# ShenhanQian/KGDet

Measured on AMD Instinct MI355X. Metric: training images/sec (whole node) KGDet R50-FPN 800x1333, higher is better.
Workload: dtype f32 (3 MFMA products per multiply on hi/lo-split operands -- fp16 parts forward, bf16 parts for gradients --, f32 accumulate); 1 GPU; KGDet R50-FPN train step, 2 img/GPU at 800x1333 (padded 800x1344), DeformConv fwd/bwd + focal/moment losses + grad-clip + Adam; no collective at dp1 (one rank: nothing to exchange); global_batch=2, parallelism=dp1

## Files before the change

include/kgdet_hip.h:

```cpp
#ifndef KGDET_HIP_H_
#define KGDET_HIP_H_

#include <stddef.h>
#include <stdint.h>

#ifdef __cplusplus
extern "C" {
#endif

#define KGDET_OK 0
#define KGDET_E_SHAPE 1
#define KGDET_E_WORKSPACE 2
#define KGDET_E_HIP 3
size_t kgdet_conv_packed_bytes(int32_t M, int32_t K, int32_t taps);
int kgdet_conv_pack(const float *w, int32_t O, int32_t C, int32_t taps, int32_t transpose, void *packed, void *stream);
int kgdet_conv_pack_fmt(const float *w, int32_t O, int32_t C, int32_t taps, int32_t transpose, void *packed,
                        int32_t operand_format, void *stream);
int kgdet_conv_pack_both_fmt(const float *w, int32_t O, int32_t C, int32_t taps, void *packed, void *packed_t,
                             int32_t forward_format, void *stream);
int kgdet_conv_apply_epilogue_fmt(const void *packed, const float *x, float *y, const float *bias, const float *residual,
                                  int32_t relu, int64_t B, int32_t M, int32_t K, int32_t H, int32_t W, int32_t taps,
                                  int32_t stride, int32_t operand_format, void *workspace, size_t workspace_bytes,
                                  void *stream);
int kgdet_conv_apply_gated_fmt(const void *packed, const float *x, float *y, const float *bias, const float *residual,
                               int32_t relu, const float *gate, int64_t B, int32_t M, int32_t K, int32_t H, int32_t W,
                               int32_t taps, int32_t stride, int32_t operand_format, void *workspace, size_t workspace_bytes,
                               void *stream);
int kgdet_stem_conv7x7_s2_fmt(const void *packed, const float *x, float *y, int64_t B, int32_t H, int32_t W,
                              int32_t operand_format, void *stream);
int kgdet_conv_pack_both(const float *w, int32_t O, int32_t C, int32_t taps, void *packed, void *packed_t, void *stream);
int64_t kgdet_conv_pack_blocks(int32_t O, int32_t C, int32_t taps);
int kgdet_conv_pack_multi(const int64_t *desc_dev, int32_t n, int64_t total_blocks, void *stream);
size_t kgdet_conv_apply_workspace_bytes(int64_t B, int32_t M, int32_t K, int32_t H, int32_t W, int32_t taps,
                                        int32_t stride);
int kgdet_conv_apply(const void *packed, const float *x, float *y, int64_t B, int32_t M, int32_t K, int32_t H, int32_t W,
                     int32_t taps, int32_t stride, void *workspace, size_t workspace_bytes, void *stream);
int kgdet_conv_apply_epilogue(const void *packed, const float *x, float *y, const float *bias, const float *residual,
                              int32_t relu, int64_t B, int32_t M, int32_t K, int32_t H, int32_t W, int32_t taps,
                              int32_t stride, void *workspace, size_t workspace_bytes, void *stream);
int kgdet_stem_conv7x7_s2(const void *packed, const float *x, float *y, int64_t B, int32_t H, int32_t W, void *stream);
int kgdet_conv3x3_s2_grad_input(const void *packed_t, const float *grad_y, float *grad_x, int64_t B, int32_t C, int32_t O,
                                int32_t Hin, int32_t Win, void *stream);
size_t kgdet_conv3x3_s2_grad_weight_workspace_bytes(int64_t B, int32_t O, int32_t C, int32_t H, int32_t W);
int kgdet_conv3x3_s2_grad_weight(const float *grad_y, const float *x, float *grad_w, int64_t B, int32_t O, int32_t C, int32_t H,
                                 int32_t W, void *workspace, size_t workspace_bytes, void *stream);
size_t kgdet_conv1x1_grad_weight_workspace_bytes(int64_t B, int32_t O, int32_t C, int64_t HW);
int kgdet_conv1x1_grad_weight(const float *grad_y, const float *x, float *grad_w, int64_t B, int32_t O, int32_t C,
                              int64_t HW, void *workspace, size_t workspace_bytes, void *stream);
size_t kgdet_conv3x3_grad_weight_workspace_bytes(int64_t B, int32_t O, int32_t C, int32_t H, int32_t W);
int kgdet_conv3x3_grad_weight(const float *grad_y, const float *x, float *grad_w, int64_t B, int32_t O, int32_t C,
                              int32_t H, int32_t W, void *workspace, size_t workspace_bytes, void *stream);

int kgdet_bn_act_forward(const float *x, const float *gamma, const float *beta, const float *mean, const float *var,
                         float eps, const float *residual, float *y, int64_t N, int32_t C, int64_t HW, int32_t relu,
                         void *stream);
int32_t kgdet_bn_act_partials(int64_t N, int32_t C, int64_t HW);
int kgdet_bn_act_backward(const float *grad_y, const float *x, const float *y, const float *gamma, const float *beta,
                          const float *mean, const float *var, float eps, int32_t has_residual, int32_t relu,
                          float *grad_x, float *grad_residual, float *partial, float *sums, int64_t N, int32_t C,
                          int64_t HW, void *stream);
int kgdet_conv1x1_nhwc_residual(const void *x, const void *weight, const float *bias, const void *residual, void *out,
                                int64_t M, int32_t K, int32_t N, int32_t relu, void *stream);
int kgdet_conv1x1_nhwc_residual_in(const void *x, const float *in_bias, const void *weight, const float *bias,
                                   const void *residual, void *out, int64_t M, int32_t K, int32_t N, int32_t relu,
                                   void *stream);
int kgdet_bn_fold_backward(const float *grad_z, const float *z, int32_t relu, float *g, float *partial, int64_t N, int32_t C,
                           int64_t HW, void *stream);
int kgdet_bn_fold_finish(const float *partial, int32_t P, const float *w, float *G , const float *s,
                         const float *mean, const float *var, float eps, float *grad_beta ,
                         float *grad_gamma , int32_t O, int32_t CK, void *stream);
int kgdet_conv1x1_grad_weight_fold(const float *grad_y, const float *x, float *grad_w, int64_t B, int32_t O, int32_t C,
                                   int64_t HW, void *workspace, size_t workspace_bytes, const float *w, const float *s,
                                   const float *mean, const float *var, float eps, const float *bn_partial, int32_t P,
                                   float *grad_beta , float *grad_gamma , void *stream);
int kgdet_conv3x3_grad_weight_fold(const float *grad_y, const float *x, float *grad_w, int64_t B, int32_t O, int32_t C,
                                   int32_t H, int32_t W, void *workspace, size_t workspace_bytes, const float *w,
                                   const float *s, const float *mean, const float *var, float eps, const float *bn_partial,
                                   int32_t P, float *grad_beta , float *grad_gamma , void *stream);
int kgdet_bn_relu_maxpool(const float *x, const float *gamma, const float *beta, const float *mean, const float *var,
                          float eps, float *y, int64_t N, int32_t C, int32_t H, int32_t W, void *stream);

int kgdet_bias_act(void *x, const float *bias, const void *residual, int64_t N, int32_t C, int64_t HW, int32_t dtype,
                   int32_t relu, int32_t channels_last, void *stream);
int kgdet_bias_relu_maxpool_nhwc(const void *x, const float *bias, void *y, int64_t N, int32_t C, int32_t H, int32_t W,
                                 int32_t dtype, void *stream);

#define KGDET_E_UNSUPPORTED 4
#define KGDET_E_PARTIAL 5

const char *kgdet_last_error(void);
int kgdet_version(void);
int kgdet_device_cu_count(void);

#define KGDET_OPT_EXACT_BACKWARD 0
#define KGDET_OPT_FWD_COLUMN_WAVE 1
#define KGDET_OPT_WGRAD_STREAMK 2
#define KGDET_OPT_BWD_PHASE 3
#define KGDET_OPT_COUNT 4
int kgdet_set_option(int32_t option, int32_t value);

typedef struct kgdet_dcn_shape {
  int32_t N, C, H, W;
  int32_t O, kh, kw;
  int32_t stride_h, stride_w, pad_h, pad_w, dil_h, dil_w;
  int32_t groups, deformable_groups;
  int32_t out_channel_offset, out_channels_total;
} kgdet_dcn_shape;

#define KGDET_DCN_RELU 1u
#define KGDET_DCN_BF16 2u
#define KGDET_DCN_EXACT_FP32 4u

int kgdet_dcn_output_size(const kgdet_dcn_shape *s, int32_t *Ho, int32_t *Wo);

size_t kgdet_dcn_packed_weight_bytes(const kgdet_dcn_shape *s);
size_t kgdet_dcn_workspace_bytes(const kgdet_dcn_shape *s);

int kgdet_dcn_pack_weight(const kgdet_dcn_shape *s, const float *weight, float *packed, void *stream);
int kgdet_dcn_pack_weight_multi(int32_t n, const kgdet_dcn_shape *const *shapes, const float *const *weights,
                                float *const *packeds, void *stream);
int kgdet_dcn_pack_weight_images(int32_t n, const kgdet_dcn_shape *const *shapes, const float *const *weights,
                                 float *const *packeds, uint32_t images, void *stream);
int32_t kgdet_dcn_split_path_complete(const kgdet_dcn_shape *shape);
int kgdet_dcn_unpack_weight_grad(const kgdet_dcn_shape *s, const float *packed, float *grad_weight,
                                 int accumulate, void *stream);

int kgdet_deform_conv_forward(const kgdet_dcn_shape *s, const float *input, const float *offset,
                              const float *mask , const float *packed_weight,
                              const float *bias , float *output, uint32_t flags,
                              void *workspace, size_t workspace_bytes, void *stream);

size_t kgdet_dcn_group_workspace_bytes(int32_t n, const kgdet_dcn_shape *const *shapes);

int kgdet_deform_conv_forward_grouped(int32_t n, const kgdet_dcn_shape *const *shapes, const float *const *inputs,
                                      const float *const *offsets, const float *const *masks ,
                                      const float *const *packed_weights, const float *const *biases ,
                                      float *const *outputs, uint32_t flags, void *workspace,
                                      size_t workspace_bytes, void *stream);

int kgdet_deform_conv_grad_input(const kgdet_dcn_shape *s, const float *offset, const float *mask ,
                                 const float *packed_weight, const float *grad_output, float *grad_input,
                                 uint32_t flags, void *workspace, size_t workspace_bytes, void *stream);

int kgdet_deform_conv_grad_offset(const kgdet_dcn_shape *s, const float *input, const float *offset,
                                  const float *packed_weight, const float *grad_output, float *grad_offset,
                                  uint32_t flags, void *workspace, size_t workspace_bytes, void *stream);

int kgdet_deform_conv_backward_input_grouped(int32_t n, const kgdet_dcn_shape *const *shapes, const float *const *inputs,
                                             const float *const *offsets, const float *const *packed_weights,
                                             const float *const *grad_outputs, float *const *grad_inputs,
                                             float *const *grad_offsets, void *workspace, size_t workspace_bytes,
                                             void *stream);

int kgdet_deform_conv_grad_weight_grouped(int32_t n, const kgdet_dcn_shape *const *shapes, const float *const *inputs,
                                          const float *const *offsets, const float *const *grad_outputs,
                                          float *const *grad_weights, void *workspace, size_t workspace_bytes,
                                          void *stream);

int kgdet_deform_conv_backward_input(const kgdet_dcn_shape *s, const float *input, const float *offset,
                                     const float *mask , const float *packed_weight,
                                     const float *grad_output, float *grad_input, float *grad_offset,
                                     float *grad_mask , void *workspace,
                                     size_t workspace_bytes, void *stream);

int kgdet_deform_conv_backward_weight(const kgdet_dcn_shape *s, const float *input, const float *offset,
                                      const float *mask , const float *grad_output,
                                      float *grad_weight, float *grad_bias , int accumulate,
                                      void *workspace, size_t workspace_bytes, void *stream);

typedef struct kgdet_psroi_shape {
  int32_t B, C, H, W;
  int32_t R;
  int32_t out_dim, group_size, pooled_size, part_size, sample_per_part;
  int32_t no_trans, num_classes;
  float spatial_scale, trans_std;
} kgdet_psroi_shape;

size_t kgdet_deform_psroi_forward_workspace_bytes(const kgdet_psroi_shape *s);
int kgdet_deform_psroi_forward(const kgdet_psroi_shape *s, const float *data, const float *rois,
                               const float *trans, float *out, float *count, void *workspace, size_t workspace_bytes,
                               void *stream);
size_t kgdet_deform_psroi_backward_workspace_bytes(const kgdet_psroi_shape *s);
int kgdet_deform_psroi_backward(const kgdet_psroi_shape *s, const float *grad_out, const float *count,
                                const float *data, const float *rois, const float *trans,
                                float *grad_data, float *grad_trans, void *workspace, size_t workspace_bytes,
                                void *stream);

int kgdet_sigmoid_focal_loss_forward(const float *logits, const int64_t *targets, int64_t num,
                                     int32_t num_classes, float gamma, float alpha, float *losses,
                                     void *stream);
int kgdet_sigmoid_focal_loss_backward(const float *logits, const int64_t *targets, const float *d_losses,
                                      int64_t num, int32_t num_classes, float gamma, float alpha,
                                      float *d_logits, void *stream);

#define KGDET_HEAD_MAX_IMAGES 16
typedef struct kgdet_head_targets {
  int32_t B, H, W, num_classes, num_keypoints;
  float stride;
  int32_t num_gt[KGDET_HEAD_MAX_IMAGES];
  const float *gt_bboxes[KGDET_HEAD_MAX_IMAGES];
  const int64_t *gt_labels[KGDET_HEAD_MAX_IMAGES];
  const float *gt_keypoints[KGDET_HEAD_MAX_IMAGES];
  int32_t valid_h[KGDET_HEAD_MAX_IMAGES], valid_w[KGDET_HEAD_MAX_IMAGES];
} kgdet_head_targets;
// ... 108 lines not shown
```

kgdet_amd/conv1x1.py:

```python
import ctypes
import weakref

import torch

from . import _lib


import os as _os
SPLIT_GRAD_WEIGHT_3X3 = _os.environ.get('KGDET_SPLIT_WGRAD3', '1') == '1'
PACK_BOTH = _os.environ.get('KGDET_PACK_BOTH', '1') == '1'


PAD_GRAD_WEIGHT_3X3 = _os.environ.get('KGDET_NO_WPAD') is None
DIRECT_ODD_MAPS = _os.environ.get('KGDET_DIRECT_ODD_MAPS', '1') == '1'
ENABLED = True


RAGGED_1X1 = _os.environ.get('KGDET_CONV_RAGGED_1X1', '1') == '1'


def applicable(x, weight, stride=(1, 1), padding=(0, 0), dilation=(1, 1), groups=1):
    k = weight.shape[2]
    aligned = weight.shape[1] % 16 == 0 and weight.shape[0] % 16 == 0
    return (ENABLED and x.is_cuda and x.dtype == torch.float32 and weight.dtype == torch.float32 and x.dim() == 4
            and weight.shape[2] == weight.shape[3] and k in (1, 3) and tuple(stride) == (1, 1)
            and tuple(padding) == (k // 2, k // 2) and tuple(dilation) == (1, 1) and groups == 1
            and x.is_contiguous() and (aligned or (k == 1 and RAGGED_1X1 and (weight.shape[0] * weight.shape[1]) % 2 == 0))
            and ((x.shape[2] * x.shape[3]) % 2 == 0 or DIRECT_ODD_MAPS) and x.shape[2] * x.shape[3] >= 4
            and not torch.is_autocast_enabled())


_L = None
_sizes = {}


def _lib_sizes():
    global _L
    if _L is None:
        L = _lib.lib()
        vp, i32, i64, sz = ctypes.c_void_p, ctypes.c_int32, ctypes.c_int64, ctypes.c_size_t
        for name, res, args in (
                ('kgdet_conv_packed_bytes', sz, [i32, i32, i32]),
                ('kgdet_conv_apply_workspace_bytes', sz, [i64, i32, i32, i32, i32, i32, i32]),
                ('kgdet_conv1x1_grad_weight_workspace_bytes', sz, [i64, i32, i32, i64]),
                ('kgdet_conv3x3_grad_weight_workspace_bytes', sz, [i64, i32, i32, i32, i32]),
                ('kgdet_conv_pack_fmt', ctypes.c_int, [vp, i32, i32, i32, i32, vp, i32, vp]),
                ('kgdet_conv_pack_both_fmt', ctypes.c_int, [vp, i32, i32, i32, vp, vp, i32, vp]),
                ('kgdet_conv_pack_blocks', i64, [i32, i32, i32]),
                ('kgdet_conv_pack_multi', ctypes.c_int, [vp, i32, i64, vp]),
                ('kgdet_conv_apply', ctypes.c_int, [vp, vp, vp, i64, i32, i32, i32, i32, i32, i32, vp, sz, vp]),
                ('kgdet_conv_apply_epilogue_fmt', ctypes.c_int,
                 [vp, vp, vp, vp, vp, i32, i64, i32, i32, i32, i32, i32, i32, i32, vp, sz, vp]),
                ('kgdet_conv_apply_gated_fmt', ctypes.c_int,
                 [vp, vp, vp, vp, vp, i32, vp, i64, i32, i32, i32, i32, i32, i32, i32, vp, sz, vp]),
                ('kgdet_conv3x3_s2_grad_input', ctypes.c_int, [vp, vp, vp, i64, i32, i32, i32, i32, vp]),
                ('kgdet_conv3x3_s2_grad_weight_workspace_bytes', sz, [i64, i32, i32, i32, i32]),
                ('kgdet_conv3x3_s2_grad_weight', ctypes.c_int, [vp, vp, vp, i64, i32, i32, i32, i32, vp, sz, vp]),
                ('kgdet_conv1x1_grad_weight', ctypes.c_int, [vp, vp, vp, i64, i32, i32, i64, vp, sz, vp]),
                ('kgdet_conv1x1_grad_weight_fold', ctypes.c_int,
                 [vp, vp, vp, i64, i32, i32, i64, vp, sz, vp, vp, vp, vp, ctypes.c_float, vp, i32, vp, vp, vp]),
                ('kgdet_conv3x3_grad_weight_fold', ctypes.c_int,
                 [vp, vp, vp, i64, i32, i32, i32, i32, vp, sz, vp, vp, vp, vp, ctypes.c_float, vp, i32, vp, vp, vp]),
                ('kgdet_conv3x3_grad_weight', ctypes.c_int, [vp, vp, vp, i64, i32, i32, i32, i32, vp, sz, vp])):
            fn = getattr(L, name)
            fn.restype, fn.argtypes = res, args
        _L = L
    return _L


def _size(name, *args):
    key = (name, args)
    n = _sizes.get(key)
    if n is None:
        n = _sizes[key] = getattr(_lib_sizes(), name)(*args)
    return n


def _stream():
    return _lib.raw_stream()


FORWARD_F16 = _os.environ.get('KGDET_CONV_FWD_F16', '1') == '1'


def _mark(img, f16):
    img.kgdet_f16 = bool(f16)
    return img


def _pack(weight, transpose):
    L = _lib_sizes()
    O, C, taps = weight.shape[0], weight.shape[1], weight.shape[2] * weight.shape[3]
    M, K = (C, O) if transpose else (O, C)
    img = torch.empty(_size('kgdet_conv_packed_bytes', M, K, taps), dtype=torch.uint8, device=weight.device)
    f16 = FORWARD_F16 and not transpose
    _lib.check(L.kgdet_conv_pack_fmt(weight.data_ptr(), O, C, taps, 1 if transpose else 0, img.data_ptr(), 1 if f16 else 0,
                                     _stream()), 'conv_pack')
    return _mark(img, f16)


def _pack_both(weight):
    L = _lib_sizes()
    O, C, taps = weight.shape[0], weight.shape[1], weight.shape[2] * weight.shape[3]
    img = torch.empty(_size('kgdet_conv_packed_bytes', O, C, taps), dtype=torch.uint8, device=weight.device)
    img_t = torch.empty(_size('kgdet_conv_packed_bytes', C, O, taps), dtype=torch.uint8, device=weight.device)
    _lib.check(L.kgdet_conv_pack_both_fmt(weight.data_ptr(), O, C, taps, img.data_ptr(), img_t.data_ptr(),
                                          1 if FORWARD_F16 else 0, _stream()), 'conv_pack_both')
    return _mark(img, FORWARD_F16), _mark(img_t, False)


def _apply(img, x, M, taps, stride=1, bias=None, residual=None, relu=False, gate=None):
    L = _lib_sizes()
    B, K, H, W = x.shape
    y = torch.empty((B, M, (H + stride - 1) // stride, (W + stride - 1) // stride), dtype=torch.float32, device=x.device)
    nbytes = _size('kgdet_conv_apply_workspace_bytes', B, M, K, H, W, taps, stride)
    ws = torch.empty(nbytes, dtype=torch.uint8, device=x.device) if nbytes else None
    if gate is not None and (gate.shape != y.shape or gate.dtype != torch.float32 or not gate.is_contiguous()):
        raise ValueError('gate must be a contiguous fp32 tensor of the output\'s shape')
    _lib.check(L.kgdet_conv_apply_gated_fmt(
        img.data_ptr(), x.data_ptr(), y.data_ptr(), bias.data_ptr() if bias is not None else None,
        residual.data_ptr() if residual is not None else None, 1 if relu else 0,
        gate.data_ptr() if gate is not None else None, B, M, K, H, W, taps, stride,
        1 if getattr(img, 'kgdet_f16', False) else 0, ws.data_ptr() if nbytes else None, nbytes, _stream()), 'conv_apply')
    return y


def gate_applicable(y_shape):
    return (y_shape[2] * y_shape[3]) % 2 == 0


class _Entry(object):
    __slots__ = ('ref', 'img', 'img_t', 'token', 'ptr')


_entries = {}
_token = 0
_generation = 0
_table = None
PACK_MULTI = _os.environ.get('KGDET_PACK_MULTI', '1') == '1'


FOLD_BN = _os.environ.get('KGDET_FOLD_BN', '1') == '1'


class _FoldEntry(object):
    __slots__ = ('ref', 'bn', 'img', 'img_t', 's', 't', 'token', 'ptr')


_fold_entries = {}
_fold_flat = None


def _fold_refresh(live):
    global _fold_flat
    key = tuple((k, e.ptr, id(e.bn()), id(e.bn().weight), id(e.bn().bias), id(e.bn().running_mean), id(e.bn().running_var),
                 e.bn().weight.data_ptr(), e.bn().running_var.data_ptr()) for k, e in live)
    if _fold_flat is None or _fold_flat[0] != key:
        dev = live[0][1].img.device
        sizes = [e.ref().shape[0] for _, e in live]
        total = sum(sizes)
        S, T, TMP = (torch.empty(total, dtype=torch.float32, device=dev) for _ in range(3))
        EPS = torch.cat([torch.full((n,), float(e.bn().eps), dtype=torch.float32) for n, (_, e) in zip(sizes, live)]).to(dev)
        sv, tv, mv, off = [], [], [], 0
        for n, (_, e) in zip(sizes, live):
            sv.append(S[off:off + n]); tv.append(T[off:off + n]); mv.append(TMP[off:off + n])
            e.s, e.t = sv[-1], tv[-1]
            off += n
        bns = [e.bn() for _, e in live]
        _fold_flat = (key, S, T, TMP, EPS, sv, tv, mv, [b.weight for b in bns], [b.bias for b in bns],
                      [b.running_mean for b in bns], [b.running_var for b in bns])
    _, S, T, TMP, EPS, sv, tv, mv, gammas, betas, means, vars_ = _fold_flat
    with torch.no_grad():
        torch._foreach_copy_(mv, vars_)
        TMP.add_(EPS).rsqrt_()
        torch._foreach_copy_(sv, gammas)
        S.mul_(TMP)
        torch._foreach_copy_(tv, means)
        T.mul_(S).neg_()
        torch._foreach_add_(tv, betas)


def _launch_multi():
    global _table
    dead = [k for k, e in _entries.items() if e.ref() is None or e.ref().data_ptr() != e.ptr]
    for k in dead:
        del _entries[k]
    dead = [k for k, e in _fold_entries.items() if e.ref() is None or e.bn() is None or e.ref().data_ptr() != e.ptr]
    for k in dead:
        del _fold_entries[k]
    for k in _fold_entries:
        _entries.pop(k, None)
    if not _entries and not _fold_entries:
        return
    live = list(_entries.items())
    folded = list(_fold_entries.items())
    if folded:
        _fold_refresh(folded)
    key = (tuple((k, e.ptr, e.img.data_ptr(), e.img_t.data_ptr()) for k, e in live),
           tuple((k, e.ptr, e.img.data_ptr(), e.img_t.data_ptr(), e.s.data_ptr()) for k, e in folded))
    L = _lib_sizes()
    if _table is None or _table[0] != key:
        rows, first = [], 0
        for _, e in live + folded:
            w = e.ref()
            O, C, taps = w.shape[0], w.shape[1], w.shape[2] * w.shape[3]
            rows.append([w.data_ptr(), e.img.data_ptr(), e.img_t.data_ptr(), (O << 32) | C,
                         (taps << 32) | first | ((1 << 62) if getattr(e.img, 'kgdet_f16', False) else 0),
                         e.s.data_ptr() if isinstance(e, _FoldEntry) else 0])
            first += L.kgdet_conv_pack_blocks(O, C, taps)
        dev = (live + folded)[0][1].img.device
        _table = (key, torch.tensor(rows, dtype=torch.int64).to(dev), first)
    _lib.check(L.kgdet_conv_pack_multi(_table[1].data_ptr(), len(live) + len(folded), _table[2], _stream()), 'conv_pack_multi')
    for _, e in live + folded:
        e.token = _token


def fold_images(weight, bn):
    if not (FOLD_BN and PACK_MULTI and _token):
        return None
    e = _fold_entries.get(id(weight))
    if e is not None and e.ref() is weight and e.ptr == weight.data_ptr() and e.bn() is bn:
        return (e.img, e.img_t, e.s, e.t) if e.token == _token else None
    O, C, taps = weight.shape[0], weight.shape[1], weight.shape[2] * weight.shape[3]
    if (isinstance(weight, torch.nn.Parameter) and weight.is_contiguous() and O % 16 == 0 and C % 16 == 0 and bn.affine
            and taps in (1, 9)):
        e = _FoldEntry()
        e.ref, e.bn, e.ptr, e.token = weakref.ref(weight), weakref.ref(bn), weight.data_ptr(), 0
        e.img = _mark(torch.empty(_size('kgdet_conv_packed_bytes', O, C, taps), dtype=torch.uint8, device=weight.device),
                      FORWARD_F16)
        e.img_t = _mark(torch.empty(_size('kgdet_conv_packed_bytes', C, O, taps), dtype=torch.uint8, device=weight.device), False)
        e.s = e.t = None
        _fold_entries[id(weight)] = e
    return None


class step_scope(object):

    def __enter__(self):
        global _token, _generation
        self.prev = _token
        _generation += 1
        _token = _generation
        if PACK_MULTI and (_entries or _fold_entries):
            _launch_multi()

    def __exit__(self, *exc):
        global _token
        _token = self.prev


_aliases = {}


def alias(proxy, param):
    key = id(proxy)
    _aliases[key] = (weakref.ref(proxy, lambda _r, key=key: _aliases.pop(key, None)), weakref.ref(param))


def forward_images(x, weight):
    both = PACK_BOTH and x.requires_grad and (weight.shape[0] % 16 == 0 or weight.shape[2] == 1)
    a = _aliases.get(id(weight))
    if a is not None and a[0]() is weight:
        origin = a[1]()
        if origin is not None and origin.data_ptr() == weight.data_ptr() and origin.shape == weight.shape:
            weight = origin
    if both and PACK_MULTI and _token:
        e = _entries.get(id(weight))
        if e is not None and e.ref() is weight and e.ptr == weight.data_ptr():
            if e.token != _token:
                _lib.check(_lib_sizes().kgdet_conv_pack_both_fmt(weight.data_ptr(), weight.shape[0], weight.shape[1],
                                                                 weight.shape[2] * weight.shape[3], e.img.data_ptr(),
                                                                 e.img_t.data_ptr(), 1 if getattr(e.img, 'kgdet_f16', False) else 0,
                                                                 _stream()), 'conv_pack_both')
                e.token = _token
            return e.img, e.img_t
        img, img_t = _pack_both(weight)
        if isinstance(weight, torch.nn.Parameter):
            e = _Entry()
            e.ref, e.img, e.img_t, e.token, e.ptr = weakref.ref(weight), img, img_t, _token, weight.data_ptr()
            _entries[id(weight)] = e
        return img, img_t
    if both:
        return _pack_both(weight)
    return _pack(weight, False), None


def grad_weight(x, weight, gy):
    O, C, k = weight.shape[0], weight.shape[1], weight.shape[2]
    L = _lib_sizes()
    if k == 3 and SPLIT_GRAD_WEIGHT_3X3 and C % 128 == 0:
        if x.shape[3] % 4 and not PAD_GRAD_WEIGHT_3X3:
            return torch.nn.grad.conv2d_weight(x, weight.shape, gy, padding=1)
        B, H, W = x.shape[0], x.shape[2], x.shape[3]
        nbytes = _size('kgdet_conv3x3_grad_weight_workspace_bytes', B, O, C, H, W)
        ws = torch.empty(nbytes, dtype=torch.uint8, device=x.device)
        gw = torch.empty_like(weight)
        _lib.check(L.kgdet_conv3x3_grad_weight(gy.data_ptr(), x.data_ptr(), gw.data_ptr(), B, O, C, H, W,
                                               ws.data_ptr(), nbytes, _stream()), 'conv3x3_grad_weight')
        return gw
    if k != 1 or ((x.shape[2] * x.shape[3]) % 4 != 0 and not PAD_GRAD_WEIGHT_3X3):
        return torch.nn.grad.conv2d_weight(x, weight.shape, gy, padding=k // 2)
    B, HW = x.shape[0], x.shape[2] * x.shape[3]
    nbytes = _size('kgdet_conv1x1_grad_weight_workspace_bytes', B, O, C, HW)
    ws = torch.empty(nbytes, dtype=torch.uint8, device=x.device)
    gw = torch.empty_like(weight)
    _lib.check(L.kgdet_conv1x1_grad_weight(gy.data_ptr(), x.data_ptr(), gw.data_ptr(), B, O, C, HW,
                                           ws.data_ptr(), nbytes, _stream()), 'conv1x1_grad_weight')
    return gw


def grad_weight_fold_route(x, weight):
    C, k = weight.shape[1], weight.shape[2]
    if k == 3 and SPLIT_GRAD_WEIGHT_3X3 and C % 128 == 0 and (x.shape[3] % 4 == 0 or PAD_GRAD_WEIGHT_3X3):
        return 3
    if k == 1 and ((x.shape[2] * x.shape[3]) % 4 == 0 or PAD_GRAD_WEIGHT_3X3):
        return 1
    return 0


def grad_weight_fold(x, weight, gy, s, mean, var, eps, bn_partial, P, want_gamma=True):
    O, C, k = weight.shape[0], weight.shape[1], weight.shape[2]
    L = _lib_sizes()
    if bn_partial is None:
        P = 0

        class bn_partial(object):
            @staticmethod
            def data_ptr():
                return None
    if k == 3 and SPLIT_GRAD_WEIGHT_3X3 and C % 128 == 0 and (x.shape[3] % 4 == 0 or PAD_GRAD_WEIGHT_3X3):
        B, H, W = x.shape[0], x.shape[2], x.shape[3]
        nbytes = _size('kgdet_conv3x3_grad_weight_workspace_bytes', B, O, C, H, W)
        ws = torch.empty(nbytes, dtype=torch.uint8, device=x.device)
        gw = torch.empty_like(weight)
        sums = torch.empty((2, O), dtype=torch.float32, device=x.device)
        _lib.check(L.kgdet_conv3x3_grad_weight_fold(gy.data_ptr(), x.data_ptr(), gw.data_ptr(), B, O, C, H, W, ws.data_ptr(), nbytes,
                                                    weight.data_ptr(), s.data_ptr(), mean.data_ptr(), var.data_ptr(), eps,
                                                    bn_partial.data_ptr(), P, sums[0].data_ptr(),
                                                    sums[1].data_ptr() if want_gamma else None, _stream()), 'conv3x3_grad_weight_fold')
        return gw, sums
    if k == 1 and ((x.shape[2] * x.shape[3]) % 4 == 0 or PAD_GRAD_WEIGHT_3X3):
        B, HW = x.shape[0], x.shape[2] * x.shape[3]
        nbytes = _size('kgdet_conv1x1_grad_weight_workspace_bytes', B, O, C, HW)
        ws = torch.empty(nbytes, dtype=torch.uint8, device=x.device)
        gw = torch.empty_like(weight)
        sums = torch.empty((2, O), dtype=torch.float32, device=x.device)
        _lib.check(L.kgdet_conv1x1_grad_weight_fold(gy.data_ptr(), x.data_ptr(), gw.data_ptr(), B, O, C, HW, ws.data_ptr(), nbytes,
                                                    weight.data_ptr(), s.data_ptr(), mean.data_ptr(), var.data_ptr(), eps,
                                                    bn_partial.data_ptr(), P, sums[0].data_ptr(),
                                                    sums[1].data_ptr() if want_gamma else None, _stream()), 'conv1x1_grad_weight_fold')
        return gw, sums
    return None


def grad_input(weight, img_t, gy, residual=None, gate=None):
    C, k = weight.shape[1], weight.shape[2]
    return _apply(img_t if img_t is not None else _pack(weight, True), gy, C, k * k, residual=residual, gate=gate)


class _ConvSplit(torch.autograd.Function):
    @staticmethod
    def forward(ctx, x, weight):
        weight = weight.contiguous()
        img, ctx.img_t = forward_images(x, weight)
        ctx.save_for_backward(x, weight)
        return _apply(img, x, weight.shape[0], weight.shape[2] * weight.shape[3])

    @staticmethod
    def backward(ctx, gy):
        x, weight = ctx.saved_tensors
        gy = gy.contiguous()
        gx = grad_input(weight, ctx.img_t, gy) if ctx.needs_input_grad[0] else None
        gw = grad_weight(x, weight, gy) if ctx.needs_input_grad[1] else None
        return gx, gw


def conv_split(x, weight):
    return _ConvSplit.apply(x, weight)


PAD_ODD_MAPS = _os.environ.get('KGDET_PAD_ODD_MAPS', '1') == '1'


def odd_map_applicable(x, weight, stride=(1, 1), padding=(0, 0), dilation=(1, 1), groups=1):
    return (PAD_ODD_MAPS and x.dim() == 4 and (x.shape[2] * x.shape[3]) % 2 == 1 and x.shape[2] % 2 == 1 and x.is_cuda
            and x.dtype == torch.float32 and x.is_contiguous()
            and applicable(_PadProbe(x), weight, stride, padding, dilation, groups))


class _PadProbe(object):

    def __init__(self, x):
        self.is_cuda, self.dtype = x.is_cuda, x.dtype
        self.shape = (x.shape[0], x.shape[1], x.shape[2], x.shape[3] + 1)

    def dim(self):
        return 4

    def is_contiguous(self):
        return True


def pad_odd(x):
    return torch.nn.functional.pad(x, (0, 1))


def unpad_odd(y, width):
    return y[..., :width].contiguous()


conv1x1 = conv_split


BIAS_GRAD_IN_WGRAD = _os.environ.get('KGDET_BIAS_GRAD_IN_WGRAD', '1') == '1'
_ones_cache = {}


def _ones(n, device):
    t = _ones_cache.get((n, device))
    if t is None:
        t = _ones_cache[(n, device)] = torch.ones(n, dtype=torch.float32, device=device)
    return t


class _ConvBiasAct(torch.autograd.Function):

    @staticmethod
    def forward(ctx, x, weight, bias, relu):
        weight = weight.contiguous()
        img, ctx.img_t = forward_images(x, weight)
        y = _apply(img, x, weight.shape[0], weight.shape[2] * weight.shape[3], 1, bias.contiguous(), None, relu)
        ctx.relu = relu
        ctx.save_for_backward(x, weight, y if relu else None)
        return y

    @staticmethod
    def backward(ctx, gy):
        x, weight, y = ctx.saved_tensors
        if ctx.relu:
            gy = torch.ops.aten.threshold_backward(gy, y, 0)
        gy = gy.contiguous()
        gx = grad_input(weight, ctx.img_t, gy) if ctx.needs_input_grad[0] else None
        if BIAS_GRAD_IN_WGRAD and ctx.needs_input_grad[1] and ctx.needs_input_grad[2] and grad_weight_fold_route(x, weight):
            one = _ones(weight.shape[0], weight.device)
            res = grad_weight_fold(x, weight, gy, one, one, one, 0.0, None, 0, want_gamma=False)
            if res is not None:
                return gx, res[0], res[1][0], None
        gw = grad_weight(x, weight, gy) if ctx.needs_input_grad[1] else None
        gb = gy.sum((0, 2, 3)) if ctx.needs_input_grad[2] else None
        return gx, gw, gb, None


CACHE_INFER_CASTS = _os.environ.get('KGDET_CACHE_INFER_CASTS', '1') == '1'


GEMM_1X1_NCHW = _os.environ.get('KGDET_INFER_GEMM_1X1_NCHW', '1') == '1'


_cast_cache = weakref.WeakKeyDictionary()


def invalidate_inference_caches():
    global _fold_flat
    _cast_cache.clear()
    _fold_flat = None
    from . import backbone, dcn
    backbone.clear_fold_cache()
    dcn.clear_pack_cache()


def conv_infer(conv, x):
    if (CACHE_INFER_CASTS and type(conv) is torch.nn.Conv2d and not torch.is_grad_enabled() and x.is_cuda
            and torch.is_autocast_enabled() and conv.weight.dtype == torch.float32 and conv.padding_mode == 'zeros'):
        dt = torch.get_autocast_dtype('cuda')
        cl = x.dim() == 4 and not x.is_contiguous() and x.is_contiguous(memory_format=torch.channels_last)
        key = (conv.weight._version, conv.weight.data_ptr(), id(conv.weight),
               None if conv.bias is None else (conv.bias._version, conv.bias.data_ptr(), id(conv.bias)), dt, cl)
        c = _cast_cache.get(conv)
        if c is None or c[0] != key:
            w = conv.weight.detach().to(dt)
            if cl:
                w = w.contiguous(memory_format=torch.channels_last)
            c = (key, w, None if conv.bias is None else conv.bias.detach().to(dt))
            _cast_cache[conv] = c
        if (GEMM_1X1_NCHW and not cl and x.dim() == 4 and x.is_contiguous() and x.dtype == dt and conv.kernel_size == (1, 1)
                and conv.stride == (1, 1) and conv.padding == (0, 0) and conv.groups == 1):
            B, _, H, W = x.shape
            y = torch.matmul(c[1].view(c[1].shape[0], -1), x.view(B, x.shape[1], H * W))
            if c[2] is not None:
                y += c[2].view(1, -1, 1)
            return y.view(B, -1, H, W)
        return torch.nn.functional.conv2d(x, c[1], c[2], conv.stride, conv.padding, conv.dilation, conv.groups)
    return conv(x)


def conv_bias_act(conv, x, relu=False):
    if (type(conv) is torch.nn.Conv2d and conv.bias is not None and torch.is_grad_enabled()
            and conv.bias.dtype == torch.float32
            and applicable(x, conv.weight, conv.stride, conv.padding, conv.dilation, conv.groups)):
        return _ConvBiasAct.apply(x, conv.weight, conv.bias, relu)
    if (type(conv) is torch.nn.Conv2d and conv.bias is not None and torch.is_grad_enabled() and conv.bias.dtype == torch.float32
            and odd_map_applicable(x, conv.weight, conv.stride, conv.padding, conv.dilation, conv.groups)):
        return unpad_odd(_ConvBiasAct.apply(pad_odd(x), conv.weight, conv.bias, relu), x.shape[3])
    y = conv_infer(conv, x)
    return torch.relu(y) if relu else y


class _ConvSplitStride2(torch.autograd.Function):

    @staticmethod
# ... 54 lines not shown
```

kgdet_amd/csrc/conv1x1.hip:

```cpp
#include "common.h"

namespace kgdet {

namespace {

typedef __bf16 bf16x8 __attribute__((ext_vector_type(8)));
typedef float f32x16 __attribute__((ext_vector_type(16)));
typedef float f32x4 __attribute__((ext_vector_type(4)));
typedef float f32x2 __attribute__((ext_vector_type(2)));

constexpr int kTM = 128, kTN = 128, kTK = 16;
constexpr int kPart = 2 * kTM * 16;
constexpr int kStage = 2 * kPart;

typedef __bf16 bf16x2 __attribute__((ext_vector_type(2)));
__device__ __forceinline__ void split_pair(float v0, float v1, unsigned &hi, unsigned &lo) {
  const f32x2 v = {v0, v1};
  hi = __builtin_bit_cast(unsigned, __builtin_convertvector(v, bf16x2));
  const f32x2 hf = {__uint_as_float(hi << 16), __uint_as_float(hi & 0xffff0000u)};
  lo = __builtin_bit_cast(unsigned, __builtin_convertvector(v - hf, bf16x2));
}
__device__ __forceinline__ void split8(const float (&v)[8], bf16x8 &hi, bf16x8 &lo) {
  typedef unsigned u32x4 __attribute__((ext_vector_type(4)));
  u32x4 h, l;
// ... 277 lines not shown
    }
    const float *xp = xb + (long long)(c16 * kTK + kq * 4) * Nin + shift;
    if (TAPS == 1 && (K & (kTK - 1)) && c16 == K / kTK) {
#pragma unroll
      for (int j = 0; j < 4; ++j) R.v[j] = xb[(long long)min(c16 * kTK + kq * 4 + j, K - 1) * Nin];
    } else {
#pragma unroll
      for (int j = 0; j < 4; ++j) R.v[j] = xp[(long long)j * Nin];
    }
  };
  auto commit = [&](int buf, const Regs &R) {
    unsigned char *As = smem + buf * kBuf, *Bs = As + kStage;
    *reinterpret_cast<f32x4 *>(As + (tid & 511) * 16) = R.a;
    uint2 hi, lo;
#ifdef KGDET_CONV_ABL_NOSPLIT
    hi.x = __float_as_uint(R.v[0]); hi.y = __float_as_uint(R.v[1]); lo.x = __float_as_uint(R.v[2]); lo.y = __float_as_uint(R.v[3]);
#else
    split_pair_t<F16>(R.live ? R.v[0] : 0.0f, R.live ? R.v[1] : 0.0f, hi.x, lo.x);
    split_pair_t<F16>(R.live ? R.v[2] : 0.0f, R.live ? R.v[3] : 0.0f, hi.y, lo.y);
#endif
    unsigned char *dst = Bs + (kq >> 1) * (TN * 16) + n_local * 16 + (kq & 1) * 8;
    *reinterpret_cast<uint2 *>(dst) = hi;
    *reinterpret_cast<uint2 *>(dst + kPartB) = lo;
  };
  auto multiply = [&](int buf) {
    const unsigned char *A = smem + buf * kBuf + (lane >> 5) * (kTM * 16) + (wm * 64 + (lane & 31)) * 16;
    const unsigned char *Bp = smem + buf * kBuf + kStage + (lane >> 5) * (TN * 16) + (wn * 32 + (lane & 31)) * 16;
    bf16x8 a[2][2], bb[2];
#ifdef KGDET_CONV_ABL_NOLDSREAD
#pragma unroll
    for (int pt = 0; pt < 2; ++pt) {
      a[pt][0] = __builtin_bit_cast(bf16x8, acc[0].lo.lo); a[pt][1] = __builtin_bit_cast(bf16x8, acc[1].lo.lo);
      bb[pt] = __builtin_bit_cast(bf16x8, acc[1].hi.lo);
    }
#else
#pragma unroll
    for (int pt = 0; pt < 2; ++pt) {
      a[pt][0] = *reinterpret_cast<const bf16x8 *>(A + pt * kPart);
      a[pt][1] = *reinterpret_cast<const bf16x8 *>(A + pt * kPart + 32 * 16);
      bb[pt] = *reinterpret_cast<const bf16x8 *>(Bp + pt * kPartB);
    }
#endif
#ifdef KGDET_CONV_ABL_NOMFMA
#pragma unroll
    for (int mi = 0; mi < 2; ++mi) {
      const f32x4 q = __builtin_bit_cast(f32x4, a[0][mi]) + __builtin_bit_cast(f32x4, a[1][mi]) + __builtin_bit_cast(f32x4, bb[0]) + __builtin_bit_cast(f32x4, bb[1]);
      acc[mi][0] += q[0]; acc[mi][1] += q[1]; acc[mi][2] += q[2]; acc[mi][3] += q[3];
    }
    if (false)
#endif
#pragma unroll
    for (int mi = 0; mi < 2; ++mi) {
      acc[mi] = mfma_t<F16>(a[1][mi], bb[0], acc[mi]);
      acc[mi] = mfma_t<F16>(a[0][mi], bb[1], acc[mi]);
      acc[mi] = mfma_t<F16>(a[0][mi], bb[0], acc[mi]);
    }
  };
  {
    Regs R[kPF];
#pragma unroll
    for (int i = 0; i < kPF; ++i) issue(i, R[i]);
#ifdef KGDET_GATE_EARLY
    if (!F16 && gate) {
#pragma unroll
      for (int mi = 0; mi < 2; ++mi)
#pragma unroll
        for (int r = 0; r < 16; ++r) asm volatile("" : "+v"(gv[mi][r]));
    }
#endif
    commit(0, R[0]);
    const int full = stages / kPF * kPF;
    for (int s0 = 0; s0 < full; s0 += kPF) {
#pragma unroll
      for (int u = 0; u < kPF; ++u) {
        const int s = s0 + u;
        __syncthreads();
        issue(s + kPF, R[u]);
        multiply(s & 1);
        commit((s + 1) & 1, R[(u + 1) % kPF]);
      }
    }
#pragma unroll
    for (int u = 0; u < kPF - 1; ++u) {
      const int s = full + u;
      if (s < stages) {
        __syncthreads();
        multiply(s & 1);
        if (s + 1 < stages) commit((s + 1) & 1, R[u + 1]);
      }
    }
  }

  float *yb = y + (long long)part * part_stride + (long long)b * M * N;
  const int n = n0 + wn * 32 + (lane & 31);
  if constexpr (F16) {
#pragma unroll
    for (int mi = 0; mi < 2; ++mi)
#pragma unroll
      for (int r = 0; r < 16; ++r) acc[mi][r] *= 1.0f / kF16WeightScale;
  }
  if (bias || residual) {
    const int nc = min(n, N - 1);
    float add[2][16];
#pragma unroll
    for (int mi = 0; mi < 2; ++mi)
#pragma unroll
      for (int r = 0; r < 16; ++r) {
        const int m = min(mt * kTM + wm * 64 + mi * 32 + (r & 3) + 8 * (r >> 2) + 4 * (lane >> 5), M - 1);
        float v = bias ? bias[m] : 0.0f;
        if (residual) v += residual[((long long)b * M + m) * N + nc];
        add[mi][r] = v;
      }
#pragma unroll
    for (int mi = 0; mi < 2; ++mi)
#pragma unroll
      for (int r = 0; r < 16; ++r) acc[mi][r] += add[mi][r];
  }
  if (gate) {
#ifdef KGDET_GATE_EARLY
    if constexpr (F16)
#endif
    {
    const int nc = min(n, N - 1);
#pragma unroll
    for (int mi = 0; mi < 2; ++mi)
#pragma unroll
      for (int r = 0; r < 16; ++r) {
        const int m = min(mt * kTM + wm * 64 + mi * 32 + (r & 3) + 8 * (r >> 2) + 4 * (lane >> 5), M - 1);
        gv[mi][r] = gate[((long long)b * M + m) * N + nc];
      }
    }
#pragma unroll
    for (int mi = 0; mi < 2; ++mi)
#pragma unroll
      for (int r = 0; r < 16; ++r) acc[mi][r] = gv[mi][r] > 0.0f ? acc[mi][r] : 0.0f;
  }
#pragma unroll
  for (int mi = 0; mi < 2; ++mi)
#pragma unroll
    for (int r = 0; r < 16; ++r) {
      const int m = mt * kTM + wm * 64 + mi * 32 + (r & 3) + 8 * (r >> 2) + 4 * (lane >> 5);
      if (m < M && n < N) yb[(long long)m * N + n] = relu ? fmaxf(acc[mi][r], 0.0f) : acc[mi][r];
    }
}

#ifdef KGDET_CONV_TRACE
static __device__ unsigned long long g_conv_trace[1024 * 8];
#define CV_NOW() __builtin_amdgcn_s_memtime()
#define CV_ADD(cat) do { const unsigned long long n__ = CV_NOW(); tr[cat] += n__ - tr_t; tr_t = n__; } while (0)
#else
#define CV_ADD(cat) do { } while (0)
#endif
constexpr int kPatchMax = 256;
constexpr int kPatchPart = 2 * kPatchMax * 16;
constexpr int kPatchBuf = 2 * kPatchPart;
constexpr int kPatchLds = 6 * kStage + 2 * kPatchBuf;

__global__ __launch_bounds__(kNNThreads) void conv3x3_patch(const unsigned char *__restrict__ img,
                                                            const float *__restrict__ x, float *__restrict__ y, int M,
                                                            int K, int H, int W, int n_mt, int tiles_x, int n_nt, int tiles,
                                                            int ksplit, long long part_stride, int TX, int TY,
                                                            const float *__restrict__ bias,
                                                            const float *__restrict__ residual, int relu,
    const float *__restrict__ gate = nullptr) {
  extern __shared__ __attribute__((aligned(16))) unsigned char smem[];
  const int unit = xcd_tile(blockIdx.x, tiles * ksplit);
  if (unit >= tiles * ksplit) return;
  const int part = unit % ksplit, tile = unit / ksplit;
  const int tid = threadIdx.x, lane = tid & 63, wave = tid >> 6, wm = wave & 1, wn = wave >> 1;
  const int N = H * W;
  const int chunks_all = K / kTK, per = (chunks_all + ksplit - 1) / ksplit;
  const int c_begin = part * per, c_end = max(c_begin, min(chunks_all, c_begin + per));
  const int chunks = c_end - c_begin, stages = chunks * 9;
  const int mt = tile % n_mt, nt = (tile / n_mt) % n_nt, b = tile / (n_mt * n_nt);
  const int y0 = (nt / tiles_x) * TY, x0 = (nt % tiles_x) * TX;
  const int PW = TX + 2, PP = PW * (TY + 2);

  const int khalf_l = tid >> 8, pp = tid & 255;
  const int ppy = pp / PW, ppx = pp - ppy * PW;
  const int iy = y0 - 1 + ppy, ix = x0 - 1 + ppx;
  const bool p_live = pp < PP && iy >= 0 && iy < H && ix >= 0 && ix < W;
  const float *xb = x + ((long long)b * K + khalf_l * 8) * N + (p_live ? iy * W + ix : 0);
  unsigned char *b_dst = smem + 6 * kStage + (khalf_l * kPatchMax + pp) * 16;

  const int q = min(wn * 32 + (lane & 31), TX * TY - 1);
  const int py = q / TX, px = q - py * TX;
  const unsigned char *b_row0 = smem + 6 * kStage + ((lane >> 5) * kPatchMax + py * PW + px) * 16;
  const int row_pitch = PW * 16;
  const unsigned char *a_rd = smem + (lane >> 5) * (kTM * 16) + (wm * 64 + (lane & 31)) * 16;
  const unsigned char *ai = img + (long long)mt * (chunks_all * 9) * kStage + (long long)min(c_begin, chunks_all - 1) * 9 * kStage + tid * 16;

  f32x16 acc[2];
#pragma unroll
  for (int i = 0; i < 2; ++i)
#pragma unroll
    for (int r = 0; r < 16; ++r) acc[i][r] = 0.0f;

  float bv[8];
  auto issue_b = [&](int ci) {
    const float *xp = xb + (long long)min(c_begin + min(ci, chunks - 1), chunks_all - 1) * kTK * N;
#pragma unroll
    for (int j = 0; j < 8; ++j) bv[j] = xp[(long long)j * N];
  };
  auto commit_b = [&](int buf) {
    float v[8];
#pragma unroll
    for (int j = 0; j < 8; ++j) asm volatile("" : "+v"(bv[j]));
#pragma unroll
    for (int j = 0; j < 8; ++j) v[j] = p_live ? bv[j] : 0.0f;
    bf16x8 hi, lo;
    split8(v, hi, lo);
    *reinterpret_cast<bf16x8 *>(b_dst + buf * kPatchBuf) = hi;
    *reinterpret_cast<bf16x8 *>(b_dst + buf * kPatchBuf + kPatchPart) = lo;
  };
  f32x4 R[3];
#ifdef KGDET_PATCH_ABL_NOAGLOBAL
  auto issue_a = [&](int s, f32x4 &r) { r[0] = (float)s; };
#else
  auto issue_a = [&](int s, f32x4 &r) { r = *reinterpret_cast<const f32x4 *>(ai + (long long)max(min(s, stages - 1), 0) * kStage); };
#endif

  struct Frags {
    bf16x8 a[2][2], b[2];
  };
  auto read_frags = [&](Frags &F, const unsigned char *A, const unsigned char *Bp) {
#ifdef KGDET_PATCH_ABL_NOLDSREAD
#pragma unroll
    for (int pt = 0; pt < 2; ++pt) {
      F.a[pt][0] = __builtin_bit_cast(bf16x8, acc[0].lo.lo); F.a[pt][1] = __builtin_bit_cast(bf16x8, acc[1].lo.lo);
      F.b[pt] = __builtin_bit_cast(bf16x8, acc[1].hi.lo);
    }
    return;
#endif
#pragma unroll
    for (int pt = 0; pt < 2; ++pt) {
      F.a[pt][0] = *reinterpret_cast<const bf16x8 *>(A + pt * kPart);
      F.a[pt][1] = *reinterpret_cast<const bf16x8 *>(A + pt * kPart + 32 * 16);
      F.b[pt] = *reinterpret_cast<const bf16x8 *>(Bp + pt * kPatchPart);
    }
  };
  auto mma = [&](const Frags &F) {
#ifdef KGDET_PATCH_ABL_NOMFMA
#pragma unroll
    for (int mi = 0; mi < 2; ++mi) {
      const f32x4 qv = __builtin_bit_cast(f32x4, F.a[0][mi]) + __builtin_bit_cast(f32x4, F.a[1][mi]) + __builtin_bit_cast(f32x4, F.b[0]) + __builtin_bit_cast(f32x4, F.b[1]);
      acc[mi][0] += qv[0]; acc[mi][1] += qv[1]; acc[mi][2] += qv[2]; acc[mi][3] += qv[3];
    }
    return;
#endif
#pragma unroll
    for (int mi = 0; mi < 2; ++mi) {
      acc[mi] = __builtin_amdgcn_mfma_f32_32x32x16_bf16(F.a[1][mi], F.b[0], acc[mi], 0, 0, 0);
      acc[mi] = __builtin_amdgcn_mfma_f32_32x32x16_bf16(F.a[0][mi], F.b[1], acc[mi], 0, 0, 0);
      acc[mi] = __builtin_amdgcn_mfma_f32_32x32x16_bf16(F.a[0][mi], F.b[0], acc[mi], 0, 0, 0);
    }
  };
#ifdef KGDET_CONV_TRACE
  unsigned long long tr[8] = {0, 0, 0, 0, 0, 0, 0, 0};
  unsigned long long tr_t = CV_NOW();
  const unsigned long long tr_start = tr_t;
#endif
  issue_b(0);
#pragma unroll
  for (int j = 0; j < 3; ++j) issue_a(j, R[j]);
  commit_b(0);
#pragma unroll
  for (int j = 0; j < 3; ++j) {
    *reinterpret_cast<f32x4 *>(smem + j * kStage + tid * 16) = R[j];
    issue_a(3 + j, R[j]);
  }
  Frags F[2];
  CV_ADD(5);
  for (int ci = 0; ci < chunks; ++ci) {
    issue_b(ci + 1);
    const unsigned char *brow = b_row0 + (ci & 1) * kPatchBuf;
    const int set0 = (ci & 1) * 3 * kStage;
#pragma unroll
    for (int r = 0; r < 3; ++r) {
      const int g = ci * 3 + r;
      const int cur = (r & 1) ? 3 * kStage - set0 : set0, nxt = 3 * kStage - cur;
#ifndef KGDET_PATCH_ABL_NOBARRIER
      __syncthreads();
#endif
      CV_ADD(0);
      read_frags(F[0], a_rd + cur, brow + r * row_pitch);
#pragma unroll
      for (int j = 0; j < 3; ++j) {
        if (j < 2) read_frags(F[(j + 1) & 1], a_rd + cur + (j + 1) * kStage, brow + r * row_pitch + (j + 1) * 16);
        __builtin_amdgcn_sched_barrier(0);
        CV_ADD(1);
        mma(F[j & 1]);
        __builtin_amdgcn_sched_barrier(0);
        CV_ADD(2);
        *reinterpret_cast<f32x4 *>(smem + nxt + j * kStage + tid * 16) = R[j];
        issue_a(3 * (g + 2) + j, R[j]);
        if (r == 2 && j == 1) commit_b((ci + 1) & 1);
        __builtin_amdgcn_sched_barrier(0);
        CV_ADD(3);
      }
    }
  }

#ifdef KGDET_CONV_TRACE
  tr[6] = CV_NOW() - tr_start;
  tr[7] = stages;
  tr[4] = ((unsigned long long)__builtin_amdgcn_s_getreg((20 << 0) | (0 << 6) | (31 << 11)) << 32) |
          __builtin_amdgcn_s_getreg((4 << 0) | (0 << 6) | (31 << 11));
  tr[5] = tr_start;
  if (tid == 0 && blockIdx.x < 1024)
    for (int c = 0; c < 8; ++c) g_conv_trace[blockIdx.x * 8 + c] = tr[c];
#endif
  float *yb = y + (long long)part * part_stride + (long long)b * M * N;
  const int qq = wn * 32 + (lane & 31);
  const int oy = y0 + py, ox = x0 + px;
  const bool o_live = qq < TX * TY && oy < H && ox < W;
  const int n = o_live ? oy * W + ox : 0;
  if (bias || residual) {
    float add[2][16];
#pragma unroll
    for (int mi = 0; mi < 2; ++mi)
#pragma unroll
      for (int r = 0; r < 16; ++r) {
        const int m = min(mt * kTM + wm * 64 + mi * 32 + (r & 3) + 8 * (r >> 2) + 4 * (lane >> 5), M - 1);
        float v = bias ? bias[m] : 0.0f;
        if (residual) v += residual[((long long)b * M + m) * N + n];
        add[mi][r] = v;
      }
#pragma unroll
    for (int mi = 0; mi < 2; ++mi)
#pragma unroll
      for (int r = 0; r < 16; ++r) acc[mi][r] += add[mi][r];
  }
  if (gate) {
    float gv[2][16];
#pragma unroll
    for (int mi = 0; mi < 2; ++mi)
#pragma unroll
      for (int r = 0; r < 16; ++r) {
        const int m = min(mt * kTM + wm * 64 + mi * 32 + (r & 3) + 8 * (r >> 2) + 4 * (lane >> 5), M - 1);
        gv[mi][r] = gate[((long long)b * M + m) * N + n];
      }
#pragma unroll
    for (int mi = 0; mi < 2; ++mi)
#pragma unroll
      for (int r = 0; r < 16; ++r) acc[mi][r] = gv[mi][r] > 0.0f ? acc[mi][r] : 0.0f;
  }
#pragma unroll
  for (int mi = 0; mi < 2; ++mi)
#pragma unroll
    for (int r = 0; r < 16; ++r) {
      const int m = mt * kTM + wm * 64 + mi * 32 + (r & 3) + 8 * (r >> 2) + 4 * (lane >> 5);
      if (m < M && o_live) yb[(long long)m * N + n] = relu ? fmaxf(acc[mi][r], 0.0f) : acc[mi][r];
    }
}

template <int WAVES, int NB, bool F16 = false>
__global__ __launch_bounds__(64 * WAVES) void conv3x3_patch4(const unsigned char *__restrict__ img,
                                                             const float *__restrict__ x, float *__restrict__ y, int M,
                                                             int K, int H, int W, int n_mt, int tiles_x, int n_nt,
                                                             int tiles, int ksplit, long long part_stride, int TX, int TY,
                                                             const float *__restrict__ bias,
                                                             const float *__restrict__ residual, int relu,
    const float *__restrict__ gate = nullptr) {
  __shared__ __attribute__((aligned(16))) unsigned char smem[2 * kPatchBuf];
  if constexpr (F16) f16_saturate_on();
  constexpr int HALVES = 4 / WAVES, THREADS = 64 * WAVES, PXT = kPatchMax / THREADS;
  const int unit0 = xcd_tile(blockIdx.x, tiles * ksplit * HALVES);
  if (unit0 >= tiles * ksplit * HALVES) return;
  const int half = unit0 % HALVES, unit = unit0 / HALVES;
  const int part = unit % ksplit, tile = unit / ksplit;
  const int tid = threadIdx.x, lane = tid & 63, wave = (tid >> 6) + half * WAVES;
  const int N = H * W;
  const int chunks_all = K / kTK, per = (chunks_all + ksplit - 1) / ksplit;
  const int c_begin = part * per, c_end = max(c_begin, min(chunks_all, c_begin + per));
  const int chunks = c_end - c_begin, stages = chunks * 9;
  const int mt = tile % n_mt, nt = (tile / n_mt) % n_nt, b = tile / (n_mt * n_nt);
  const int y0 = (nt / tiles_x) * TY, x0 = (nt % tiles_x) * TX;
  const int PW = TX + 2, PP = PW * (TY + 2);

  if (mt * kTM + half * 64 >= M) return;
  bool p_live[PXT];
  int p_off[PXT];
#pragma unroll
  for (int i = 0; i < PXT; ++i) {
    const int pp = tid + i * THREADS;
    const int ppy = pp / PW, ppx = pp - ppy * PW;
    const int iy = y0 - 1 + ppy, ix = x0 - 1 + ppx;
    p_live[i] = pp < PP && iy >= 0 && iy < H && ix >= 0 && ix < W;
    p_off[i] = p_live[i] ? iy * W + ix : 0;
  }
  const float *xb = x + (long long)b * K * N;
  unsigned char *b_dst = smem + tid * 16;

  int b_rd[NB], o_n[NB];
  bool o_live[NB];
#pragma unroll
  for (int nb = 0; nb < NB; ++nb) {
    const int qq = nb * 32 + (lane & 31), q = min(qq, TX * TY - 1);
    const int py = q / TX, px = q - py * TX;
    b_rd[nb] = ((lane >> 5) * kPatchMax + py * PW + px) * 16;
    o_live[nb] = qq < TX * TY && y0 + py < H && x0 + px < W;
    o_n[nb] = o_live[nb] ? (y0 + py) * W + x0 + px : 0;
  }
  const int row_pitch = PW * 16;
  const unsigned char *ag = img + ((long long)mt * chunks_all + min(c_begin, chunks_all - 1)) * 9 * kStage +
                            (lane >> 5) * (kTM * 16) + (wave * 32 + (lane & 31)) * 16;

  f32x16 acc[NB];
#pragma unroll
  for (int i = 0; i < NB; ++i)
#pragma unroll
    for (int r = 0; r < 16; ++r) acc[i][r] = 0.0f;

  float bv[PXT][16];
  auto issue_b = [&](int ci) {
    const float *xp = xb + (long long)min(c_begin + min(ci, chunks - 1), chunks_all - 1) * kTK * N;
#pragma unroll
    for (int i = 0; i < PXT; ++i)
#pragma unroll
      for (int j = 0; j < 16; ++j) bv[i][j] = xp[(long long)j * N + p_off[i]];
  };
  auto commit_b = [&](int buf) {
#pragma unroll
    for (int i = 0; i < PXT; ++i)
#pragma unroll
      for (int j = 0; j < 16; ++j) asm volatile("" : "+v"(bv[i][j]));
#pragma unroll
    for (int i = 0; i < PXT; ++i)
#pragma unroll
      for (int kh = 0; kh < 2; ++kh) {
        float v[8];
#pragma unroll
        for (int j = 0; j < 8; ++j) v[j] = p_live[i] ? bv[i][kh * 8 + j] : 0.0f;
        bf16x8 hi, lo;
        split8_t<F16>(v, hi, lo);
        unsigned char *d = b_dst + i * THREADS * 16 + buf * kPatchBuf + kh * (kPatchMax * 16);
        *reinterpret_cast<bf16x8 *>(d) = hi;
        *reinterpret_cast<bf16x8 *>(d + kPatchPart) = lo;
      }
  };
  bf16x8 AR[3][2];
  auto issue_a = [&](int s, bf16x8 (&r)[2]) {
    const unsigned char *p = ag + (long long)max(min(s, stages - 1), 0) * kStage;
    r[0] = *reinterpret_cast<const bf16x8 *>(p);
    r[1] = *reinterpret_cast<const bf16x8 *>(p + kPart);
  };

  issue_b(0);
#pragma unroll
  for (int j = 0; j < 3; ++j) issue_a(j, AR[j]);
  commit_b(0);
  for (int ci = 0; ci < chunks; ++ci) {
    issue_b(ci + 1);
    __syncthreads();
    const unsigned char *bbuf = smem + (ci & 1) * kPatchBuf;
#pragma unroll
    for (int t = 0; t < 9; ++t) {
      const int s = ci * 9 + t;
      const unsigned char *bt = bbuf + (t / 3) * row_pitch + (t % 3) * 16;
      bf16x8 bf[NB][2];
#pragma unroll
      for (int nb = 0; nb < NB; ++nb) {
        bf[nb][0] = *reinterpret_cast<const bf16x8 *>(bt + b_rd[nb]);
        bf[nb][1] = *reinterpret_cast<const bf16x8 *>(bt + b_rd[nb] + kPatchPart);
      }
#pragma unroll
      for (int nb = 0; nb < NB; ++nb) acc[nb] = mfma_t<F16>(AR[t % 3][1], bf[nb][0], acc[nb]);
#pragma unroll
      for (int nb = 0; nb < NB; ++nb) acc[nb] = mfma_t<F16>(AR[t % 3][0], bf[nb][1], acc[nb]);
#pragma unroll
      for (int nb = 0; nb < NB; ++nb) acc[nb] = mfma_t<F16>(AR[t % 3][0], bf[nb][0], acc[nb]);
      __builtin_amdgcn_sched_barrier(0);
      issue_a(s + 3, AR[t % 3]);
      if (t == 6) commit_b((ci + 1) & 1);
      __builtin_amdgcn_sched_barrier(0);
    }
  }

  float *yb = y + (long long)part * part_stride + (long long)b * M * N;
  const int m0 = mt * kTM + wave * 32 + 4 * (lane >> 5);
#pragma unroll
  for (int nb = 0; nb < NB; ++nb) {
    if constexpr (F16) {
#pragma unroll
      for (int r = 0; r < 16; ++r) acc[nb][r] *= 1.0f / kF16WeightScale;
    }
    if (bias || residual) {
      float add[16];
#pragma unroll
      for (int r = 0; r < 16; ++r) {
        const int m = min(m0 + (r & 3) + 8 * (r >> 2), M - 1);
        float v = bias ? bias[m] : 0.0f;
        if (residual) v += residual[((long long)b * M + m) * N + o_n[nb]];
        add[r] = v;
      }
#pragma unroll
      for (int r = 0; r < 16; ++r) acc[nb][r] += add[r];
    }
    if (gate) {
      float gv[16];
#pragma unroll
      for (int r = 0; r < 16; ++r) gv[r] = gate[((long long)b * M + min(m0 + (r & 3) + 8 * (r >> 2), M - 1)) * N + o_n[nb]];
#pragma unroll
      for (int r = 0; r < 16; ++r) acc[nb][r] = gv[r] > 0.0f ? acc[nb][r] : 0.0f;
    }
#pragma unroll
    for (int r = 0; r < 16; ++r) {
      const int m = m0 + (r & 3) + 8 * (r >> 2);
      if (m < M && o_live[nb]) yb[(long long)m * N + o_n[nb]] = relu ? fmaxf(acc[nb][r], 0.0f) : acc[nb][r];
    }
  }
}

__global__ __launch_bounds__(256) void conv3x3_s2_grad_input(const unsigned char *__restrict__ img_t,
                                                             const float *__restrict__ gy, float *__restrict__ gx, int M,
                                                             int K, int H, int W, int Hin, int Win, int n_mt, int tiles_x,
                                                             int n_nt, int tiles, int TX, int TY) {
  __shared__ __attribute__((aligned(16))) unsigned char smem[2 * kPatchBuf];
  constexpr int NB = 2;
  const int tile = xcd_tile(blockIdx.x, tiles);
  if (tile >= tiles) return;
  const int tid = threadIdx.x, lane = tid & 63, wave = tid >> 6;
  const int N = H * W;
  const int chunks = K / kTK, stages = chunks * 9;
  const int mt = tile % n_mt, nt = (tile / n_mt) % n_nt, b = tile / (n_mt * n_nt);
  const int y0 = (nt / tiles_x) * TY, x0 = (nt % tiles_x) * TX;
  const int PW = TX + 2, PP = PW * (TY + 2);

  const int pp = tid;
  const int ppy = pp / PW, ppx = pp - ppy * PW;
  const int iy = y0 - 1 + ppy, ix = x0 - 1 + ppx;
  const bool p_live = pp < PP && iy >= 0 && iy < H && ix >= 0 && ix < W;
  const float *xb = gy + (long long)b * K * N + (p_live ? iy * W + ix : 0);
  unsigned char *b_dst = smem + pp * 16;

  int b_rd[NB], o_y[NB], o_x[NB];
#pragma unroll
  for (int nb = 0; nb < NB; ++nb) {
    const int qq = nb * 32 + (lane & 31), q = min(qq, TX * TY - 1);
    const int py = q / TX, px = q - py * TX;
    b_rd[nb] = ((lane >> 5) * kPatchMax + py * PW + px) * 16;
    const bool live = qq < TX * TY && y0 + py < H && x0 + px < W;
    o_y[nb] = live ? 2 * (y0 + py) : Hin;
    o_x[nb] = 2 * (x0 + px);
  }
  const int row_pitch = PW * 16;
  const unsigned char *ag = img_t + (long long)mt * stages * kStage + (lane >> 5) * (kTM * 16) + (wave * 32 + (lane & 31)) * 16;

  f32x16 acc[4][NB];
#pragma unroll
  for (int c = 0; c < 4; ++c)
#pragma unroll
    for (int i = 0; i < NB; ++i)
#pragma unroll
      for (int r = 0; r < 16; ++r) acc[c][i][r] = 0.0f;

  float bv[16];
  auto issue_b = [&](int ci) {
    const float *xp = xb + (long long)min(ci, chunks - 1) * kTK * N;
#pragma unroll
    for (int j = 0; j < 16; ++j) bv[j] = xp[(long long)j * N];
  };
  auto commit_b = [&](int buf) {
#pragma unroll
    for (int j = 0; j < 16; ++j) asm volatile("" : "+v"(bv[j]));
#pragma unroll
    for (int kh = 0; kh < 2; ++kh) {
      float v[8];
#pragma unroll
      for (int j = 0; j < 8; ++j) v[j] = p_live ? bv[kh * 8 + j] : 0.0f;
      bf16x8 hi, lo;
      split8(v, hi, lo);
      *reinterpret_cast<bf16x8 *>(b_dst + buf * kPatchBuf + kh * (kPatchMax * 16)) = hi;
      *reinterpret_cast<bf16x8 *>(b_dst + buf * kPatchBuf + kh * (kPatchMax * 16) + kPatchPart) = lo;
    }
  };
  bf16x8 AR[3][2];
  auto issue_a = [&](int s, bf16x8 (&r)[2]) {
    const int sc = min(s, stages - 1), ci = sc / 9, t = sc - ci * 9;
    const unsigned char *p = ag + (long long)(ci * 9 + 8 - t) * kStage;
    r[0] = *reinterpret_cast<const bf16x8 *>(p);
    r[1] = *reinterpret_cast<const bf16x8 *>(p + kPart);
  };

  issue_b(0);
#pragma unroll
  for (int j = 0; j < 3; ++j) issue_a(j, AR[j]);
  commit_b(0);
  for (int ci = 0; ci < chunks; ++ci) {
    issue_b(ci + 1);
    __syncthreads();
    const unsigned char *bbuf = smem + (ci & 1) * kPatchBuf;
#pragma unroll
    for (int t = 0; t < 9; ++t) {
      constexpr int kDummy = 0;
      const int ky = t / 3, kx = t % 3;
      const int cls = 2 * (ky != 1) + (kx != 1), dy = ky == 0, dx = kx == 0;
      const unsigned char *bt = bbuf + (1 + dy) * row_pitch + (1 + dx) * 16;
      bf16x8 bf[NB][2];
#pragma unroll
      for (int nb = 0; nb < NB; ++nb) {
        bf[nb][0] = *reinterpret_cast<const bf16x8 *>(bt + b_rd[nb]);
        bf[nb][1] = *reinterpret_cast<const bf16x8 *>(bt + b_rd[nb] + kPatchPart);
      }
#pragma unroll
      for (int nb = 0; nb < NB; ++nb) acc[cls][nb] = __builtin_amdgcn_mfma_f32_32x32x16_bf16(AR[t % 3][1], bf[nb][0], acc[cls][nb], 0, 0, 0);
#pragma unroll
      for (int nb = 0; nb < NB; ++nb) acc[cls][nb] = __builtin_amdgcn_mfma_f32_32x32x16_bf16(AR[t % 3][0], bf[nb][1], acc[cls][nb], 0, 0, 0);
#pragma unroll
      for (int nb = 0; nb < NB; ++nb) acc[cls][nb] = __builtin_amdgcn_mfma_f32_32x32x16_bf16(AR[t % 3][0], bf[nb][0], acc[cls][nb], 0, 0, 0);
      __builtin_amdgcn_sched_barrier(0);
      issue_a(ci * 9 + t + 3, AR[t % 3]);
      if (t == 6) commit_b((ci + 1) & 1);
      __builtin_amdgcn_sched_barrier(0);
      (void)kDummy;
    }
  }

  const long long Nin = (long long)Hin * Win;
  float *xo = gx + (long long)b * M * Nin;
  const int m0 = mt * kTM + wave * 32 + 4 * (lane >> 5);
#pragma unroll
  for (int nb = 0; nb < NB; ++nb)
#pragma unroll
    for (int r = 0; r < 16; ++r) {
      const int m = m0 + (r & 3) + 8 * (r >> 2);
      if (m >= M) continue;
      float *row = xo + (long long)m * Nin;
#pragma unroll
      for (int pa = 0; pa < 2; ++pa) {
        const int oy = o_y[nb] + pa;
        if (oy >= Hin) continue;
#pragma unroll
        for (int qa = 0; qa < 2; ++qa)
          if (o_x[nb] + qa < Win) row[(long long)oy * Win + o_x[nb] + qa] = acc[2 * pa + qa][nb][r];
      }
    }
}

constexpr int kStemTY = 8, kStemTX = 16, kStemPH = 2 * kStemTY + 5, kStemPW = 2 * kStemTX + 5, kStemK = 160;

template <bool F16>
__global__ __launch_bounds__(256) void stem_conv7x7_s2(const unsigned char *__restrict__ img, const float *__restrict__ x,
                                                       float *__restrict__ y, int H, int W, int Ho, int Wo, int tiles_x,
                                                       int tiles_per_image) {
  __shared__ float patch[3 * kStemPH * kStemPW];
  __shared__ int koff[kStemK];
  if constexpr (F16) f16_saturate_on();
  const int tid = threadIdx.x, lane = tid & 63, wave = tid >> 6;
  const int b = blockIdx.x / tiles_per_image, nt = blockIdx.x - b * tiles_per_image;
  const int oy0 = (nt / tiles_x) * kStemTY, ox0 = (nt % tiles_x) * kStemTX;
  const int iy0 = 2 * oy0 - 3, ix0 = 2 * ox0 - 3;
  const float *xb = x + (long long)b * 3 * H * W;
  for (int i = tid; i < 3 * kStemPH * kStemPW; i += 256) {
    const int c = i / (kStemPH * kStemPW), r = i - c * (kStemPH * kStemPW), py = r / kStemPW, px = r - py * kStemPW;
    const int iy = iy0 + py, ix = ix0 + px;
    patch[i] = (iy >= 0 && iy < H && ix >= 0 && ix < W) ? xb[((long long)c * H + iy) * W + ix] : 0.0f;
  }
  if (tid < kStemK) {
    const int c = tid / 49, r = tid - c * 49, ky = r / 7, kx = r - ky * 7;
    koff[tid] = tid < 147 ? c * (kStemPH * kStemPW) + ky * kStemPW + kx : 0;
  }
  __syncthreads();
  const int q = wave * 32 + (lane & 31), py = q / kStemTX, px = q - py * kStemTX;
  const float *pbase = patch + (2 * py) * kStemPW + 2 * px;
  const int kh = (lane >> 5) * 8;
  const unsigned char *ag = img + (lane >> 5) * (kTM * 16) + (lane & 31) * 16;
  f32x16 acc[2];
#pragma unroll
  for (int i = 0; i < 2; ++i)
#pragma unroll
    for (int r = 0; r < 16; ++r) acc[i][r] = 0.0f;
#pragma unroll
  for (int s = 0; s < kStemK / kTK; ++s) {
    bf16x8 a[2][2];
#pragma unroll
    for (int mi = 0; mi < 2; ++mi) {
      a[0][mi] = *reinterpret_cast<const bf16x8 *>(ag + (long long)s * kStage + mi * 32 * 16);
      a[1][mi] = *reinterpret_cast<const bf16x8 *>(ag + (long long)s * kStage + kPart + mi * 32 * 16);
    }
    float v[8];
#pragma unroll
    for (int j = 0; j < 8; ++j) v[j] = pbase[koff[s * kTK + kh + j]];
    bf16x8 bhi, blo;
    split8_t<F16>(v, bhi, blo);
#pragma unroll
    for (int mi = 0; mi < 2; ++mi) {
      acc[mi] = mfma_t<F16>(a[1][mi], bhi, acc[mi]);
      acc[mi] = mfma_t<F16>(a[0][mi], blo, acc[mi]);
      acc[mi] = mfma_t<F16>(a[0][mi], bhi, acc[mi]);
    }
  }
  const int oy = oy0 + py, ox = ox0 + px;
  if (oy < Ho && ox < Wo) {
    float *yb = y + (long long)b * 64 * Ho * Wo + (long long)oy * Wo + ox;
#pragma unroll
    for (int mi = 0; mi < 2; ++mi)
#pragma unroll
      for (int r = 0; r < 16; ++r) {
        const int m = mi * 32 + (r & 3) + 8 * (r >> 2) + 4 * (lane >> 5);
        yb[(long long)m * Ho * Wo] = F16 ? acc[mi][r] * (1.0f / kF16WeightScale) : acc[mi][r];
      }
  }
}

__global__ __launch_bounds__(256) void conv1x1_sum(const float *__restrict__ parts, float *__restrict__ out,
                                                   long long n, long long stride, int count) {
  for (long long i = (blockIdx.x * 256LL + threadIdx.x) * 2; i < n; i += gridDim.x * 512LL) {
    f32x2 s = {0.0f, 0.0f};
    int k = 0;
    for (; k + 8 <= count; k += 8) {
      f32x2 v[8];
#pragma unroll
      for (int e = 0; e < 8; ++e) v[e] = *reinterpret_cast<const f32x2 *>(parts + (long long)(k + e) * stride + i);
#pragma unroll
      for (int e = 0; e < 8; ++e) s += v[e];
    }
    for (; k + 2 <= count; k += 2) {
      const f32x2 v0 = *reinterpret_cast<const f32x2 *>(parts + (long long)k * stride + i);
      const f32x2 v1 = *reinterpret_cast<const f32x2 *>(parts + (long long)(k + 1) * stride + i);
      s = (s + v0) + v1;
    }
    for (; k < count; ++k) s += *reinterpret_cast<const f32x2 *>(parts + (long long)k * stride + i);
    *reinterpret_cast<f32x2 *>(out + i) = s;
  }
}

__global__ __launch_bounds__(256) void conv1x1_sum_epilogue(const float *__restrict__ parts, float *__restrict__ out,
                                                            long long n, long long stride, int count,
                                                            const float *__restrict__ bias, const float *__restrict__ residual,
                                                            int relu, int M, long long HW,
                                                            const float *__restrict__ gate = nullptr) {
  for (long long i = (blockIdx.x * 256LL + threadIdx.x) * 2; i < n; i += gridDim.x * 512LL) {
    f32x2 s = {0.0f, 0.0f};
    int k = 0;
    for (; k + 4 <= count; k += 4) {
      f32x2 v[4];
#pragma unroll
      for (int e = 0; e < 4; ++e) v[e] = *reinterpret_cast<const f32x2 *>(parts + (long long)(k + e) * stride + i);
#pragma unroll
      for (int e = 0; e < 4; ++e) s += v[e];
    }
    for (; k < count; ++k) s += *reinterpret_cast<const f32x2 *>(parts + (long long)k * stride + i);
    if (bias) {
      const float b = bias[(i / HW) % M];
      s[0] += b; s[1] += b;
    }
    if (residual) s += *reinterpret_cast<const f32x2 *>(residual + i);
    if (relu) { s[0] = fmaxf(s[0], 0.0f); s[1] = fmaxf(s[1], 0.0f); }
    if (gate) {
      const f32x2 gv = *reinterpret_cast<const f32x2 *>(gate + i);
      s[0] = gv[0] > 0.0f ? s[0] : 0.0f; s[1] = gv[1] > 0.0f ? s[1] : 0.0f;
    }
    *reinterpret_cast<f32x2 *>(out + i) = s;
  }
}

struct ConvFoldArgs {
  const float *w, *s, *mean, *var, *bn_partial;
  float *grad_beta, *grad_gamma;
  float eps;
  int P;
};
template <bool T9>
__global__ __launch_bounds__(1024) void conv_wsum_fold(const float *__restrict__ parts, float *__restrict__ out, int C,
                                                       long long stride, int count, const ConvFoldArgs f) {
  extern __shared__ float row_s[];
  __shared__ float red[2][16];
  const int o = blockIdx.x, CK = T9 ? 9 * C : C;
  const int nthr = blockDim.x, tid = threadIdx.x;
  const float so = f.s[o];
  const float *wr = f.w + (long long)o * CK;
  const float *pr = parts + (long long)o * CK;
  float *gr = out + (long long)o * CK;
  float dot = 0.0f, sb = 0.0f;
  for (int q = tid; q < CK; q += nthr) {
    float g0 = 0.0f;
    int k = 0;
    for (; k + 16 <= count; k += 16) {
      float v[16];
#pragma unroll
      for (int e = 0; e < 16; ++e) v[e] = pr[(long long)(k + e) * stride + q];
#pragma unroll
      for (int e = 0; e < 16; ++e) g0 += v[e];
    }
    if (k + 8 <= count) {
      float v[8];
#pragma unroll
      for (int e = 0; e < 8; ++e) v[e] = pr[(long long)(k + e) * stride + q];
#pragma unroll
      for (int e = 0; e < 8; ++e) g0 += v[e];
      k += 8;
    }
    for (; k < count; ++k) g0 += pr[(long long)k * stride + q];
    if constexpr (T9) {
      row_s[(q % C) * 9 + q / C] = g0;
    } else {
      dot += wr[q] * g0;
      gr[q] = g0 * so;
    }
  }
  if constexpr (T9) {
    __syncthreads();
    for (int j = tid; j < CK; j += nthr) {
      const float g0 = row_s[j];
      dot += wr[j] * g0;
      gr[j] = g0 * so;
    }
  }
  for (int k = tid; k < f.P; k += nthr) sb += f.bn_partial[(long long)o * f.P + k];
#pragma unroll
  for (int d = 32; d > 0; d >>= 1) { dot += __shfl_xor(dot, d); sb += __shfl_xor(sb, d); }
  if ((tid & 63) == 0) { red[0][tid >> 6] = sb; red[1][tid >> 6] = dot; }
  __syncthreads();
  if (tid == 0) {
    float b = 0.0f, d = 0.0f;
    for (int w = 0; w < (nthr >> 6); ++w) { b += red[0][w]; d += red[1][w]; }
    if (f.grad_beta) f.grad_beta[o] = b;
    if (f.grad_gamma) f.grad_gamma[o] = (d - f.mean[o] * b) / sqrtf(f.var[o] + f.eps);
  }
}

__global__ __launch_bounds__(256) void conv3x3_wsum(const float *__restrict__ parts, float *__restrict__ out, int O, int C,
                                                    int count) {
  const long long n = (long long)O * C * 9;
  for (long long i = blockIdx.x * 256LL + threadIdx.x; i < n; i += gridDim.x * 256LL) {
    const int o = (int)(i / (9 * C)), rem = (int)(i - (long long)o * 9 * C), t = rem / C, ch = rem - t * C;
    float s = 0.0f;
    int k = 0;
    for (; k + 8 <= count; k += 8) {
      float v[8];
#pragma unroll
      for (int e = 0; e < 8; ++e) v[e] = parts[(long long)(k + e) * n + i];
#pragma unroll
      for (int e = 0; e < 8; ++e) s += v[e];
    }
    for (; k < count; ++k) s += parts[(long long)k * n + i];
    out[((long long)o * C + ch) * 9 + t] = s;
  }
}

template <int TAPS, int DX>
__device__ __forceinline__ void conv_nt8_body(const float *__restrict__ a, const float *__restrict__ bm,
                                              float *__restrict__ partial, int M, int N, int L, int B, int n_mt, int n_nt,
                                              int stages_per_image, int per, int H, int W, int Cin, int unit,
                                              unsigned char *smem, float *__restrict__ row_sums, int rs_stride) {
  const int tile = unit % (n_mt * n_nt), split = unit / (n_mt * n_nt);
  const int mt = tile % n_mt, nt = tile / n_mt;
  const int tid = threadIdx.x, lane = tid & 63, wave = tid >> 6, wm = wave & 1, wn = wave >> 1;
  const int row = tid >> 2, q = tid & 3;
  const bool rs_on = row_sums != nullptr && nt == 0;
  float rs = 0.0f;
  const int total = B * stages_per_image;
  const int s_begin = split * per, s_end = min(total, s_begin + per);
  const int am = min(mt * kTM + row, M - 1);
  const bool a_real = mt * kTM + row < M;
  const int tap = TAPS == 9 ? (nt * kTN) / Cin : 0;
  const int dy = TAPS == 9 ? tap / 3 - 1 : 0;
  constexpr int dx = DX, off = dx < 0 ? -4 : 0, sh = dx - off;
  constexpr int NB = (TAPS == 9 && dx != 0) ? 8 : 4;
  const int bcols = TAPS == 9 ? Cin : N;
  const int bn_raw = TAPS == 9 ? nt * kTN - tap * Cin + row : nt * kTN + row;
  const int bn = min(bn_raw, bcols - 1);
  const bool b_real = bn_raw < bcols;
  const float inv_w = 1.0f / (float)W;

  f32x16 acc[2];
#pragma unroll
  for (int i = 0; i < 2; ++i)
#pragma unroll
    for (int r = 0; r < 16; ++r) acc[i][r] = 0.0f;

  struct Regs {
    f32x4 va;
    float vb[NB];
    int p0;
  };
  auto issue = [&](int s, Regs &R) {
    const int sc = min(s, s_end - 1);
    const int img = sc / stages_per_image, st = sc - img * stages_per_image;
    const int p0 = st * kTK + q * 4;
    R.p0 = p0;
    const float *ap = a + ((long long)img * M + am) * L, *bp = bm + ((long long)img * bcols + bn) * L;
    R.va = *reinterpret_cast<const f32x4 *>(ap + min(p0, L - 4));
    const int base = p0 + dy * W + off;
#pragma unroll
    for (int k = 0; k < NB / 4; ++k) {
      const f32x4 w = *reinterpret_cast<const f32x4 *>(bp + min(max(base + 4 * k, 0), L - 4));
#pragma unroll
      for (int e = 0; e < 4; ++e) R.vb[4 * k + e] = w[e];
    }
  };
  auto commit = [&](int buf, const Regs &R, bool real = true) {
    unsigned char *As = smem + buf * 2 * kStage, *Bs = As + kStage;
    const bool in_img = R.p0 < L;
    bool row_ok = in_img && b_real;
    int w0 = 0;
    if (TAPS == 9) {
      const int h = (int)(((float)R.p0 + 0.5f) * inv_w);
      w0 = R.p0 - h * W;
      row_ok = row_ok && h + dy >= 0 && h + dy < H;
    }
    float fa[4], fb[4];
#pragma unroll
    for (int i = 0; i < 4; ++i) {
      fa[i] = (in_img && a_real) ? R.va[i] : 0.0f;
      const int col = w0 + i + dx;
      const bool ok = TAPS == 9 ? (row_ok && col >= 0 && col < W) : row_ok;
      fb[i] = ok ? R.vb[i + (TAPS == 9 ? sh : 0)] : 0.0f;
    }
    if (rs_on && real) rs += (fa[0] + fa[1]) + (fa[2] + fa[3]);
    uint2 ahi, alo, bhi, blo;
    split_pair(fa[0], fa[1], ahi.x, alo.x);
    split_pair(fa[2], fa[3], ahi.y, alo.y);
    split_pair(fb[0], fb[1], bhi.x, blo.x);
    split_pair(fb[2], fb[3], bhi.y, blo.y);
    const int o = (q >> 1) * (kTM * 16) + row * 16 + (q & 1) * 8;
    *reinterpret_cast<uint2 *>(As + o) = ahi;
    *reinterpret_cast<uint2 *>(As + kPart + o) = alo;
    *reinterpret_cast<uint2 *>(Bs + o) = bhi;
    *reinterpret_cast<uint2 *>(Bs + kPart + o) = blo;
  };
  auto multiply = [&](int buf) {
    const unsigned char *A = smem + buf * 2 * kStage + (lane >> 5) * (kTM * 16) + (wm * 64 + (lane & 31)) * 16;
    const unsigned char *Bp = smem + buf * 2 * kStage + kStage + (lane >> 5) * (kTN * 16) + (wn * 32 + (lane & 31)) * 16;
    bf16x8 fa[2][2], fb[2];
#pragma unroll
    for (int pt = 0; pt < 2; ++pt) {
      fa[pt][0] = *reinterpret_cast<const bf16x8 *>(A + pt * kPart);
      fa[pt][1] = *reinterpret_cast<const bf16x8 *>(A + pt * kPart + 32 * 16);
      fb[pt] = *reinterpret_cast<const bf16x8 *>(Bp + pt * kPart);
    }
#pragma unroll
    for (int mi = 0; mi < 2; ++mi) {
      acc[mi] = __builtin_amdgcn_mfma_f32_32x32x16_bf16(fa[1][mi], fb[0], acc[mi], 0, 0, 0);
      acc[mi] = __builtin_amdgcn_mfma_f32_32x32x16_bf16(fa[0][mi], fb[1], acc[mi], 0, 0, 0);
      acc[mi] = __builtin_amdgcn_mfma_f32_32x32x16_bf16(fa[0][mi], fb[0], acc[mi], 0, 0, 0);
    }
  };
  constexpr int PF = 4;
  const int n = s_end - s_begin;
  if (n > 0) {
    Regs R[PF];
#pragma unroll
    for (int i = 0; i < PF; ++i) issue(s_begin + i, R[i]);
    commit(0, R[0]);
    const int full = n / PF * PF;
    for (int j0 = 0; j0 < full; j0 += PF) {
#pragma unroll
      for (int u = 0; u < PF; ++u) {
        const int j = j0 + u;
        __syncthreads();
        issue(s_begin + j + PF, R[u]);
        multiply(j & 1);
        commit((j + 1) & 1, R[(u + 1) % PF], j + 1 < n);
      }
    }
#pragma unroll
    for (int u = 0; u < PF - 1; ++u) {
      const int j = full + u;
      if (j < n) {
        __syncthreads();
        multiply(j & 1);
        if (j + 1 < n) commit((j + 1) & 1, R[u + 1]);
      }
    }
  }
  float *out = partial + (long long)split * M * N;
  const int nn = nt * kTN + wn * 32 + (lane & 31);
#pragma unroll
  for (int mi = 0; mi < 2; ++mi)
#pragma unroll
    for (int r = 0; r < 16; ++r) {
      const int m = mt * kTM + wm * 64 + mi * 32 + (r & 3) + 8 * (r >> 2) + 4 * (lane >> 5);
      if (m < M && nn < N) out[(long long)m * N + nn] = acc[mi][r];
    }
  if (rs_on) {
    rs += __shfl_xor(rs, 1);
    rs += __shfl_xor(rs, 2);
    if (q == 0 && a_real) row_sums[(long long)(mt * kTM + row) * rs_stride + split] = rs;
  }
}

template <int TAPS>
__global__ __launch_bounds__(kNNThreads) void conv_nt8(const float *__restrict__ a, const float *__restrict__ bm,
                                                       float *__restrict__ partial, int M, int N, int L, int B, int n_mt,
                                                       int n_nt, int stages_per_image, int per, int H, int W, int Cin,
                                                       int units, float *__restrict__ row_sums = nullptr, int rs_stride = 0) {
  __shared__ __attribute__((aligned(16))) unsigned char smem[2 * 2 * kStage];
  const int unit = units > 0 ? xcd_tile(blockIdx.x, units) : (int)blockIdx.x;
  if (units > 0 && unit >= units) return;
  if (TAPS == 9) {
// ... 103 lines not shown
          w0 = p0 - h0 * W;
          row_ok = row_ok && (unsigned)(h0 + dy) < (unsigned)H;
        }
        ok[0] = row_ok && (TAPS == 1 || dx >= 0 || w0 > 0);
        ok[1] = ok[2] = row_ok;
        ok[3] = row_ok && (TAPS == 1 || dx <= 0 || w0 + 4 < W);
      } else {
        const int h0 = TAPS == 9 ? (int)(((float)p0 + 0.5f) * inv_w) : 0;
        const int w0 = p0 - h0 * W;
#pragma unroll
        for (int i = 0; i < 4; ++i) {
          bool v = p0 + i < L;
          if (TAPS == 9) {
            const bool wrap = w0 + i >= W;
            const int h = h0 + (wrap ? 1 : 0) + dy, w = w0 + i - (wrap ? W : 0) + dx;
            v = v && h >= 0 && h < H && w >= 0 && w < W;
          }
          ok[i] = v;
        }
      }
#pragma unroll
      for (int k = 0; k < 4; ++k) {
        f32x4 fa = R.va[k], fb = R.vb[k];
        if (rs_on) rs[k] += (p0 < L) ? (fa[0] + fa[1]) + (fa[2] + fa[3]) : 0.0f;
#pragma unroll
        for (int i = 0; i < 4; ++i) fb[i] = ok[i] ? fb[i] : 0.0f;
        uint2 ahi, alo, bhi, blo;
#ifdef KGDET_NTP_ABL_NOSPLIT
        ahi = uint2{__float_as_uint(fa[0]), __float_as_uint(fa[1])}; alo = uint2{__float_as_uint(fa[2]), __float_as_uint(fa[3])};
        bhi = uint2{__float_as_uint(fb[0]), __float_as_uint(fb[1])}; blo = uint2{__float_as_uint(fb[2]), __float_as_uint(fb[3])};
#else
        split_pair(fa[0], fa[1], ahi.x, alo.x);
        split_pair(fa[2], fa[3], ahi.y, alo.y);
        split_pair(fb[0], fb[1], bhi.x, blo.x);
        split_pair(fb[2], fb[3], bhi.y, blo.y);
#endif
        *reinterpret_cast<uint2 *>(As + k * 32 * 16) = ahi;
        *reinterpret_cast<uint2 *>(As + kPPart + k * 32 * 16) = alo;
        *reinterpret_cast<uint2 *>(Bs + k * 32 * 16) = bhi;
        *reinterpret_cast<uint2 *>(Bs + kPPart + k * 32 * 16) = blo;
      }
    };
    if (n > 0) {
      Regs R0, R1;
      issue(R0);
      issue(R1);
      commit(0, R0);
      issue(R0);
      __syncthreads();
      for (int j = 0; j < n; j += 2) {
        if (j + 1 < n) commit(1, R1);
        issue(R1);
        __syncthreads();
        if (j + 1 < n) {
          if (j + 2 < n) commit(0, R0);
          issue(R0);
          __syncthreads();
        }
      }
    }
    if (rs_on) {
#pragma unroll
      for (int k = 0; k < 4; ++k) {
        float v = rs[k];
        v += __shfl_xor(v, 1);
        v += __shfl_xor(v, 2);
        v += __shfl_xor(v, 4);
        const int m = mt * kTM + rp + 32 * k;
        if (q == 0 && m < M) row_sums[(long long)m * rs_stride + split] = v;
      }
    }
  } else {
    const int wm = wave & 1, wn = wave >> 1;
    f32x16 acc[2][kPNI];
#pragma unroll
    for (int mi = 0; mi < 2; ++mi)
#pragma unroll
      for (int ni = 0; ni < kPNI; ++ni)
#pragma unroll
        for (int r = 0; r < 16; ++r) acc[mi][ni][r] = 0.0f;
    const int fo = (lane >> 5) * kPKH + (lane & 31) * 16;
    auto multiply = [&](int buf) __attribute__((always_inline)) {
      const unsigned char *A = smem + buf * kPStage + fo + wm * 64 * 16;
      const unsigned char *Bp = smem + buf * kPStage + kPOperand + fo + wn * (32 * kPNI) * 16;
      bf16x8 fa[2][2][2], fb[2][2][kPNI];
#pragma unroll
      for (int ks = 0; ks < 2; ++ks)
#pragma unroll
        for (int pt = 0; pt < 2; ++pt) {
#pragma unroll
          for (int i = 0; i < 2; ++i) fa[ks][pt][i] = *reinterpret_cast<const bf16x8 *>(A + ks * kPKS + pt * kPPart + i * 32 * 16);
#pragma unroll
          for (int i = 0; i < kPNI; ++i) fb[ks][pt][i] = *reinterpret_cast<const bf16x8 *>(Bp + ks * kPKS + pt * kPPart + i * 32 * 16);
        }
#pragma unroll
      for (int ks = 0; ks < 2; ++ks) {
#pragma unroll
        for (int mi = 0; mi < 2; ++mi)
#pragma unroll
          for (int ni = 0; ni < kPNI; ++ni)
            acc[mi][ni] = __builtin_amdgcn_mfma_f32_32x32x16_bf16(fa[ks][1][mi], fb[ks][0][ni], acc[mi][ni], 0, 0, 0);
#pragma unroll
        for (int mi = 0; mi < 2; ++mi)
#pragma unroll
          for (int ni = 0; ni < kPNI; ++ni)
            acc[mi][ni] = __builtin_amdgcn_mfma_f32_32x32x16_bf16(fa[ks][0][mi], fb[ks][1][ni], acc[mi][ni], 0, 0, 0);
#pragma unroll
        for (int mi = 0; mi < 2; ++mi)
#pragma unroll
          for (int ni = 0; ni < kPNI; ++ni)
            acc[mi][ni] = __builtin_amdgcn_mfma_f32_32x32x16_bf16(fa[ks][0][mi], fb[ks][0][ni], acc[mi][ni], 0, 0, 0);
      }
    };
    if (n > 0) {
      __syncthreads();
      for (int j = 0; j < n; j += 2) {
        multiply(0);
        __syncthreads();
        if (j + 1 < n) {
          multiply(1);
          __syncthreads();
        }
      }
    }
    float *out = partial + (long long)split * M * N;
#pragma unroll
    for (int mi = 0; mi < 2; ++mi)
#pragma unroll
      for (int ni = 0; ni < kPNI; ++ni) {
        const int nn = nt * kTN + wn * (32 * kPNI) + ni * 32 + (lane & 31);
#pragma unroll
        for (int r = 0; r < 16; ++r) {
          const int m = mt * kTM + wm * 64 + mi * 32 + (r & 3) + 8 * (r >> 2) + 4 * (lane >> 5);
          if (m < M && nn < N) out[(long long)m * N + nn] = acc[mi][ni][r];
        }
      }
  }
}

template <int TAPS, bool ALIGNED>
__global__ __launch_bounds__(kPThreads, 1) void conv_ntp(const float *__restrict__ a, const float *__restrict__ bm,
                                                         float *__restrict__ partial, int M, int N, int L, int B, int n_mt,
                                                         int n_nt, int stages_per_image, int per, int H, int W, int Cin,
                                                         int units, float *__restrict__ row_sums = nullptr, int rs_stride = 0) {
  extern __shared__ __attribute__((aligned(16))) unsigned char smem[];
  const int unit = units > 0 ? xcd_tile(blockIdx.x, units) : (int)blockIdx.x;
  if (units > 0 && unit >= units) return;
  if (threadIdx.x >= kPCons * 64)
    conv_ntp_role<TAPS, true, ALIGNED>(a, bm, partial, M, N, L, B, n_mt, n_nt, stages_per_image, per, H, W, Cin, unit, smem, row_sums, rs_stride);
  else
    conv_ntp_role<TAPS, false, ALIGNED>(a, bm, partial, M, N, L, B, n_mt, n_nt, stages_per_image, per, H, W, Cin, unit, smem, row_sums, rs_stride);
}

namespace {

int nt_splits(int tiles, int total_stages) {
  static const int round_up = [] { const char *e = getenv("KGDET_NT_SPLITS_UP"); return e ? atoi(e) : 0; }();
  const int most = (total_stages + 31) / 32;
  int splits = (256 + tiles - 1) / tiles;
  if (!round_up) {
    double best = 1e30;
    const int s_max = 2 * ((256 + tiles - 1) / tiles) < 128 ? 2 * ((256 + tiles - 1) / tiles) : 128;
    for (int s = 1; s <= s_max; ++s) {
      const double t = (double)((tiles * s + 255) / 256) / s;
      if (t < best) best = t;
    }
    splits = 0;
    for (int s = 1; s <= s_max && !splits; ++s)
      if ((double)((tiles * s + 255) / 256) / s <= best * (1.0 + 1e-9) && tiles * s >= 224 && tiles * s <= 256) splits = s;
    for (int s = s_max; s >= 1 && !splits; --s)
      if ((double)((tiles * s + 255) / 256) / s <= best * (1.0 + 1e-9)) splits = s;
  }
  if (splits > most) splits = most;
  if (splits > 128) splits = 128;
  return splits < 1 ? 1 : splits;
}

bool nt_xcd() {
  static const bool on = [] { const char *e = getenv("KGDET_NT_XCD"); return !e || atoi(e) != 0; }();
  return on;
}
int nt_units(int units) { return nt_xcd() ? units : 0; }
int nt_grid(int units) { return nt_xcd() ? (units + 7) / 8 * 8 : units; }

bool ntp_on(int taps, bool odd = false) {
  static const int mode = [] { const char *e = getenv("KGDET_NT_PC"); return e ? atoi(e) : 1; }();
  return mode == 2 || (mode == 1 && (taps == 9 || odd));
}
int ntp_lds() { return kPLds; }
int ntp_attr() {
  static thread_local bool set = false;
  if (!set) {
    KGDET_HIP_TRY(hipFuncSetAttribute((const void *)conv_ntp<1, false>, hipFuncAttributeMaxDynamicSharedMemorySize, ntp_lds()));
    KGDET_HIP_TRY(hipFuncSetAttribute((const void *)conv_ntp<1, true>, hipFuncAttributeMaxDynamicSharedMemorySize, ntp_lds()));
    KGDET_HIP_TRY(hipFuncSetAttribute((const void *)conv_ntp<9, false>, hipFuncAttributeMaxDynamicSharedMemorySize, ntp_lds()));
    KGDET_HIP_TRY(hipFuncSetAttribute((const void *)conv_ntp<9, true>, hipFuncAttributeMaxDynamicSharedMemorySize, ntp_lds()));
    set = true;
  }
  return KGDET_OK;
}

int nn_ksplit(long long tiles, int stages) {
  if (tiles >= 200) return 1;
  int k = (int)((384 + tiles - 1) / tiles);
  const int most = stages / 8;
  if (k > most) k = most;
  if (k > 8) k = 8;
  return k < 1 ? 1 : k;
}

struct NNPlan {
  bool patch;
  int TX, TY, NB, NW, tiles_x, n_nt, ks;
  long long tiles;
};
int conv_patch_mode() {
  static const int on = [] { const char *e = getenv("KGDET_CONV3X3_PATCH"); return e ? atoi(e) : 2; }();
  return on;
}
bool conv_patch_enabled() { return conv_patch_mode() != 0; }
NNPlan plan_nn(long long B, int M, int K, int H, int W, int taps, int stride) {
  NNPlan p;
  const int Ho = (H + stride - 1) / stride, Wo = (W + stride - 1) / stride;
  const int n_mt = (M + kTM - 1) / kTM;
  p.patch = false;
  p.TX = p.TY = p.tiles_x = 0;
  p.NB = p.NW = 4;
  p.n_nt = (int)(((long long)Ho * Wo + kTN - 1) / kTN);
  if (taps == 9 && stride == 1 && conv_patch_enabled()) {
    long long best = -1;
    p.NB = 4;
    for (int cap = 128; cap <= (conv_patch_mode() >= 2 && M > 64 ? 160 : 128); cap += 32)
      for (int tx = 8; tx <= 126 && tx <= (W + 7) / 8 * 8; ++tx) {
        const int ty = cap / tx;
        if (ty < 1 || (tx + 2) * (ty + 2) > kPatchMax) continue;
        const long long n = (long long)((H + ty - 1) / ty) * ((W + tx - 1) / tx);
        const long long units = n * n_mt * B;
        const long long rounds = units <= 256 ? 256 : units <= 512 ? 512 : units;
        const long long cost = (rounds * (cap / 32)) * 4096 + n * 8 + (cap == 160) * 4 + ((tx + 2) * (ty + 2) > 230);
        if (best < 0 || cost < best) { best = cost; p.TX = tx; p.TY = ty; p.NB = cap / 32; }
      }
    static const int force_tx = [] { const char *e = getenv("KGDET_CONV_TX"); return e ? atoi(e) : 0; }();
    if (force_tx > 0 && (force_tx + 2) * (128 / force_tx + 2) <= kPatchMax) { p.TX = force_tx; p.TY = 128 / force_tx; p.NB = 4; }
    if (best >= 0) {
      p.patch = true;
      p.tiles_x = (W + p.TX - 1) / p.TX;
      p.n_nt = p.tiles_x * ((H + p.TY - 1) / p.TY);
    }
  }
  if (!p.patch) {
    static const int force_nw = [] { const char *e = getenv("KGDET_CONV_NW"); return e ? atoi(e) : 0; }();
    const long long hw = (long long)Ho * Wo;
    const long long u4 = (long long)n_mt * ((hw + 127) / 128) * B, u5 = (long long)n_mt * ((hw + 159) / 160) * B;
    const long long c4 = ((u4 + 255) / 256) * 4, c5 = ((u5 + 255) / 256) * 5;
    if (force_nw == 5 || (force_nw == 0 && u4 >= 200 && u5 >= 200 && c5 * 10 <= c4 * 9)) {
      p.NW = 5;
      p.n_nt = (int)((hw + 159) / 160);
    }
  }
  p.tiles = (long long)n_mt * p.n_nt * B;
  p.ks = nn_ksplit(p.tiles, taps * ((K + kTK - 1) / kTK));
  if (p.patch && p.tiles < 200) {
    static const int old_rule = [] { const char *e = getenv("KGDET_CONV_KS_OLD"); return e ? atoi(e) : 0; }();
    const int chunks = K / kTK;
    double best = 1e30;
    p.ks = 1;
    for (int ks = 1; ks <= 8 && ks * 2 <= chunks; ++ks) {
      const double out_mb = (double)B * M * Ho * Wo * 4e-6;
      const double cost = (double)((p.tiles * ks + 255) / 256) * ((chunks + ks - 1) / ks) + 0.114 * out_mb * ks;
      if (cost < best) { best = cost; p.ks = ks; }
    }
    if (old_rule) p.ks = nn_ksplit(p.tiles, chunks * 2);
  }
  static const int force_ks = [] { const char *e = getenv("KGDET_CONV_KS"); return e ? atoi(e) : 0; }();
  if (force_ks > 0) p.ks = force_ks;
  return p;
}

}

}

using namespace kgdet;

#ifdef KGDET_CONV_TRACE
extern "C" int kgdet_debug_read_conv_trace(unsigned long long *out) {
  return (int)hipMemcpyFromSymbol(out, HIP_SYMBOL(kgdet::g_conv_trace), sizeof(unsigned long long) * 1024 * 8);
}
#endif

extern "C" size_t kgdet_conv_packed_bytes(int32_t M, int32_t K, int32_t taps) {
  if (M <= 0 || K <= 0 || (taps == 9 && K % kTK) || (taps != 1 && taps != 9)) return 0;
  return (size_t)((M + kTM - 1) / kTM) * ((K + kTK - 1) / kTK) * taps * kStage;
}

extern "C" int kgdet_conv_pack_fmt(const float *w, int32_t O, int32_t C, int32_t taps, int32_t transpose, void *packed,
                                   int32_t operand_format, void *stream) {
  const int M = transpose ? C : O, K = transpose ? O : C;
  KGDET_CHECK_SHAPE(taps == 1 || taps == 9, "taps must be 1 (1x1) or 9 (3x3)");
  KGDET_CHECK_SHAPE(O > 0 && C > 0 && (taps == 1 || K % kTK == 0), "reduction length %d is not a multiple of 16", K);
  KGDET_CHECK_SHAPE(w && packed, "null pointer");
  const long long total = (long long)((M + kTM - 1) / kTM) * ((K + kTK - 1) / kTK) * taps * 2 * kTM;
  const long long blocks = (total + 255) / 256;
  hipLaunchKernelGGL(conv1x1_pack, dim3((unsigned)(blocks > 65535 ? 65535 : blocks)), dim3(256), 0, (hipStream_t)stream, w,
                     O, C, taps, transpose, (unsigned char *)packed, (unsigned char *)nullptr, operand_format == 1 ? 1 : 0);
  KGDET_CHECK_LAUNCH("conv_pack");
  return KGDET_OK;
}

extern "C" int kgdet_conv_pack(const float *w, int32_t O, int32_t C, int32_t taps, int32_t transpose, void *packed,
                               void *stream) {
  return kgdet_conv_pack_fmt(w, O, C, taps, transpose, packed, 0, stream);
}

extern "C" int kgdet_conv_pack_both_fmt(const float *w, int32_t O, int32_t C, int32_t taps, void *packed, void *packed_t,
                                        int32_t forward_format, void *stream) {
  KGDET_CHECK_SHAPE(taps == 1 || taps == 9, "taps must be 1 (1x1) or 9 (3x3)");
  KGDET_CHECK_SHAPE(O > 0 && C > 0 && (taps == 1 || (O % kTK == 0 && C % kTK == 0)), "O and C must be multiples of 16");
  KGDET_CHECK_SHAPE(w && packed && packed_t, "null pointer");
  const long long t0 = (long long)((O + kTM - 1) / kTM) * ((C + kTK - 1) / kTK) * taps * 2 * kTM;
  const long long t1 = (long long)((C + kTM - 1) / kTM) * ((O + kTK - 1) / kTK) * taps * 2 * kTM;
  const long long blocks = ((t0 > t1 ? t0 : t1) + 255) / 256;
  hipLaunchKernelGGL(conv1x1_pack, dim3((unsigned)(blocks > 32768 ? 32768 : blocks), 2), dim3(256), 0,
                     (hipStream_t)stream, w, O, C, taps, 0, (unsigned char *)packed, (unsigned char *)packed_t,
                     forward_format == 1 ? 1 : 0);
  KGDET_CHECK_LAUNCH("conv_pack_both");
  return KGDET_OK;
}

extern "C" int kgdet_conv_pack_both(const float *w, int32_t O, int32_t C, int32_t taps, void *packed, void *packed_t,
                                    void *stream) {
  return kgdet_conv_pack_both_fmt(w, O, C, taps, packed, packed_t, 0, stream);
}

extern "C" int64_t kgdet_conv_pack_blocks(int32_t O, int32_t C, int32_t taps) {
  if (O <= 0 || C <= 0 || (taps == 9 && (O % kTK || C % kTK)) || (taps != 1 && taps != 9)) return 0;
  const long long t0 = (long long)((O + kTM - 1) / kTM) * ((C + kTK - 1) / kTK) * taps * 2 * kTM;
  const long long t1 = (long long)((C + kTM - 1) / kTM) * ((O + kTK - 1) / kTK) * taps * 2 * kTM;
  return ((t0 > t1 ? t0 : t1) + 255) / 256;
}

extern "C" int kgdet_conv_pack_multi(const int64_t *desc_dev, int32_t n, int64_t total_blocks, void *stream) {
  KGDET_CHECK_SHAPE(desc_dev && n > 0 && total_blocks > 0 && total_blocks < (1LL << 31), "bad descriptor table");
  hipLaunchKernelGGL(conv1x1_pack_multi, dim3((unsigned)total_blocks), dim3(256), 0, (hipStream_t)stream,
                     (const long long *)desc_dev, n);
  KGDET_CHECK_LAUNCH("conv_pack_multi");
  return KGDET_OK;
}

// ... 314 lines not shown
  return conv3x3_s2_col_bytes(B, C, H, W) + conv1x1_gw_workspace(B, O, 9 * C, HWo, nullptr);
}

extern "C" int kgdet_conv3x3_s2_grad_weight(const float *grad_y, const float *x, float *grad_w, int64_t B, int32_t O, int32_t C,
                                            int32_t H, int32_t W, void *workspace, size_t workspace_bytes, void *stream) {
  KGDET_CHECK_SHAPE(B > 0 && O > 0 && C > 0 && H > 0 && W > 0 && (long long)9 * C * ((H + 1) / 2) * ((W + 1) / 2) < (1LL << 30), "bad sizes");
  KGDET_CHECK_SHAPE(grad_y && x && grad_w && workspace, "null pointer");
  KGDET_CHECK_SHAPE(workspace_bytes >= kgdet_conv3x3_s2_grad_weight_workspace_bytes(B, O, C, H, W), "workspace too small");
  KGDET_CHECK_SHAPE(((long long)O * C) % 2 == 0, "O*C must be even");
  const int Ho = (H + 1) / 2, Wo = (W + 1) / 2;
  float *col = static_cast<float *>(workspace);
  const long long total = (long long)B * C * Ho * Wo;
  const long long blocks = (total + 255) / 256;
  hipLaunchKernelGGL(conv_s2_gather9, dim3((unsigned)(blocks > 16384 ? 16384 : blocks)), dim3(256), 0, (hipStream_t)stream, x, col, C,
                     H, W, Ho, Wo, (long long)B * C);
  KGDET_CHECK_LAUNCH("conv_s2_gather9");
  const size_t cb = conv3x3_s2_col_bytes(B, C, H, W);
  return conv1x1_grad_weight_impl(grad_y, col, grad_w, B, O, 9 * C, (long long)Ho * Wo, static_cast<unsigned char *>(workspace) + cb,
                                  workspace_bytes - cb, stream, nullptr, C);
}

extern "C" int kgdet_conv1x1_grad_weight(const float *grad_y, const float *x, float *grad_w, int64_t B, int32_t O,
                                         int32_t C, int64_t HW, void *workspace, size_t workspace_bytes,
                                         void *stream) {
  return conv1x1_grad_weight_impl(grad_y, x, grad_w, B, O, C, HW, workspace, workspace_bytes, stream, nullptr);
}

static int fold_args(ConvFoldArgs &f, const float *w, const float *s, const float *mean, const float *var, float eps,
                     const float *bn_partial, int32_t P, float *grad_beta, float *grad_gamma) {
  KGDET_CHECK_SHAPE(w && s && mean && var && ((bn_partial && P > 0) || (!bn_partial && P == 0)),
                    "null pointer (folded BatchNorm arguments; bn_partial == NULL goes with P == 0)");
  f.w = w; f.s = s; f.mean = mean; f.var = var; f.bn_partial = bn_partial; f.grad_beta = grad_beta; f.grad_gamma = grad_gamma;
  f.eps = eps; f.P = P;
  return KGDET_OK;
}

extern "C" int kgdet_conv1x1_grad_weight_fold(const float *grad_y, const float *x, float *grad_w, int64_t B, int32_t O,
                                              int32_t C, int64_t HW, void *workspace, size_t workspace_bytes, const float *w,
                                              const float *s, const float *mean, const float *var, float eps,
                                              const float *bn_partial, int32_t P, float *grad_beta, float *grad_gamma,
                                              void *stream) {
  ConvFoldArgs f;
  if (int rc = fold_args(f, w, s, mean, var, eps, bn_partial, P, grad_beta, grad_gamma)) return rc;
  return conv1x1_grad_weight_impl(grad_y, x, grad_w, B, O, C, HW, workspace, workspace_bytes, stream, &f);
}

static size_t conv3x3_gw_workspace(int64_t B, int32_t O, int32_t C, int32_t H, int32_t W, size_t *rows_at) {
  const int Wp = (W + 3) & ~3;
  const int tiles = ((O + kTM - 1) / kTM) * (9 * C / kTN);
  const int stages = (int)(B * (((long long)H * Wp + kTK - 1) / kTK));
  const int splits = nt_splits(tiles, stages);
  size_t bytes = (size_t)splits * O * C * 9 * sizeof(float);
  if (Wp != W) bytes = ((bytes + 255) & ~(size_t)255) + (size_t)B * (O + C) * H * Wp * sizeof(float);
  bytes = (bytes + 255) & ~(size_t)255;
  if (rows_at) *rows_at = bytes;
  return bytes + (size_t)splits * O * sizeof(float);
}

extern "C" size_t kgdet_conv3x3_grad_weight_workspace_bytes(int64_t B, int32_t O, int32_t C, int32_t H, int32_t W) {
  if (B <= 0 || O <= 0 || C <= 0 || H <= 0 || W <= 0) return 0;
  return conv3x3_gw_workspace(B, O, C, H, W, nullptr);
}

static int conv3x3_grad_weight_impl(const float *grad_y, const float *x, float *grad_w, int64_t B, int32_t O, int32_t C,
                                    int32_t H, int32_t W, void *workspace, size_t workspace_bytes, void *stream,
                                    const ConvFoldArgs *fold) {
  KGDET_CHECK_SHAPE(B > 0 && O > 0 && C > 0 && H > 0 && W > 0 && (long long)H * (W + 3) < (1LL << 23), "bad sizes");
  if (C % kTN != 0) {
    set_error("conv3x3_grad_weight needs C %% 128 == 0 (C=%d)", C);
    return KGDET_E_UNSUPPORTED;
  }
  KGDET_CHECK_SHAPE(grad_y && x && grad_w && workspace, "null pointer");
  KGDET_CHECK_SHAPE(workspace_bytes >= kgdet_conv3x3_grad_weight_workspace_bytes(B, O, C, H, W), "workspace too small");
  const int W_true = W;
  size_t rows_at = 0;
  conv3x3_gw_workspace(B, O, C, H, W, &rows_at);
  float *row_sums = (fold && !fold->bn_partial) ? reinterpret_cast<float *>(static_cast<unsigned char *>(workspace) + rows_at) : nullptr;
  const bool use_ntp = ntp_on(9) && W >= 4 && (long long)H * W >= 4 && (long long)H * W <= (1ll << 21) &&
                       (long long)(O > C ? O : C) * H * ((W + 3) & ~3) < (1ll << 30);
  if (W % 4 && use_ntp) {
    W = (W + 3) & ~3;
  } else if (W % 4) {
    const int Wp = (W + 3) & ~3;
    const int tiles_ = ((O + kTM - 1) / kTM) * (9 * C / kTN);
    const int stages_ = (int)(B * (((long long)H * Wp + kTK - 1) / kTK));
    const size_t part = ((size_t)nt_splits(tiles_, stages_) * O * C * 9 * sizeof(float) + 255) & ~(size_t)255;
    float *gyp = reinterpret_cast<float *>(static_cast<unsigned char *>(workspace) + part);
    float *xp = gyp + (size_t)B * O * H * Wp;
    const long long rows_a = (long long)B * O * H, rows_b = (long long)B * C * H;
    const long long most = (rows_a > rows_b ? rows_a : rows_b) * Wp;
    const long long blocks = (most + 255) / 256;
    hipLaunchKernelGGL(pad_rows2, dim3((unsigned)(blocks > 4096 ? 4096 : blocks), 2), dim3(256), 0, (hipStream_t)stream,
                       grad_y, gyp, rows_a, x, xp, rows_b, W, Wp);
    KGDET_CHECK_LAUNCH("pad_rows2");
    grad_y = gyp;
    x = xp;
    W = Wp;
  }
  const int HW = H * W;
  const int n_mt = (O + kTM - 1) / kTM, n_nt = 9 * C / kTN, tiles = n_mt * n_nt;
  const int spi = (HW + kTK - 1) / kTK, total = (int)(B * spi);
  const int splits = nt_splits(tiles, total);
  const int per = (total + splits - 1) / splits;
  if (use_ntp) {
    if (int rc = ntp_attr()) return rc;
    const int L = H * W_true;
    const int spi32 = (L + kPK - 1) / kPK, total32 = (int)(B * spi32), per32 = (total32 + splits - 1) / splits;
    if (W_true % 4 == 0)
      hipLaunchKernelGGL((conv_ntp<9, true>), dim3(nt_grid(tiles * splits)), dim3(kPThreads), ntp_lds(), (hipStream_t)stream, grad_y, x,
                         (float *)workspace, O, 9 * C, L, (int)B, n_mt, n_nt, spi32, per32, H, W_true, C, nt_units(tiles * splits),
                         row_sums, splits);
    else
      hipLaunchKernelGGL((conv_ntp<9, false>), dim3(nt_grid(tiles * splits)), dim3(kPThreads), ntp_lds(), (hipStream_t)stream, grad_y, x,
                         (float *)workspace, O, 9 * C, L, (int)B, n_mt, n_nt, spi32, per32, H, W_true, C, nt_units(tiles * splits),
                         row_sums, splits);
    KGDET_CHECK_LAUNCH("conv_ntp<9>");
  } else {
    hipLaunchKernelGGL(conv_nt8<9>, dim3(nt_grid(tiles * splits)), dim3(kNNThreads), 0, (hipStream_t)stream, grad_y, x,
                       (float *)workspace, O, 9 * C, HW, (int)B, n_mt, n_nt, spi, per, H, W, C, nt_units(tiles * splits), row_sums,
                       splits);
    KGDET_CHECK_LAUNCH("conv_nt8<9>");
  }
  const long long n = (long long)O * C * 9;
  if (fold) {
    ConvFoldArgs f = *fold;
    if (row_sums) { f.bn_partial = row_sums; f.P = splits; }
    hipLaunchKernelGGL(conv_wsum_fold<true>, dim3(O), dim3(fold_threads(9 * C)), (size_t)9 * C * sizeof(float),
                       (hipStream_t)stream, (const float *)workspace, grad_w, C, n, splits, f);
    KGDET_CHECK_LAUNCH("conv_wsum_fold");
    return KGDET_OK;
  }
  const long long blocks = (n + 255) / 256;
  hipLaunchKernelGGL(conv3x3_wsum, dim3((unsigned)(blocks > 4096 ? 4096 : blocks)), dim3(256), 0, (hipStream_t)stream,
                     (const float *)workspace, grad_w, O, C, splits);
  KGDET_CHECK_LAUNCH("conv3x3_wsum");
  return KGDET_OK;
}

extern "C" int kgdet_conv3x3_grad_weight(const float *grad_y, const float *x, float *grad_w, int64_t B, int32_t O,
                                         int32_t C, int32_t H, int32_t W, void *workspace, size_t workspace_bytes,
                                         void *stream) {
  return conv3x3_grad_weight_impl(grad_y, x, grad_w, B, O, C, H, W, workspace, workspace_bytes, stream, nullptr);
}

extern "C" int kgdet_conv3x3_grad_weight_fold(const float *grad_y, const float *x, float *grad_w, int64_t B, int32_t O,
                                              int32_t C, int32_t H, int32_t W, void *workspace, size_t workspace_bytes,
                                              const float *w, const float *s, const float *mean, const float *var, float eps,
                                              const float *bn_partial, int32_t P, float *grad_beta, float *grad_gamma,
                                              void *stream) {
  ConvFoldArgs f;
  if (int rc = fold_args(f, w, s, mean, var, eps, bn_partial, P, grad_beta, grad_gamma)) return rc;
  return conv3x3_grad_weight_impl(grad_y, x, grad_w, B, O, C, H, W, workspace, workspace_bytes, stream, &f);
}
```

kgdet_amd/heads.py:

```python
from __future__ import division

import ctypes
import os

import numpy as np
import torch
import torch.nn as nn

from . import conv1x1, dcn, moment
from .layers import ConvModule, bias_init_with_prob, normal_init
from .points import (PointGenerator, dense_targets_applicable, multi_apply, point_target_kp,
                     point_target_kp_dense)
from .postprocess import multiclass_nms_kp, multiclass_nms_kp_batched
from .registry import HEADS, build_loss

_KERNELS = (3, 5, 7)
_GROUP_POINTS = (9, 25, 49)


def _base_offset(k):
    pad = (k - 1) // 2
    base = np.arange(-pad, pad + 1).astype(np.float64)
    yx = np.stack([np.repeat(base, k), np.tile(base, k)], axis=1).reshape(-1)
    return torch.tensor(yx).view(1, -1, 1, 1)


_FUSED_OFFSETS = os.environ.get('KGDET_FUSED_OFFSETS', '1') == '1'


class _PtsFromOffsets(torch.autograd.Function):

    @staticmethod
    def forward(ctx, pred, centres, stride, y_first):
        from . import _lib
        pred = pred.contiguous()
        B, C, H, W = pred.shape
        pts = pred.new_empty(B, H * W, C)
        _lib.check(_lib.lib().kgdet_pts_from_offsets_forward(
            _lib.ptr(pred), _lib.ptr(centres.contiguous()), _lib.ptr(pts), ctypes.c_int64(B), ctypes.c_int32(C),
            ctypes.c_int64(H * W), ctypes.c_float(stride), ctypes.c_int32(1 if y_first else 0), _lib.current_stream()),
            'pts_from_offsets_forward')
        ctx.shape, ctx.stride, ctx.y_first = (B, C, H, W), stride, y_first
        return pts

    @staticmethod
    @torch.autograd.function.once_differentiable
    def backward(ctx, g):
        from . import _lib
        B, C, H, W = ctx.shape
        g = g.contiguous()
        grad = g.new_empty(B, C, H, W)
        _lib.check(_lib.lib().kgdet_pts_from_offsets_backward(
            _lib.ptr(g), _lib.ptr(grad), ctypes.c_int64(B), ctypes.c_int32(C), ctypes.c_int64(H * W),
            ctypes.c_float(ctx.stride), ctypes.c_int32(1 if ctx.y_first else 0), _lib.current_stream()),
            'pts_from_offsets_backward')
        return grad, None, None, None


class _RepOffsets(torch.autograd.Function):

    @staticmethod
    def forward(ctx, reppts, gm):
        from . import _lib
        reppts = reppts.contiguous()
        B, C, H, W = reppts.shape
        ks = (ctypes.c_int32 * 3)(*_KERNELS)
        outs = [reppts.new_empty(B, 2 * k * k, H, W) for k in _KERNELS]
        _lib.check(_lib.lib().kgdet_reppts_offsets_forward(
            _lib.ptr(reppts), ctypes.c_int32(B), ctypes.c_int32(C), ctypes.c_int32(H * W), ks, ctypes.c_float(gm),
            _lib.ptr(outs[0]), _lib.ptr(outs[1]), _lib.ptr(outs[2]), _lib.current_stream()), 'reppts_offsets_forward')
        ctx.gm, ctx.shape = gm, (B, C, H, W)
        return tuple(outs)

    @staticmethod
    @torch.autograd.function.once_differentiable
    def backward(ctx, g0, g1, g2):
        from . import _lib
        B, C, H, W = ctx.shape
        gs = [None if g is None else g.contiguous() for g in (g0, g1, g2)]
        like = next(g for g in gs if g is not None)
        grad = like.new_empty(B, C, H, W)
        ks = (ctypes.c_int32 * 3)(*_KERNELS)
        _lib.check(_lib.lib().kgdet_reppts_offsets_backward(
            _lib.ptr(gs[0]), _lib.ptr(gs[1]), _lib.ptr(gs[2]), ctypes.c_int32(B), ctypes.c_int32(C), ctypes.c_int32(H * W), ks,
            ctypes.c_float(ctx.gm), _lib.ptr(grad), _lib.current_stream()), 'reppts_offsets_backward')
        return grad, None


class Kp3RepBlock(nn.Module):

    def __init__(self, deform_conv, cls_out_channels, in_channels=256, feat_channels=256, num_reppts=9,
                 num_keypts=17, gradient_mul=0.1):
        super().__init__()
        self.deform_conv = deform_conv
        self.gradient_mul = gradient_mul
        keypts_out_dim = 2 * num_keypts
        reppts_out_dim = 2 * num_reppts
        self.relu = nn.ReLU(inplace=False)

        if deform_conv:
            for k in _KERNELS:
                setattr(self, 'dcn_kernel_%d' % k, k)
                setattr(self, 'dcn_pad_%d' % k, (k - 1) // 2)
                setattr(self, 'dcn_base_offset_%d' % k, _base_offset(k))
                setattr(self, 'cls_dfmconv_%d' % k, dcn.DeformConv(in_channels, feat_channels, k, 1, (k - 1) // 2))
            self.cls_out = nn.Conv2d(feat_channels * 3, cls_out_channels, 1, 1, 0)
            for k in _KERNELS:
                setattr(self, 'keypts_dfmconv_%d' % k,
                        dcn.DeformConv(in_channels, feat_channels, k, 1, (k - 1) // 2))
            self.keypts_out = nn.Conv2d(feat_channels * 3, keypts_out_dim, 1, 1, 0)
            self.reppts_out = nn.Conv2d(keypts_out_dim, reppts_out_dim, 1, 1, 0)
        else:
            self.cls_conv = nn.Conv2d(in_channels, feat_channels, 3, 1, 1)
            self.cls_out = nn.Conv2d(feat_channels, cls_out_channels, 1, 1, 0)
            self.keypts_conv = nn.Conv2d(in_channels, feat_channels, 3, 1, 1)
            self.keypts_out = nn.Conv2d(feat_channels, keypts_out_dim, 1, 1, 0)
            self.reppts_out = nn.Conv2d(keypts_out_dim, reppts_out_dim, 1, 1, 0)

        bias_cls = bias_init_with_prob(0.01)
        if self.deform_conv:
            for k in _KERNELS:
                normal_init(getattr(self, 'cls_dfmconv_%d' % k), std=0.01)
                normal_init(getattr(self, 'keypts_dfmconv_%d' % k), std=0.01)
        else:
            normal_init(self.cls_conv, std=0.01)
            normal_init(self.keypts_conv, std=0.01)
        normal_init(self.cls_out, std=0.01, bias=bias_cls)
        normal_init(self.keypts_out, std=0.01)
        normal_init(self.reppts_out, std=0.01)

    def _dcn_offsets(self, reppts_offset, like):
        if (_FUSED_OFFSETS and reppts_offset.is_cuda and reppts_offset.dtype == torch.float32
                and not torch.is_autocast_enabled()):
            return list(_RepOffsets.apply(reppts_offset, float(self.gradient_mul)))
        offsets, start = [], 0
        for k, n in zip(_KERNELS, _GROUP_POINTS):
            part = reppts_offset[:, 2 * start:2 * (start + n), :, :]
            start += n
            part = self.gradient_mul * part + (1 - self.gradient_mul) * part.detach()
            offsets.append(part - self._base_offset_on(k, like))
        return offsets

    def _base_offset_on(self, k, like):
        cache = self.__dict__.setdefault('_base_offset_cache', {})
        key = (k, like.device, like.dtype)
        if key not in cache:
            cache[key] = getattr(self, 'dcn_base_offset_%d' % k).to(device=like.device, dtype=like.dtype)
        return cache[key]

    def forward(self, cls_feat, pts_feat, reppts_offset=None):
        if self.deform_conv:
            offsets = self._dcn_offsets(reppts_offset, pts_feat)
            pads = [getattr(self, 'dcn_pad_%d' % k) for k in _KERNELS]
            cls_dfmconv_feat, keypts_dfmconv_feat = dcn.deform_conv_cat_multi(
                [cls_feat, pts_feat], offsets,
                [[getattr(self, 'cls_dfmconv_%d' % k).weight for k in _KERNELS],
                 [getattr(self, 'keypts_dfmconv_%d' % k).weight for k in _KERNELS]], pads)
            cls_out = conv1x1.conv_bias_act(self.cls_out, cls_dfmconv_feat)
            keypts_out = conv1x1.conv_bias_act(self.keypts_out, keypts_dfmconv_feat)
            reppts_out = conv1x1.conv_bias_act(self.reppts_out, keypts_out)
        else:
            cls_out = conv1x1.conv_bias_act(self.cls_out, conv1x1.conv_bias_act(self.cls_conv, cls_feat, relu=True))
            keypts_out = conv1x1.conv_bias_act(self.keypts_out, conv1x1.conv_bias_act(self.keypts_conv, pts_feat, relu=True))
            reppts_out = conv1x1.conv_bias_act(self.reppts_out, keypts_out)
        return cls_out, keypts_out, reppts_out


def _normalised_loss(loss_module, pred, target, weight, normalize_term, avg_factor):
    from .losses import SmoothL1Loss
    if type(loss_module) is SmoothL1Loss:
        return loss_module(pred, target, weight, avg_factor=avg_factor, divisor=normalize_term)
    return loss_module(pred / normalize_term, target / normalize_term, weight, avg_factor=avg_factor)


class PointHeadMixin(object):

    def points2bbox(self, pts, y_first=True):
        pts_reshape = pts.reshape(pts.shape[0], -1, 2, *pts.shape[2:])
        pts_y = pts_reshape[:, :, 0, ...] if y_first else pts_reshape[:, :, 1, ...]
        pts_x = pts_reshape[:, :, 1, ...] if y_first else pts_reshape[:, :, 0, ...]
        if self.transform_method == 'minmax':
            pass
        elif self.transform_method == 'partial_minmax':
            pts_y = pts_y[:, :4, ...]
            pts_x = pts_x[:, :4, ...]
        elif self.transform_method == 'moment':
            moment_transfer = (self.moment_transfer * self.moment_mul) + (
                self.moment_transfer.detach() * (1 - self.moment_mul))
            if pts.dim() == 2:
                return moment.moment_bbox(pts.reshape(pts.shape[0], -1, 1, 1), moment_transfer, y_first).reshape(-1, 4)
            return moment.moment_bbox(pts, moment_transfer, y_first)
        else:
            raise NotImplementedError
        return torch.cat([pts_x.min(dim=1, keepdim=True)[0], pts_y.min(dim=1, keepdim=True)[0],
                          pts_x.max(dim=1, keepdim=True)[0], pts_y.max(dim=1, keepdim=True)[0]], dim=1)

    def points2kpt(self, pts, y_first=True):
        pts_reshape = pts.reshape(pts.shape[0], -1, 2, *pts.shape[2:])
        pts_y = pts_reshape[:, :, 0, ...] if y_first else pts_reshape[:, :, 1, ...]
        pts_x = pts_reshape[:, :, 1, ...] if y_first else pts_reshape[:, :, 0, ...]
        return torch.stack([pts_x, pts_y], dim=2).reshape(*pts.shape)

    def get_points(self, featmap_sizes, img_metas, device='cuda'):
        num_imgs = len(img_metas)
        num_levels = len(featmap_sizes)
        multi_level_points = [
            self.point_generators[i].grid_points(featmap_sizes[i], self.point_strides[i], device=device)
            for i in range(num_levels)
        ]
        points_list = [[point.clone() for point in multi_level_points] for _ in range(num_imgs)]
        valid_flag_list = []
        for img_meta in img_metas:
            multi_level_flags = []
            for i in range(num_levels):
                point_stride = self.point_strides[i]
                feat_h, feat_w = featmap_sizes[i]
                h, w, _ = img_meta['pad_shape']
                valid_feat_h = min(int(np.ceil(h / point_stride)), feat_h)
                valid_feat_w = min(int(np.ceil(w / point_stride)), feat_w)
                multi_level_flags.append(self.point_generators[i].valid_flags(
                    (feat_h, feat_w), (valid_feat_h, valid_feat_w), device=device))
            valid_flag_list.append(multi_level_flags)
        return points_list, valid_flag_list

    def centers_to_bboxes(self, point_list):
        bbox_list = []
        for point in point_list:
            bbox = []
            for i_lvl in range(len(self.point_strides)):
                scale = self.point_base_scale * self.point_strides[i_lvl] * 0.5
                bbox_shift = torch.Tensor([-scale, -scale, scale, scale]).view(1, 4).type_as(point[0])
                bbox_center = torch.cat([point[i_lvl][:, :2], point[i_lvl][:, :2]], dim=1)
                bbox.append(bbox_center + bbox_shift)
            bbox_list.append(bbox)
        return bbox_list

    def offset_to_pts(self, center_list, pred_list, y_first=True):
        num_points = pred_list[0].size(1) // 2
        pts_list = []
        for i_lvl in range(len(self.point_strides)):
            pred = pred_list[i_lvl]
            B = pred.shape[0]
            if (_FUSED_OFFSETS and pred.is_cuda and pred.dtype == torch.float32 and not torch.is_autocast_enabled()
                    and pred.numel() > 0):
                centers = torch.stack([center_list[i_img][i_lvl][:, :2] for i_img in range(B)], 0)
                pts_list.append(_PtsFromOffsets.apply(pred, centers, float(self.point_strides[i_lvl]), bool(y_first)))
                continue
            shift = pred.permute(0, 2, 3, 1).reshape(B, -1, num_points, 2)
            if y_first:
                shift = shift.flip(-1)
            centers = torch.stack([center_list[i_img][i_lvl][:, :2] for i_img in range(B)], 0)
            pts = shift * self.point_strides[i_lvl] + centers.unsqueeze(2)
            pts_list.append(pts.reshape(B, -1, 2 * num_points))
        return pts_list


@HEADS.register_module
class RepPointsHeadKp3RepCas1AssignOnce(PointHeadMixin, nn.Module):

    def __init__(self,
                 num_classes,
                 in_channels,
                 feat_channels=256,
                 point_feat_channels=256,
                 stacked_convs=3,
                 num_reppts=9,
                 num_keypts=17,
                 gradient_mul=0.1,
                 point_strides=[8, 16, 32, 64, 128],
                 point_base_scale=4,
                 flip_forward=False,
                 conv_cfg=None,
                 norm_cfg=None,
                 loss_cls_1=dict(type='FocalLoss', use_sigmoid=True, gamma=2.0, alpha=0.25, loss_weight=0.5),
                 loss_cls_2=dict(type='FocalLoss', use_sigmoid=True, gamma=2.0, alpha=0.25, loss_weight=0.5),
                 loss_cls_3=dict(type='FocalLoss', use_sigmoid=True, gamma=2.0, alpha=0.25, loss_weight=1.0),
                 loss_bbox_1=dict(type='SmoothL1Loss', beta=1.0 / 9.0, loss_weight=0.5),
                 loss_bbox_2=dict(type='SmoothL1Loss', beta=1.0 / 9.0, loss_weight=0.5),
                 loss_bbox_3=dict(type='SmoothL1Loss', beta=1.0 / 9.0, loss_weight=1.0),
                 loss_kpt_1=dict(type='SmoothL1Loss', beta=1.0 / 9.0, loss_weight=0.5),
                 loss_kpt_2=dict(type='SmoothL1Loss', beta=1.0 / 9.0, loss_weight=0.5),
                 loss_kpt_3=dict(type='SmoothL1Loss', beta=1.0 / 9.0, loss_weight=1.0),
                 use_grid_points=False,
                 center_init=True,
                 transform_method='moment',
                 moment_mul=0.01):
        super().__init__()
        self.in_channels = in_channels
        self.num_classes = num_classes
        self.feat_channels = feat_channels
        self.point_feat_channels = point_feat_channels
        self.stacked_convs = stacked_convs
        self.num_keypts = num_keypts
        self.num_reppts = sum(_GROUP_POINTS)
        self.gradient_mul = gradient_mul
        self.point_base_scale = point_base_scale
        self.point_strides = point_strides
        self.flip_forward = flip_forward
        self.conv_cfg = conv_cfg
        self.norm_cfg = norm_cfg
        self.use_sigmoid_cls = loss_cls_3.get('use_sigmoid', False)
        self.sampling = loss_cls_3['type'] not in ['FocalLoss']
        for stage, cfgs in enumerate(((loss_cls_1, loss_bbox_1, loss_kpt_1), (loss_cls_2, loss_bbox_2, loss_kpt_2),
                                      (loss_cls_3, loss_bbox_3, loss_kpt_3)), 1):
            setattr(self, 'loss_cls_%d' % stage, build_loss(cfgs[0]))
            setattr(self, 'loss_bbox_%d' % stage, build_loss(cfgs[1]))
            setattr(self, 'loss_kpt_%d' % stage, build_loss(cfgs[2]))
        self.use_grid_points = use_grid_points
        self.center_init = center_init
        self.transform_method = transform_method
        if self.transform_method == 'moment':
            self.moment_transfer = nn.Parameter(data=torch.zeros(2), requires_grad=True)
            self.moment_mul = moment_mul
        self.cls_out_channels = self.num_classes - 1 if self.use_sigmoid_cls else self.num_classes
        self.point_generators = [PointGenerator() for _ in self.point_strides]
        self._init_layers()

    def _init_layers(self):
        self.relu = nn.ReLU(inplace=False)
        self.cls_convs = nn.ModuleList()
        self.reg_convs = nn.ModuleList()
        for i in range(self.stacked_convs):
            chn = self.in_channels if i == 0 else self.feat_channels
            self.cls_convs.append(ConvModule(chn, self.feat_channels, 3, stride=1, padding=1,
                                             conv_cfg=self.conv_cfg, norm_cfg=self.norm_cfg))
            self.reg_convs.append(ConvModule(chn, self.feat_channels, 3, stride=1, padding=1,
                                             conv_cfg=self.conv_cfg, norm_cfg=self.norm_cfg))
        for stage, deform in ((1, False), (2, True), (3, True)):
            setattr(self, 'kp_rep_block_%d' % stage,
                    Kp3RepBlock(deform, self.cls_out_channels, self.feat_channels, self.point_feat_channels,
                                self.num_reppts, self.num_keypts, self.gradient_mul))

    def init_weights(self):
        for m in self.cls_convs:
            normal_init(m.conv, std=0.01)
        for m in self.reg_convs:
            normal_init(m.conv, std=0.01)

    def forward_single(self, x):
        cls_feat = x
        pts_feat = x
        for cls_conv in self.cls_convs:
            cls_feat = cls_conv(cls_feat)
        for reg_conv in self.reg_convs:
            pts_feat = reg_conv(pts_feat)

        cls_out_1, keypts_out_1, reppts_out_1 = self.kp_rep_block_1(cls_feat, pts_feat)
        bbox_out_1 = self.points2bbox(reppts_out_1)

        cls_out_2, keypts_out_2, reppts_out_2 = self.kp_rep_block_2(cls_feat, pts_feat, reppts_out_1)
        keypts_out_2 = keypts_out_2 + keypts_out_1.detach()
        reppts_out_2 = reppts_out_2 + reppts_out_1.detach()
        bbox_out_2 = self.points2bbox(reppts_out_2)

        cls_out_3, keypts_out_3, reppts_out_3 = self.kp_rep_block_3(cls_feat, pts_feat, reppts_out_2)
        keypts_out_3 = keypts_out_3 + keypts_out_2.detach()
        reppts_out_3 = reppts_out_3 + reppts_out_2.detach()
        bbox_out_3 = self.points2bbox(reppts_out_3)
        return (cls_out_1, cls_out_2, cls_out_3, keypts_out_1, keypts_out_2, keypts_out_3, bbox_out_1,
                bbox_out_2, bbox_out_3)

    def forward_single_flip(self, feat, img_metas):
        output = self.forward_single(feat)
        output_flip = self.forward_single(torch.flip(feat, [3]))
        num_stage = len(output) // 3
        flip_indices = img_metas[0]['flip_indices']
        fused = []
        for i in range(len(output)):
            back = torch.flip(output_flip[i], [3])
            kind = i // num_stage
            if kind == 1:
                back[:, 1::2, :, :] = -back[:, 1::2, :, :]
                back = back[:, flip_indices, :, :]
            elif kind == 2:
                back[:, 0::2, :, :] = -back[:, 0::2, :, :]
                back = back[:, [2, 1, 0, 3], :, :]
            fused.append((output[i] + back) / 2)
        return tuple(fused)

    def forward(self, feats, img_metas):
        if self.flip_forward:
            return multi_apply(self.forward_single_flip, feats, img_metas=img_metas)
        return multi_apply(self.forward_single, feats)

    def loss_single(self, cls_score_1, cls_score_2, cls_score_3, kpt_pred_1, kpt_pred_2, kpt_pred_3, bbox_pred_1,
                    bbox_pred_2, bbox_pred_3, labels, label_weights, bbox_gt, bbox_weights, kpt_gt, kpt_weights,
                    stride, num_total_samples):
        labels = labels.reshape(-1)
        label_weights = label_weights.reshape(-1)
        normalize_term = self.point_base_scale * stride
        bbox_gt = bbox_gt.reshape(-1, 4)
        bbox_weights = bbox_weights.reshape(-1, 4)
        kpt_gt = kpt_gt.reshape(-1, self.num_keypts * 2)
        kpt_weights = kpt_weights.reshape(-1, self.num_keypts * 2)
        kpt_pos_num = kpt_weights.sum(1)
        kpt_weights = kpt_weights / kpt_pos_num.clamp(min=1).unsqueeze(1) * 4

        losses = []
        for stage, cls_score in enumerate((cls_score_1, cls_score_2, cls_score_3), 1):
            cls_score = cls_score.permute(0, 2, 3, 1).reshape(-1, self.cls_out_channels)
            losses.append(getattr(self, 'loss_cls_%d' % stage)(cls_score, labels, label_weights,
                                                               avg_factor=num_total_samples))
        for stage, bbox_pred in enumerate((bbox_pred_1, bbox_pred_2, bbox_pred_3), 1):
            losses.append(_normalised_loss(getattr(self, 'loss_bbox_%d' % stage), bbox_pred.reshape(-1, 4), bbox_gt,
                                           bbox_weights, normalize_term, num_total_samples))
        for stage, kpt_pred in enumerate((kpt_pred_1, kpt_pred_2, kpt_pred_3), 1):
            losses.append(_normalised_loss(getattr(self, 'loss_kpt_%d' % stage), kpt_pred.reshape(-1, self.num_keypts * 2),
                                           kpt_gt, kpt_weights, normalize_term, num_total_samples))
        return tuple(losses)

    def loss(self, cls_scores_1, cls_scores_2, cls_scores_3, keypts_preds_1, keypts_preds_2, keypts_preds_3,
             bbox_preds_1, bbox_preds_2, bbox_preds_3, gt_bboxes, gt_labels, gt_keypoints, img_metas, cfg,
             gt_bboxes_ignore=None):
        featmap_sizes = [featmap.size()[-2:] for featmap in cls_scores_3]
        assert len(featmap_sizes) == len(self.point_generators)
        label_channels = self.cls_out_channels if self.use_sigmoid_cls else 1
        device = cls_scores_3[0].device

        if cfg.uniform.assigner['type'] != 'PointAssigner':
            raise NotImplementedError
        valid_sizes = [[(min(int(np.ceil(meta['pad_shape'][0] / s)), fs[0]), min(int(np.ceil(meta['pad_shape'][1] / s)), fs[1]))
                        for s, fs in zip(self.point_strides, featmap_sizes)] for meta in img_metas]
        all_valid = all(v == tuple(fs) for per_img in valid_sizes for v, fs in zip(per_img, featmap_sizes))
        from . import head_loss
        stages = ((cls_scores_1, cls_scores_2, cls_scores_3), (keypts_preds_1, keypts_preds_2, keypts_preds_3),
                  (bbox_preds_1, bbox_preds_2, bbox_preds_3))
        level0 = None if all_valid else [per_img[0] for per_img in valid_sizes]
        if head_loss.applicable(self, cfg.uniform, stages[0], stages[1], stages[2], gt_bboxes, gt_labels, gt_keypoints,
                                gt_bboxes_ignore, valid_sizes=level0):
            return head_loss.head_loss(self, cfg.uniform, stages[0], stages[1], stages[2], gt_bboxes, gt_labels,
                                       gt_keypoints, valid_sizes=level0)

        center_list, valid_flag_list = self.get_points(featmap_sizes, img_metas, device=device)
        kpt_coords = [self.offset_to_pts(center_list, p) for p in (keypts_preds_1, keypts_preds_2, keypts_preds_3)]
        bbox_coords = [self.offset_to_pts(center_list, p, y_first=False)
                       for p in (bbox_preds_1, bbox_preds_2, bbox_preds_3)]
        candidate_list = center_list
        if not self.sampling and dense_targets_applicable(cfg.uniform, len(self.point_strides), all_valid,
                                                          gt_bboxes_ignore):
            cls_reg_targets = point_target_kp_dense(candidate_list, gt_bboxes, gt_keypoints, cfg.uniform,
                                                    gt_labels_list=gt_labels,
                                                    valid_flag_list=None if all_valid else valid_flag_list)
        else:
            cls_reg_targets = point_target_kp(candidate_list, valid_flag_list, gt_bboxes, gt_keypoints, img_metas,
                                              cfg.uniform, gt_bboxes_ignore_list=gt_bboxes_ignore,
                                              gt_labels_list=gt_labels, label_channels=label_channels,
                                              sampling=self.sampling)
        (labels_list, label_weights_list, bbox_gt_list, candidate_list, bbox_weights_list, keypoint_gt_list,
         keypoint_weights_list, num_total_pos, num_total_neg) = cls_reg_targets
        num_total_samples = (num_total_pos + num_total_neg if self.sampling else num_total_pos)

        per_level = multi_apply(self.loss_single, cls_scores_1, cls_scores_2, cls_scores_3, kpt_coords[0],
                                kpt_coords[1], kpt_coords[2], bbox_coords[0], bbox_coords[1], bbox_coords[2],
                                labels_list, label_weights_list, bbox_gt_list, bbox_weights_list, keypoint_gt_list,
                                keypoint_weights_list, self.point_strides, num_total_samples=num_total_samples)
        names = ['loss_cls_1', 'loss_cls_2', 'loss_cls_3', 'loss_bbox_1', 'loss_bbox_2', 'loss_bbox_3',
                 'loss_kpt_1', 'loss_kpt_2', 'loss_kpt_3']
        return dict(zip(names, per_level))

    def _decode_level(self, cls_score, bbox_pred, kpt_pred, points, stride, img_shape, cfg):
        num_kpt = self.num_keypts
        num_kp_channel = kpt_pred.size(0) // num_kpt
        assert num_kp_channel == 2 or num_kp_channel == 3
        assert cls_score.size()[-2:] == bbox_pred.size()[-2:] == kpt_pred.size()[-2:]
        cls_score = cls_score.permute(1, 2, 0).reshape(-1, self.cls_out_channels)
        scores = cls_score.sigmoid() if self.use_sigmoid_cls else cls_score.softmax(-1)
        bbox_pred = bbox_pred.permute(1, 2, 0).reshape(-1, 4)
        if num_kp_channel == 3:
            kpt_pred = kpt_pred.permute(1, 2, 0).reshape(-1, num_kpt * num_kp_channel)
        else:
            kpt_pred = kpt_pred.permute(1, 2, 0).reshape(-1, num_kpt, num_kp_channel)
            kpt_pred = torch.cat([kpt_pred, kpt_pred.new_full(kpt_pred[:, :, :1].size(), 1)], dim=2)
            kpt_pred = kpt_pred.reshape(-1, num_kpt * 3)
        nms_pre = cfg.get('nms_pre', -1)
        if nms_pre > 0 and scores.shape[0] > nms_pre:
            max_scores, _ = scores.max(dim=1) if self.use_sigmoid_cls else scores[:, 1:].max(dim=1)
            _, topk_inds = max_scores.topk(nms_pre)
            points = points[topk_inds, :]
            bbox_pred = bbox_pred[topk_inds, :]
            kpt_pred = kpt_pred[topk_inds, :]
            scores = scores[topk_inds, :]
        bbox_pos_center = torch.cat([points[:, :2], points[:, :2]], dim=1)
        bboxes = bbox_pred * stride + bbox_pos_center
        kpts = kpt_pred.view(-1, num_kpt, 3).clone()
        kpts[:, :, :2] = kpts[:, :, :2] * stride + points[:, :2].unsqueeze(dim=1)
        bboxes = torch.stack([bboxes[:, 0].clamp(min=0, max=img_shape[1]), bboxes[:, 1].clamp(min=0, max=img_shape[0]),
                              bboxes[:, 2].clamp(min=0, max=img_shape[1]), bboxes[:, 3].clamp(min=0, max=img_shape[0])],
                             dim=-1)
        kpts[:, :, 0] = kpts[:, :, 0].clamp(min=0, max=img_shape[1])
        kpts[:, :, 1] = kpts[:, :, 1].clamp(min=0, max=img_shape[0])
        return bboxes, scores, kpts

    def get_bboxes_single(self, cls_scores, bbox_preds, kpt_preds, mlvl_points, img_shape, scale_factor, cfg,
                          rescale=False, nms=True):
        assert len(cls_scores) == len(bbox_preds) == len(mlvl_points) == len(kpt_preds)
        decoded = [self._decode_level(c, b, k, p, self.point_strides[i], img_shape, cfg)
                   for i, (c, b, k, p) in enumerate(zip(cls_scores, bbox_preds, kpt_preds, mlvl_points))]
        mlvl_bboxes = torch.cat([d[0] for d in decoded])
# ... 156 lines not shown
```

kgdet_amd/layers.py:

```python
import ctypes
import os as _os
import warnings

import numpy as np
import torch
import torch.nn as nn

from . import conv1x1

_NORMS = {'BN': ('bn', nn.BatchNorm2d), 'SyncBN': ('bn', nn.SyncBatchNorm), 'GN': ('gn', nn.GroupNorm)}
_CONVS = {'Conv': nn.Conv2d}


def build_norm_layer(cfg, num_features, postfix=''):
    assert isinstance(cfg, dict) and 'type' in cfg
    cfg_ = dict(cfg)
    layer_type = cfg_.pop('type')
    if layer_type not in _NORMS:
        raise KeyError('Unrecognized norm type {}'.format(layer_type))
    abbr, norm_layer = _NORMS[layer_type]
    assert isinstance(postfix, (int, str))
    name = abbr + str(postfix)
    requires_grad = cfg_.pop('requires_grad', True)
    cfg_.setdefault('eps', 1e-5)
    if layer_type != 'GN':
        layer = norm_layer(num_features, **cfg_)
    else:
        assert 'num_groups' in cfg_
        layer = norm_layer(num_channels=num_features, **cfg_)
    for param in layer.parameters():
        param.requires_grad = requires_grad
    return name, layer


def build_conv_layer(cfg, *args, **kwargs):
    if cfg is None:
        cfg_ = dict(type='Conv')
    else:
        assert isinstance(cfg, dict) and 'type' in cfg
        cfg_ = dict(cfg)
    layer_type = cfg_.pop('type')
    if layer_type not in _CONVS:
        raise KeyError('Unrecognized norm type {}'.format(layer_type))
    return _CONVS[layer_type](*args, **kwargs, **cfg_)


def constant_init(module, val, bias=0):
    nn.init.constant_(module.weight, val)
    if hasattr(module, 'bias') and module.bias is not None:
        nn.init.constant_(module.bias, bias)


def xavier_init(module, gain=1, bias=0, distribution='normal'):
    assert distribution in ['uniform', 'normal']
    if distribution == 'uniform':
        nn.init.xavier_uniform_(module.weight, gain=gain)
    else:
        nn.init.xavier_normal_(module.weight, gain=gain)
    if hasattr(module, 'bias') and module.bias is not None:
        nn.init.constant_(module.bias, bias)


def normal_init(module, mean=0, std=1, bias=0):
    nn.init.normal_(module.weight, mean, std)
    if hasattr(module, 'bias') and module.bias is not None:
        nn.init.constant_(module.bias, bias)


def kaiming_init(module, mode='fan_out', nonlinearity='relu', bias=0, distribution='normal'):
    assert distribution in ['uniform', 'normal']
    if distribution == 'uniform':
        nn.init.kaiming_uniform_(module.weight, mode=mode, nonlinearity=nonlinearity)
    else:
        nn.init.kaiming_normal_(module.weight, mode=mode, nonlinearity=nonlinearity)
    if hasattr(module, 'bias') and module.bias is not None:
        nn.init.constant_(module.bias, bias)


def bias_init_with_prob(prior_prob):
    return float(-np.log((1 - prior_prob) / prior_prob))


FUSED_GN = _os.environ.get('KGDET_FUSED_GN', '1') == '1'
GN_SPLIT = _os.environ.get('KGDET_GN_SPLIT', '1') == '1'


def gn_act_applicable(x, norm):
    return (FUSED_GN and type(norm) is nn.GroupNorm and x.is_cuda and x.dtype == torch.float32 and x.dim() == 4
            and x.is_contiguous() and x.numel() > 0 and not torch.is_autocast_enabled()
            and norm.num_channels // norm.num_groups <= 64
            and (norm.num_channels // norm.num_groups) * x.shape[2] * x.shape[3] < (2 ** 31 if GN_SPLIT else 65537))


def _gn_scratch(x, N, C, groups, HW):
    from . import _lib
    L = _lib.lib()
    L.kgdet_gn_act_scratch_floats.restype = ctypes.c_size_t
    n = L.kgdet_gn_act_scratch_floats(ctypes.c_int64(N), ctypes.c_int32(C), ctypes.c_int32(groups), ctypes.c_int64(HW))
    return torch.empty(n, dtype=torch.float32, device=x.device) if n else None


def gn_act_bf16_applicable(x, norm):
    return (FUSED_GN and type(norm) is nn.GroupNorm and x.is_cuda and x.dtype == torch.bfloat16 and x.dim() == 4
            and (x.is_contiguous() or x.is_contiguous(memory_format=torch.channels_last))
            and x.numel() > 0 and not torch.is_grad_enabled()
            and norm.num_channels // norm.num_groups <= 64
            and (norm.num_channels // norm.num_groups) * x.shape[2] * x.shape[3] < (2 ** 31 if GN_SPLIT else 65537))


def gn_act_bf16(x, norm, relu):
    from . import _lib
    N, C = x.shape[0], x.shape[1]
    y = torch.empty_like(x)
    if (C // norm.num_groups) * x.shape[2] * x.shape[3] > 65536:
        scratch = _gn_scratch(x, N, C, norm.num_groups, x.shape[2] * x.shape[3])
        _lib.check(_lib.lib().kgdet_gn_act_forward_bf16_split(
            _lib.ptr(x), ctypes.c_int32(0 if x.is_contiguous() else 1), _lib.ptr(norm.weight), _lib.ptr(norm.bias),
            ctypes.c_int32(norm.num_groups), ctypes.c_float(norm.eps), ctypes.c_int32(1 if relu else 0), _lib.ptr(y),
            _lib.ptr(scratch), ctypes.c_int64(N), ctypes.c_int32(C), ctypes.c_int64(x.shape[2] * x.shape[3]),
            _lib.current_stream()), 'gn_act_forward_bf16_split')
        return y
    _lib.check(_lib.lib().kgdet_gn_act_forward_bf16(
        _lib.ptr(x), ctypes.c_int32(0 if x.is_contiguous() else 1), _lib.ptr(norm.weight), _lib.ptr(norm.bias), ctypes.c_int32(norm.num_groups), ctypes.c_float(norm.eps),
        ctypes.c_int32(1 if relu else 0), _lib.ptr(y), ctypes.c_int64(N), ctypes.c_int32(C),
        ctypes.c_int64(x.shape[2] * x.shape[3]), _lib.current_stream()), 'gn_act_forward_bf16')
    return y


class _GNAct(torch.autograd.Function):

    @staticmethod
    def forward(ctx, x, gamma, beta, groups, eps, relu):
        from . import _lib
        N, C = x.shape[0], x.shape[1]
        HW = x.shape[2] * x.shape[3]
        y = torch.empty_like(x)
        stats = torch.empty((2, N * groups), dtype=torch.float32, device=x.device)
        scratch = _gn_scratch(x, N, C, groups, HW)
        _lib.check(_lib.lib().kgdet_gn_act_forward_split(
            _lib.ptr(x), _lib.ptr(gamma), _lib.ptr(beta), ctypes.c_int32(groups), ctypes.c_float(eps),
            ctypes.c_int32(1 if relu else 0), _lib.ptr(y), ctypes.c_void_p(stats[0].data_ptr()),
            ctypes.c_void_p(stats[1].data_ptr()), _lib.ptr(scratch), ctypes.c_int64(N), ctypes.c_int32(C), ctypes.c_int64(HW),
            _lib.current_stream()), 'gn_act_forward')
        ctx.save_for_backward(x, y if relu else None, gamma, stats)
        ctx.groups, ctx.relu, ctx.has_beta = groups, relu, beta is not None
        return y

    @staticmethod
    def backward(ctx, gy):
        from . import _lib
        x, y, gamma, stats = ctx.saved_tensors
        N, C = x.shape[0], x.shape[1]
        HW = x.shape[2] * x.shape[3]
        gy = gy.contiguous()
        gx = torch.empty_like(x) if ctx.needs_input_grad[0] else None
        dgb = torch.empty((2, N, C), dtype=torch.float32, device=x.device)
        scratch = _gn_scratch(x, N, C, ctx.groups, HW)
        _lib.check(_lib.lib().kgdet_gn_act_backward_split(
            _lib.ptr(gy), _lib.ptr(x), _lib.ptr(y), _lib.ptr(gamma), ctypes.c_void_p(stats[0].data_ptr()),
            ctypes.c_void_p(stats[1].data_ptr()), ctypes.c_int32(ctx.groups), ctypes.c_int32(1 if ctx.relu else 0),
            _lib.ptr(gx), _lib.ptr(dgb), _lib.ptr(scratch), ctypes.c_int64(N), ctypes.c_int32(C), ctypes.c_int64(HW),
            _lib.current_stream()), 'gn_act_backward')
        sums = dgb.sum(1) if N > 1 else dgb[:, 0]
        ggamma = sums[0] if (gamma is not None and ctx.needs_input_grad[1]) else None
        gbeta = sums[1] if (ctx.has_beta and ctx.needs_input_grad[2]) else None
        return gx, ggamma, gbeta, None, None, None


def gn_act(x, norm, relu):
    return _GNAct.apply(x, norm.weight, norm.bias, norm.num_groups, norm.eps, relu)


class ConvModule(nn.Module):

    def __init__(self, in_channels, out_channels, kernel_size, stride=1, padding=0, dilation=1, groups=1,
                 bias='auto', conv_cfg=None, norm_cfg=None, activation='relu', inplace=True,
                 order=('conv', 'norm', 'act')):
        super(ConvModule, self).__init__()
        assert conv_cfg is None or isinstance(conv_cfg, dict)
        assert norm_cfg is None or isinstance(norm_cfg, dict)
        self.conv_cfg = conv_cfg
        self.norm_cfg = norm_cfg
        self.activation = activation
        self.inplace = inplace
        self.order = order
        assert isinstance(self.order, tuple) and len(self.order) == 3
        assert set(order) == set(['conv', 'norm', 'act'])

        self.with_norm = norm_cfg is not None
        self.with_activatation = activation is not None
        if bias == 'auto':
            bias = False if self.with_norm else True
        self.with_bias = bias
        if self.with_norm and self.with_bias:
            warnings.warn('ConvModule has norm and bias at the same time')

        self.conv = build_conv_layer(conv_cfg, in_channels, out_channels, kernel_size, stride=stride,
                                     padding=padding, dilation=dilation, groups=groups, bias=bias)
        for attr in ('in_channels', 'out_channels', 'kernel_size', 'stride', 'padding', 'dilation',
                     'transposed', 'output_padding', 'groups'):
            setattr(self, attr, getattr(self.conv, attr))

        if self.with_norm:
            norm_channels = out_channels if order.index('norm') > order.index('conv') else in_channels
            self.norm_name, norm = build_norm_layer(norm_cfg, norm_channels)
            self.add_module(self.norm_name, norm)

        if self.with_activatation:
            if self.activation not in ['relu']:
                raise ValueError('{} is currently not supported.'.format(self.activation))
            self.activate = nn.ReLU(inplace=inplace)

        self.init_weights()

    @property
    def norm(self):
        return getattr(self, self.norm_name)

    def init_weights(self):
        nonlinearity = 'relu' if self.activation is None else self.activation
        kaiming_init(self.conv, nonlinearity=nonlinearity)
        if self.with_norm:
            constant_init(self.norm, 1, bias=0)

    def forward(self, x, activate=True, norm=True):
        fused_act = False
        for li, layer in enumerate(self.order):
            if layer == 'conv':
                conv = self.conv
                if (type(conv) is nn.Conv2d and conv.bias is None and torch.is_grad_enabled()
                        and conv1x1.applicable(x, conv.weight, conv.stride, conv.padding, conv.dilation, conv.groups)):
                    x = conv1x1.conv_split(x, conv.weight)
                elif (type(conv) is nn.Conv2d and conv.bias is None and torch.is_grad_enabled()
                        and conv1x1.odd_map_applicable(x, conv.weight, conv.stride, conv.padding, conv.dilation, conv.groups)):
                    x = conv1x1.unpad_odd(conv1x1.conv_split(conv1x1.pad_odd(x), conv.weight), x.shape[3])
                elif (type(conv) is nn.Conv2d and torch.is_grad_enabled()
                        and conv1x1.applicable_stride2(x, conv.weight, conv.stride, conv.padding, conv.dilation, conv.groups)):
                    x = conv1x1.conv3x3_stride2(x, conv.weight)
                    if conv.bias is not None:
                        x = x + conv.bias.view(1, -1, 1, 1)
                elif type(conv) is nn.Conv2d and conv.bias is not None and torch.is_grad_enabled():
                    x = conv1x1.conv_bias_act(conv, x, relu=False)
                else:
                    x = conv1x1.conv_infer(conv, x)
            elif layer == 'norm' and norm and self.with_norm:
                relu_next = (activate and self.with_activatation and li + 1 < len(self.order)
                             and self.order[li + 1] == 'act')
                if gn_act_applicable(x, self.norm):
                    x = gn_act(x, self.norm, relu_next)
                    fused_act = relu_next
                elif gn_act_bf16_applicable(x, self.norm):
                    x = gn_act_bf16(x, self.norm, relu_next)
                    fused_act = relu_next
                else:
                    x = self.norm(x)
            elif layer == 'act' and activate and self.with_activatation:
                if not fused_act:
                    x = self.activate(x)
        return x



class _SharedLevels(torch.autograd.Function):

    @staticmethod
    def forward(ctx, run, n_levels, *flat):
        xs, params = flat[:n_levels], flat[n_levels:]
        ctx.levels, ctx.n_params = [], len(params)
        outs_flat = []
        for l, x in enumerate(xs):
            with torch.enable_grad():
                xin = x.detach().requires_grad_(x.requires_grad)
                proxies = [p.detach().requires_grad_(p.requires_grad) for p in params]
                outs = tuple(run(l, xin, proxies))
            ctx.levels.append((xin, proxies, outs))
            outs_flat.extend(o.detach() for o in outs)
        ctx.n_out = len(outs_flat) // max(n_levels, 1)
        return tuple(outs_flat)

    @staticmethod
    @torch.autograd.function.once_differentiable
    def backward(ctx, *gouts):
        gxs, acc = [], [None] * ctx.n_params
        for l, (xin, proxies, outs) in enumerate(ctx.levels):
            gl = gouts[l * ctx.n_out:(l + 1) * ctx.n_out]
            sel = [(o, g) for o, g in zip(outs, gl) if g is not None and o.requires_grad]
            inputs = ([xin] if xin.requires_grad else []) + [p for p in proxies if p.requires_grad]
            if not sel or not inputs:
                gxs.append(None)
                continue
            grads = torch.autograd.grad([o for o, _ in sel], inputs, [g for _, g in sel], allow_unused=True)
            grads = list(grads)
            gxs.append(grads.pop(0) if xin.requires_grad else None)
            it = iter(grads)
            mine, theirs = [], []
            for i, p in enumerate(proxies):
                if not p.requires_grad:
                    continue
                g = next(it)
                if g is None:
                    continue
                if acc[i] is None:
                    acc[i] = g if g.is_contiguous() else g.contiguous()
                else:
                    mine.append(acc[i])
                    theirs.append(g)
            if mine:
                torch._foreach_add_(mine, theirs)
        ctx.levels = None
        return (None, None) + tuple(gxs) + tuple(acc)


def shared_levels(module, single, xs):
    from torch.nn.utils import stateless
    names, params = zip(*[(n, p) for n, p in module.named_parameters()])

# ... 9 lines not shown
```

Measured before the change: 184.3 img/s.

## Fuse cls and reg head tower 3x3 convs into grouped multi-conv launches

Adds a grouped 3x3 conv kernel that handles up to eight convolutions in one launch by refactoring the patch4 conv body into a device function. Adds a grouped 3x3 weight-gradient kernel. A custom autograd function runs the cls and reg towers of the head together, layer by layer. In backward it sums the two branches' input gradients inside the kernel (sum_all) and computes all tower weight gradients in one call. This is meant to cut launch count and fill the GPU better on the small FPN levels, at the cost of extra workspace and more complex code.

```diff
diff --git a/include/kgdet_hip.h b/include/kgdet_hip.h
--- a/include/kgdet_hip.h
+++ b/include/kgdet_hip.h
@@ -50,6 +50,18 @@
 size_t kgdet_conv3x3_grad_weight_workspace_bytes(int64_t B, int32_t O, int32_t C, int32_t H, int32_t W);
 int kgdet_conv3x3_grad_weight(const float *grad_y, const float *x, float *grad_w, int64_t B, int32_t O, int32_t C,
                               int32_t H, int32_t W, void *workspace, size_t workspace_bytes, void *stream);
+int kgdet_conv3x3_group_ksplit(int32_t n, int64_t B, int32_t M, int32_t K, int32_t H, int32_t W);
+size_t kgdet_conv3x3_group_workspace_bytes(int32_t n, int64_t B, int32_t M, int32_t K, int32_t H, int32_t W, int32_t ksplit,
+                                           int32_t sum_all);
+int kgdet_conv3x3_group_apply(int32_t n, const void *const *packed, const float *const *x, float *const *y, int32_t sum_all,
+                              int64_t B, int32_t M, int32_t K, int32_t H, int32_t W, int32_t operand_format, int32_t ksplit,
+                              void *workspace, size_t workspace_bytes, void *stream);
+int kgdet_conv3x3_grad_weight_group_splits(int32_t n, int64_t B, int32_t O, int32_t C, int32_t H, int32_t W);
+size_t kgdet_conv3x3_grad_weight_group_workspace_bytes(int32_t n, int64_t B, int32_t O, int32_t C, int32_t H, int32_t W,
+                                                       int32_t splits);
+int kgdet_conv3x3_grad_weight_group(int32_t n, const float *const *grad_y, const float *const *x, float *const *grad_w,
+                                    int64_t B, int32_t O, int32_t C, int32_t H, int32_t W, int32_t splits, void *workspace,
+                                    size_t workspace_bytes, void *stream);
 
 int kgdet_bn_act_forward(const float *x, const float *gamma, const float *beta, const float *mean, const float *var,
                          float eps, const float *residual, float *y, int64_t N, int32_t C, int64_t HW, int32_t relu,
diff --git a/kgdet_amd/conv1x1.py b/kgdet_amd/conv1x1.py
--- a/kgdet_amd/conv1x1.py
+++ b/kgdet_amd/conv1x1.py
@@ -61,7 +61,15 @@
                  [vp, vp, vp, i64, i32, i32, i64, vp, sz, vp, vp, vp, vp, ctypes.c_float, vp, i32, vp, vp, vp]),
                 ('kgdet_conv3x3_grad_weight_fold', ctypes.c_int,
                  [vp, vp, vp, i64, i32, i32, i32, i32, vp, sz, vp, vp, vp, vp, ctypes.c_float, vp, i32, vp, vp, vp]),
-                ('kgdet_conv3x3_grad_weight', ctypes.c_int, [vp, vp, vp, i64, i32, i32, i32, i32, vp, sz, vp])):
+                ('kgdet_conv3x3_grad_weight', ctypes.c_int, [vp, vp, vp, i64, i32, i32, i32, i32, vp, sz, vp]),
+                ('kgdet_conv3x3_group_ksplit', ctypes.c_int, [i32, i64, i32, i32, i32, i32]),
+                ('kgdet_conv3x3_group_workspace_bytes', sz, [i32, i64, i32, i32, i32, i32, i32, i32]),
+                ('kgdet_conv3x3_group_apply', ctypes.c_int,
+                 [i32, vp, vp, vp, i32, i64, i32, i32, i32, i32, i32, i32, vp, sz, vp]),
+                ('kgdet_conv3x3_grad_weight_group_splits', ctypes.c_int, [i32, i64, i32, i32, i32, i32]),
+                ('kgdet_conv3x3_grad_weight_group_workspace_bytes', sz, [i32, i64, i32, i32, i32, i32, i32]),
+                ('kgdet_conv3x3_grad_weight_group', ctypes.c_int,
+                 [i32, vp, vp, vp, i64, i32, i32, i32, i32, i32, vp, sz, vp])):
             fn = getattr(L, name)
             fn.restype, fn.argtypes = res, args
         _L = L
@@ -257,8 +265,9 @@
     _aliases[key] = (weakref.ref(proxy, lambda _r, key=key: _aliases.pop(key, None)), weakref.ref(param))
 
 
-def forward_images(x, weight):
-    both = PACK_BOTH and x.requires_grad and (weight.shape[0] % 16 == 0 or weight.shape[2] == 1)
+def forward_images(x, weight, grad_input=None):
+    need_t = x.requires_grad if grad_input is None else grad_input
+    both = PACK_BOTH and need_t and (weight.shape[0] % 16 == 0 or weight.shape[2] == 1)
     a = _aliases.get(id(weight))
     if a is not None and a[0]() is weight:
         origin = a[1]()
@@ -356,6 +365,61 @@
 def grad_input(weight, img_t, gy, residual=None, gate=None):
     C, k = weight.shape[1], weight.shape[2]
     return _apply(img_t if img_t is not None else _pack(weight, True), gy, C, k * k, residual=residual, gate=gate)
+
+
+GROUP_MAX = 8
+
+
+def _ptrs(ts):
+    return (ctypes.c_void_p * len(ts))(*[t.data_ptr() for t in ts])
+
+
+def group_ksplit(n, x, M):
+    B, K, H, W = x.shape
+    return _lib_sizes().kgdet_conv3x3_group_ksplit(n, B, M, K, H, W)
+
+
+def group_applicable(x, weight):
+    return (applicable(x, weight, padding=(1, 1)) and weight.shape[2] == 3 and weight.shape[0] % 16 == 0
+            and weight.shape[1] % 128 == 0 and x.shape[3] >= 4 and group_ksplit(1, x, weight.shape[0]) >= 1
+            and grad_weight_group_splits(1, x, weight.shape[0]) >= 1)
+
+
+def apply_group(imgs, xs, M, sum_all=False, ksplit=0):
+    n = len(imgs)
+    assert 1 <= n <= GROUP_MAX and len(xs) == n
+    B, K, H, W = xs[0].shape
+    assert all(x.shape == xs[0].shape and x.is_contiguous() and x.dtype == torch.float32 for x in xs)
+    f16 = getattr(imgs[0], 'kgdet_f16', False)
+    assert all(getattr(i, 'kgdet_f16', False) == f16 for i in imgs), 'one operand format per group'
+    ys = [torch.empty((B, M, H, W), dtype=torch.float32, device=xs[0].device) for _ in range(1 if sum_all else n)]
+    nbytes = _size('kgdet_conv3x3_group_workspace_bytes', n, B, M, K, H, W, ksplit, 1 if sum_all else 0)
+    ws = torch.empty(nbytes, dtype=torch.uint8, device=xs[0].device) if nbytes else None
+    _lib.check(_lib_sizes().kgdet_conv3x3_group_apply(
+        n, _ptrs(imgs), _ptrs(xs), _ptrs(ys), 1 if sum_all else 0, B, M, K, H, W, 1 if f16 else 0, ksplit,
+        ws.data_ptr() if nbytes else None, nbytes, _stream()), 'conv3x3_group_apply')
+    return ys[0] if sum_all else ys
+
+
+def grad_weight_group_splits(n, x, O):
+    B, C, H, W = x.shape
+    return _lib_sizes().kgdet_conv3x3_grad_weight_group_splits(n, B, O, C, H, W)
+
+
+def grad_weight_group(xs, gys, splits=0):
+    n = len(xs)
+    assert 1 <= n <= GROUP_MAX and len(gys) == n
+    B, C, H, W = xs[0].shape
+    O = gys[0].shape[1]
+    assert all(x.shape == xs[0].shape and x.is_contiguous() for x in xs)
+    assert all(g.shape == gys[0].shape and g.is_contiguous() for g in gys)
+    gws = [torch.empty((O, C, 3, 3), dtype=torch.float32, device=xs[0].device) for _ in range(n)]
+    nbytes = _size('kgdet_conv3x3_grad_weight_group_workspace_bytes', n, B, O, C, H, W, splits)
+    ws = torch.empty(nbytes, dtype=torch.uint8, device=xs[0].device)
+    _lib.check(_lib_sizes().kgdet_conv3x3_grad_weight_group(
+        n, _ptrs(gys), _ptrs(xs), _ptrs(gws), B, O, C, H, W, splits, ws.data_ptr(), nbytes, _stream()),
+        'conv3x3_grad_weight_group')
+    return gws
 
 
 class _ConvSplit(torch.autograd.Function):
diff --git a/kgdet_amd/csrc/conv1x1.hip b/kgdet_amd/csrc/conv1x1.hip
--- a/kgdet_amd/csrc/conv1x1.hip
+++ b/kgdet_amd/csrc/conv1x1.hip
@@ -453,6 +453,7 @@
 #define CV_ADD(cat) do { } while (0)
 #endif
 constexpr int kPatchMax = 256;
+constexpr int kConvGroupMax = 8;
 constexpr int kPatchPart = 2 * kPatchMax * 16;
 constexpr int kPatchBuf = 2 * kPatchPart;
 constexpr int kPatchLds = 6 * kStage + 2 * kPatchBuf;
@@ -655,6 +656,159 @@
     }
 }
 
+template <int WAVES, int NB, bool F16>
+__device__ __forceinline__ void conv3x3_patch4_unit(unsigned char *smem, const unsigned char *__restrict__ img,
+                                                    const float *__restrict__ x, float *__restrict__ y, int M, int K, int H,
+                                                    int W, int n_mt, int tiles_x, int n_nt, int ksplit,
+                                                    long long part_stride, int TX, int TY, const float *__restrict__ bias,
+                                                    const float *__restrict__ residual, int relu,
+                                                    const float *__restrict__ gate, int unit0) {
+  constexpr int HALVES = 4 / WAVES, THREADS = 64 * WAVES, PXT = kPatchMax / THREADS;
+  const int half = unit0 % HALVES, unit = unit0 / HALVES;
+  const int part = unit % ksplit, tile = unit / ksplit;
+  const int tid = threadIdx.x, lane = tid & 63, wave = (tid >> 6) + half * WAVES;
+  const int N = H * W;
+  const int chunks_all = K / kTK, per = (chunks_all + ksplit - 1) / ksplit;
+  const int c_begin = part * per, c_end = max(c_begin, min(chunks_all, c_begin + per));
+  const int chunks = c_end - c_begin, stages = chunks * 9;
+  const int mt = tile % n_mt, nt = (tile / n_mt) % n_nt, b = tile / (n_mt * n_nt);
+  const int y0 = (nt / tiles_x) * TY, x0 = (nt % tiles_x) * TX;
+  const int PW = TX + 2, PP = PW * (TY + 2);
+
+  if (mt * kTM + half * 64 >= M) return;
+  bool p_live[PXT];
+  int p_off[PXT];
+#pragma unroll
+  for (int i = 0; i < PXT; ++i) {
+    const int pp = tid + i * THREADS;
+    const int ppy = pp / PW, ppx = pp - ppy * PW;
+    const int iy = y0 - 1 + ppy, ix = x0 - 1 + ppx;
+    p_live[i] = pp < PP && iy >= 0 && iy < H && ix >= 0 && ix < W;
+    p_off[i] = p_live[i] ? iy * W + ix : 0;
+  }
+  const float *xb = x + (long long)b * K * N;
+  unsigned char *b_dst = smem + tid * 16;
+
+  int b_rd[NB], o_n[NB];
+  bool o_live[NB];
+#pragma unroll
+  for (int nb = 0; nb < NB; ++nb) {
+    const int qq = nb * 32 + (lane & 31), q = min(qq, TX * TY - 1);
+    const int py = q / TX, px = q - py * TX;
+    b_rd[nb] = ((lane >> 5) * kPatchMax + py * PW + px) * 16;
+    o_live[nb] = qq < TX * TY && y0 + py < H && x0 + px < W;
+    o_n[nb] = o_live[nb] ? (y0 + py) * W + x0 + px : 0;
+  }
+  const int row_pitch = PW * 16;
+  const unsigned char *ag = img + ((long long)mt * chunks_all + min(c_begin, chunks_all - 1)) * 9 * kStage +
+                            (lane >> 5) * (kTM * 16) + (wave * 32 + (lane & 31)) * 16;
+
+  f32x16 acc[NB];
+#pragma unroll
+  for (int i = 0; i < NB; ++i)
+#pragma unroll
+    for (int r = 0; r < 16; ++r) acc[i][r] = 0.0f;
+
+  float bv[PXT][16];
+  auto issue_b = [&](int ci) {
+    const float *xp = xb + (long long)min(c_begin + min(ci, chunks - 1), chunks_all - 1) * kTK * N;
+#pragma unroll
+    for (int i = 0; i < PXT; ++i)
+#pragma unroll
+      for (int j = 0; j < 16; ++j) bv[i][j] = xp[(long long)j * N + p_off[i]];
+  };
+  auto commit_b = [&](int buf) {
+#pragma unroll
+    for (int i = 0; i < PXT; ++i)
+#pragma unroll
+      for (int j = 0; j < 16; ++j) asm volatile("" : "+v"(bv[i][j]));
+#pragma unroll
+    for (int i = 0; i < PXT; ++i)
+#pragma unroll
+      for (int kh = 0; kh < 2; ++kh) {
+        float v[8];
+#pragma unroll
+        for (int j = 0; j < 8; ++j) v[j] = p_live[i] ? bv[i][kh * 8 + j] : 0.0f;
+        bf16x8 hi, lo;
+        split8_t<F16>(v, hi, lo);
+        unsigned char *d = b_dst + i * THREADS * 16 + buf * kPatchBuf + kh * (kPatchMax * 16);
+        *reinterpret_cast<bf16x8 *>(d) = hi;
+        *reinterpret_cast<bf16x8 *>(d + kPatchPart) = lo;
+      }
+  };
+  bf16x8 AR[3][2];
+  auto issue_a = [&](int s, bf16x8 (&r)[2]) {
+    const unsigned char *p = ag + (long long)max(min(s, stages - 1), 0) * kStage;
+    r[0] = *reinterpret_cast<const bf16x8 *>(p);
+    r[1] = *reinterpret_cast<const bf16x8 *>(p + kPart);
+  };
+
+  issue_b(0);
+#pragma unroll
+  for (int j = 0; j < 3; ++j) issue_a(j, AR[j]);
+  commit_b(0);
+  for (int ci = 0; ci < chunks; ++ci) {
+    issue_b(ci + 1);
+    __syncthreads();
+    const unsigned char *bbuf = smem + (ci & 1) * kPatchBuf;
+#pragma unroll
+    for (int t = 0; t < 9; ++t) {
+      const int s = ci * 9 + t;
+      const unsigned char *bt = bbuf + (t / 3) * row_pitch + (t % 3) * 16;
+      bf16x8 bf[NB][2];
+#pragma unroll
+      for (int nb = 0; nb < NB; ++nb) {
+        bf[nb][0] = *reinterpret_cast<const bf16x8 *>(bt + b_rd[nb]);
+        bf[nb][1] = *reinterpret_cast<const bf16x8 *>(bt + b_rd[nb] + kPatchPart);
+      }
+#pragma unroll
+      for (int nb = 0; nb < NB; ++nb) acc[nb] = mfma_t<F16>(AR[t % 3][1], bf[nb][0], acc[nb]);
+#pragma unroll
+      for (int nb = 0; nb < NB; ++nb) acc[nb] = mfma_t<F16>(AR[t % 3][0], bf[nb][1], acc[nb]);
+#pragma unroll
+      for (int nb = 0; nb < NB; ++nb) acc[nb] = mfma_t<F16>(AR[t % 3][0], bf[nb][0], acc[nb]);
+      __builtin_amdgcn_sched_barrier(0);
+      issue_a(s + 3, AR[t % 3]);
+      if (t == 6) commit_b((ci + 1) & 1);
+      __builtin_amdgcn_sched_barrier(0);
+    }
+  }
+
+  float *yb = y + (long long)part * part_stride + (long long)b * M * N;
+  const int m0 = mt * kTM + wave * 32 + 4 * (lane >> 5);
+#pragma unroll
+  for (int nb = 0; nb < NB; ++nb) {
+    if constexpr (F16) {
+#pragma unroll
+      for (int r = 0; r < 16; ++r) acc[nb][r] *= 1.0f / kF16WeightScale;
+    }
+    if (bias || residual) {
+      float add[16];
+#pragma unroll
+      for (int r = 0; r < 16; ++r) {
+        const int m = min(m0 + (r & 3) + 8 * (r >> 2), M - 1);
+        float v = bias ? bias[m] : 0.0f;
+        if (residual) v += residual[((long long)b * M + m) * N + o_n[nb]];
+        add[r] = v;
+      }
+#pragma unroll
+      for (int r = 0; r < 16; ++r) acc[nb][r] += add[r];
+    }
+    if (gate) {
+      float gv[16];
+#pragma unroll
+      for (int r = 0; r < 16; ++r) gv[r] = gate[((long long)b * M + min(m0 + (r & 3) + 8 * (r >> 2), M - 1)) * N + o_n[nb]];
+#pragma unroll
+      for (int r = 0; r < 16; ++r) acc[nb][r] = gv[r] > 0.0f ? acc[nb][r] : 0.0f;
+    }
+#pragma unroll
+    for (int r = 0; r < 16; ++r) {
+      const int m = m0 + (r & 3) + 8 * (r >> 2);
+      if (m < M && o_live[nb]) yb[(long long)m * N + o_n[nb]] = relu ? fmaxf(acc[nb][r], 0.0f) : acc[nb][r];
+    }
+  }
+}
+
 template <int WAVES, int NB, bool F16 = false>
 __global__ __launch_bounds__(64 * WAVES) void conv3x3_patch4(const unsigned char *__restrict__ img,
                                                              const float *__restrict__ x, float *__restrict__ y, int M,
@@ -665,152 +819,32 @@
     const float *__restrict__ gate = nullptr) {
   __shared__ __attribute__((aligned(16))) unsigned char smem[2 * kPatchBuf];
   if constexpr (F16) f16_saturate_on();
-  constexpr int HALVES = 4 / WAVES, THREADS = 64 * WAVES, PXT = kPatchMax / THREADS;
+  constexpr int HALVES = 4 / WAVES;
   const int unit0 = xcd_tile(blockIdx.x, tiles * ksplit * HALVES);
   if (unit0 >= tiles * ksplit * HALVES) return;
-  const int half = unit0 % HALVES, unit = unit0 / HALVES;
-  const int part = unit % ksplit, tile = unit / ksplit;
-  const int tid = threadIdx.x, lane = tid & 63, wave = (tid >> 6) + half * WAVES;
-  const int N = H * W;
-  const int chunks_all = K / kTK, per = (chunks_all + ksplit - 1) / ksplit;
-  const int c_begin = part * per, c_end = max(c_begin, min(chunks_all, c_begin + per));
-  const int chunks = c_end - c_begin, stages = chunks * 9;
-  const int mt = tile % n_mt, nt = (tile / n_mt) % n_nt, b = tile / (n_mt * n_nt);
-  const int y0 = (nt / tiles_x) * TY, x0 = (nt % tiles_x) * TX;
-  const int PW = TX + 2, PP = PW * (TY + 2);
-
-  if (mt * kTM + half * 64 >= M) return;
-  bool p_live[PXT];
-  int p_off[PXT];
-#pragma unroll
-  for (int i = 0; i < PXT; ++i) {
-    const int pp = tid + i * THREADS;
-    const int ppy = pp / PW, ppx = pp - ppy * PW;
-    const int iy = y0 - 1 + ppy, ix = x0 - 1 + ppx;
-    p_live[i] = pp < PP && iy >= 0 && iy < H && ix >= 0 && ix < W;
-    p_off[i] = p_live[i] ? iy * W + ix : 0;
-  }
-  const float *xb = x + (long long)b * K * N;
-  unsigned char *b_dst = smem + tid * 16;
-
-  int b_rd[NB], o_n[NB];
-  bool o_live[NB];
-#pragma unroll
-  for (int nb = 0; nb < NB; ++nb) {
-    const int qq = nb * 32 + (lane & 31), q = min(qq, TX * TY - 1);
-    const int py = q / TX, px = q - py * TX;
-    b_rd[nb] = ((lane >> 5) * kPatchMax + py * PW + px) * 16;
-    o_live[nb] = qq < TX * TY && y0 + py < H && x0 + px < W;
-    o_n[nb] = o_live[nb] ? (y0 + py) * W + x0 + px : 0;
-  }
-  const int row_pitch = PW * 16;
-  const unsigned char *ag = img + ((long long)mt * chunks_all + min(c_begin, chunks_all - 1)) * 9 * kStage +
-                            (lane >> 5) * (kTM * 16) + (wave * 32 + (lane & 31)) * 16;
-
-  f32x16 acc[NB];
-#pragma unroll
-  for (int i = 0; i < NB; ++i)
-#pragma unroll
-    for (int r = 0; r < 16; ++r) acc[i][r] = 0.0f;
-
-  float bv[PXT][16];
-  auto issue_b = [&](int ci) {
-    const float *xp = xb + (long long)min(c_begin + min(ci, chunks - 1), chunks_all - 1) * kTK * N;
-#pragma unroll
-    for (int i = 0; i < PXT; ++i)
-#pragma unroll
-      for (int j = 0; j < 16; ++j) bv[i][j] = xp[(long long)j * N + p_off[i]];
-  };
-  auto commit_b = [&](int buf) {
-#pragma unroll
-    for (int i = 0; i < PXT; ++i)
-#pragma unroll
-      for (int j = 0; j < 16; ++j) asm volatile("" : "+v"(bv[i][j]));
-#pragma unroll
-    for (int i = 0; i < PXT; ++i)
-#pragma unroll
-      for (int kh = 0; kh < 2; ++kh) {
-        float v[8];
-#pragma unroll
-        for (int j = 0; j < 8; ++j) v[j] = p_live[i] ? bv[i][kh * 8 + j] : 0.0f;
-        bf16x8 hi, lo;
-        split8_t<F16>(v, hi, lo);
-        unsigned char *d = b_dst + i * THREADS * 16 + buf * kPatchBuf + kh * (kPatchMax * 16);
-        *reinterpret_cast<bf16x8 *>(d) = hi;
-        *reinterpret_cast<bf16x8 *>(d + kPatchPart) = lo;
-      }
-  };
-  bf16x8 AR[3][2];
-  auto issue_a = [&](int s, bf16x8 (&r)[2]) {
-    const unsigned char *p = ag + (long long)max(min(s, stages - 1), 0) * kStage;
-    r[0] = *reinterpret_cast<const bf16x8 *>(p);
-    r[1] = *reinterpret_cast<const bf16x8 *>(p + kPart);
-  };
-
-  issue_b(0);
-#pragma unroll
-  for (int j = 0; j < 3; ++j) issue_a(j, AR[j]);
-  commit_b(0);
-  for (int ci = 0; ci < chunks; ++ci) {
-    issue_b(ci + 1);
-    __syncthreads();
-    const unsigned char *bbuf = smem + (ci & 1) * kPatchBuf;
-#pragma unroll
-    for (int t = 0; t < 9; ++t) {
-      const int s = ci * 9 + t;
-      const unsigned char *bt = bbuf + (t / 3) * row_pitch + (t % 3) * 16;
-      bf16x8 bf[NB][2];
-#pragma unroll
-      for (int nb = 0; nb < NB; ++nb) {
-        bf[nb][0] = *reinterpret_cast<const bf16x8 *>(bt + b_rd[nb]);
-        bf[nb][1] = *reinterpret_cast<const bf16x8 *>(bt + b_rd[nb] + kPatchPart);
-      }
-#pragma unroll
-      for (int nb = 0; nb < NB; ++nb) acc[nb] = mfma_t<F16>(AR[t % 3][1], bf[nb][0], acc[nb]);
-#pragma unroll
-      for (int nb = 0; nb < NB; ++nb) acc[nb] = mfma_t<F16>(AR[t % 3][0], bf[nb][1], acc[nb]);
-#pragma unroll
-      for (int nb = 0; nb < NB; ++nb) acc[nb] = mfma_t<F16>(AR[t % 3][0], bf[nb][0], acc[nb]);
-      __builtin_amdgcn_sched_barrier(0);
-      issue_a(s + 3, AR[t % 3]);
-      if (t == 6) commit_b((ci + 1) & 1);
-      __builtin_amdgcn_sched_barrier(0);
-    }
-  }
-
-  float *yb = y + (long long)part * part_stride + (long long)b * M * N;
-  const int m0 = mt * kTM + wave * 32 + 4 * (lane >> 5);
-#pragma unroll
-  for (int nb = 0; nb < NB; ++nb) {
-    if constexpr (F16) {
-#pragma unroll
-      for (int r = 0; r < 16; ++r) acc[nb][r] *= 1.0f / kF16WeightScale;
-    }
-    if (bias || residual) {
-      float add[16];
-#pragma unroll
-      for (int r = 0; r < 16; ++r) {
-        const int m = min(m0 + (r & 3) + 8 * (r >> 2), M - 1);
-        float v = bias ? bias[m] : 0.0f;
-        if (residual) v += residual[((long long)b * M + m) * N + o_n[nb]];
-        add[r] = v;
-      }
-#pragma unroll
-      for (int r = 0; r < 16; ++r) acc[nb][r] += add[r];
-    }
-    if (gate) {
-      float gv[16];
-#pragma unroll
-      for (int r = 0; r < 16; ++r) gv[r] = gate[((long long)b * M + min(m0 + (r & 3) + 8 * (r >> 2), M - 1)) * N + o_n[nb]];
-#pragma unroll
-      for (int r = 0; r < 16; ++r) acc[nb][r] = gv[r] > 0.0f ? acc[nb][r] : 0.0f;
-    }
-#pragma unroll
-    for (int r = 0; r < 16; ++r) {
-      const int m = m0 + (r & 3) + 8 * (r >> 2);
-      if (m < M && o_live[nb]) yb[(long long)m * N + o_n[nb]] = relu ? fmaxf(acc[nb][r], 0.0f) : acc[nb][r];
-    }
-  }
+  conv3x3_patch4_unit<WAVES, NB, F16>(smem, img, x, y, M, K, H, W, n_mt, tiles_x, n_nt, ksplit, part_stride, TX, TY, bias,
+                                      residual, relu, gate, unit0);
+}
+
+struct ConvPatchGroup {
+  const unsigned char *img[kConvGroupMax];
+  const float *x[kConvGroupMax];
+  float *y[kConvGroupMax];
+  int n;
+};
+template <int WAVES, int NB, bool F16>
+__global__ __launch_bounds__(64 * WAVES) void conv3x3_patch4_group(ConvPatchGroup g, int M, int K, int H, int W, int n_mt,
+                                                                   int tiles_x, int n_nt, int tiles, int ksplit,
+                                                                   long long part_stride, int TX, int TY) {
+  __shared__ __attribute__((aligned(16))) unsigned char smem[2 * kPatchBuf];
+  if constexpr (F16) f16_saturate_on();
+  constexpr int HALVES = 4 / WAVES;
+  const int per = tiles * ksplit * HALVES;
+  const int unit = xcd_tile(blockIdx.x, per * g.n);
+  if (unit >= per * g.n) return;
+  const int p = unit / per;
+  conv3x3_patch4_unit<WAVES, NB, F16>(smem, g.img[p], g.x[p], g.y[p], M, K, H, W, n_mt, tiles_x, n_nt, ksplit, part_stride,
+                                      TX, TY, nullptr, nullptr, 0, nullptr, unit - p * per);
 }
 
 __global__ __launch_bounds__(256) void conv3x3_s2_grad_input(const unsigned char *__restrict__ img_t,
@@ -1005,9 +1039,7 @@
   }
 }
 
-__global__ __launch_bounds__(256) void conv1x1_sum(const float *__restrict__ parts, float *__restrict__ out,
-                                                   long long n, long long stride, int count) {
-  for (long long i = (blockIdx.x * 256LL + threadIdx.x) * 2; i < n; i += gridDim.x * 512LL) {
+__device__ __forceinline__ f32x2 conv1x1_sum_at(const float *__restrict__ parts, long long i, long long stride, int count) {
     f32x2 s = {0.0f, 0.0f};
     int k = 0;
     for (; k + 8 <= count; k += 8) {
@@ -1023,7 +1055,35 @@
       s = (s + v0) + v1;
     }
     for (; k < count; ++k) s += *reinterpret_cast<const f32x2 *>(parts + (long long)k * stride + i);
-    *reinterpret_cast<f32x2 *>(out + i) = s;
+    return s;
+}
+__device__ __forceinline__ void conv1x1_sum_body(const float *__restrict__ parts, float *__restrict__ out, long long n,
+                                                 long long stride, int count) {
+  for (long long i = (blockIdx.x * 256LL + threadIdx.x) * 2; i < n; i += gridDim.x * 512LL)
+    *reinterpret_cast<f32x2 *>(out + i) = conv1x1_sum_at(parts, i, stride, count);
+}
+__global__ __launch_bounds__(256) void conv1x1_sum(const float *__restrict__ parts, float *__restrict__ out,
+                                                   long long n, long long stride, int count) {
+  conv1x1_sum_body(parts, out, n, stride, count);
+}
+
+struct ConvSumGroup {
+  float *out[kConvGroupMax];
+};
+__global__ __launch_bounds__(256) void conv_group_sum(const float *__restrict__ parts, ConvSumGroup g, long long n, int count) {
+  const int p = blockIdx.y;
+  conv1x1_sum_body(parts + (long long)p * count * n, g.out[p], n, n, count);
+}
+__global__ __launch_bounds__(256) void conv_group_sum_all(const float *__restrict__ parts, float *__restrict__ out, long long n,
+                                                          int count, int problems) {
+  for (long long i = (blockIdx.x * 256LL + threadIdx.x) * 2; i < n; i += gridDim.x * 512LL) {
+    f32x2 t = {0.0f, 0.0f};
+    for (int p = 0; p < problems; ++p) {
+      const float *pp = parts + (long long)p * count * n;
+      const f32x2 v = count == 1 ? *reinterpret_cast<const f32x2 *>(pp + i) : conv1x1_sum_at(pp, i, n, count);
+      t = p == 0 ? v : t + v;
+    }
+    *reinterpret_cast<f32x2 *>(out + i) = t;
   }
 }
 
@@ -1122,8 +1182,8 @@
   }
 }
 
-__global__ __launch_bounds__(256) void conv3x3_wsum(const float *__restrict__ parts, float *__restrict__ out, int O, int C,
-                                                    int count) {
+__device__ __forceinline__ void conv3x3_wsum_body(const float *__restrict__ parts, float *__restrict__ out, int O, int C,
+                                                  int count) {
   const long long n = (long long)O * C * 9;
   for (long long i = blockIdx.x * 256LL + threadIdx.x; i < n; i += gridDim.x * 256LL) {
     const int o = (int)(i / (9 * C)), rem = (int)(i - (long long)o * 9 * C), t = rem / C, ch = rem - t * C;
@@ -1139,6 +1199,15 @@
     for (; k < count; ++k) s += parts[(long long)k * n + i];
     out[((long long)o * C + ch) * 9 + t] = s;
   }
+}
+__global__ __launch_bounds__(256) void conv3x3_wsum(const float *__restrict__ parts, float *__restrict__ out, int O, int C,
+                                                    int count) {
+  conv3x3_wsum_body(parts, out, O, C, count);
+}
+__global__ __launch_bounds__(256) void conv3x3_wsum_group(const float *__restrict__ parts, ConvSumGroup g, int O, int C,
+                                                          int count) {
+  const int p = blockIdx.y;
+  conv3x3_wsum_body(parts + (long long)p * count * O * C * 9, g.out[p], O, C, count);
 }
 
 template <int TAPS, int DX>
@@ -1548,6 +1617,26 @@
     conv_ntp_role<TAPS, false, ALIGNED>(a, bm, partial, M, N, L, B, n_mt, n_nt, stages_per_image, per, H, W, Cin, unit, smem, row_sums, rs_stride);
 }
 
+struct ConvNtpGroup {
+  const float *a[kConvGroupMax], *b[kConvGroupMax];
+  float *partial[kConvGroupMax];
+  int n;
+};
+template <int TAPS, bool ALIGNED>
+__global__ __launch_bounds__(kPThreads, 1) void conv_ntp_group(ConvNtpGroup g, int M, int N, int L, int B, int n_mt, int n_nt,
+                                                               int stages_per_image, int per, int H, int W, int Cin, int units) {
+  extern __shared__ __attribute__((aligned(16))) unsigned char smem[];
+  const int unit = xcd_tile(blockIdx.x, units * g.n);
+  if (unit >= units * g.n) return;
+  const int p = unit / units, u = unit - p * units;
+  if (threadIdx.x >= kPCons * 64)
+    conv_ntp_role<TAPS, true, ALIGNED>(g.a[p], g.b[p], g.partial[p], M, N, L, B, n_mt, n_nt, stages_per_image, per, H, W, Cin, u,
+                                       smem, nullptr, 0);
+  else
+    conv_ntp_role<TAPS, false, ALIGNED>(g.a[p], g.b[p], g.partial[p], M, N, L, B, n_mt, n_nt, stages_per_image, per, H, W, Cin, u,
+                                        smem, nullptr, 0);
+}
+
 namespace {
 
 int nt_splits(int tiles, int total_stages) {
@@ -1591,6 +1680,8 @@
     KGDET_HIP_TRY(hipFuncSetAttribute((const void *)conv_ntp<1, true>, hipFuncAttributeMaxDynamicSharedMemorySize, ntp_lds()));
     KGDET_HIP_TRY(hipFuncSetAttribute((const void *)conv_ntp<9, false>, hipFuncAttributeMaxDynamicSharedMemorySize, ntp_lds()));
     KGDET_HIP_TRY(hipFuncSetAttribute((const void *)conv_ntp<9, true>, hipFuncAttributeMaxDynamicSharedMemorySize, ntp_lds()));
+    KGDET_HIP_TRY(hipFuncSetAttribute((const void *)conv_ntp_group<9, false>, hipFuncAttributeMaxDynamicSharedMemorySize, ntp_lds()));
+    KGDET_HIP_TRY(hipFuncSetAttribute((const void *)conv_ntp_group<9, true>, hipFuncAttributeMaxDynamicSharedMemorySize, ntp_lds()));
     set = true;
   }
   return KGDET_OK;
@@ -2211,3 +2302,177 @@
   if (int rc = fold_args(f, w, s, mean, var, eps, bn_partial, P, grad_beta, grad_gamma)) return rc;
   return conv3x3_grad_weight_impl(grad_y, x, grad_w, B, O, C, H, W, workspace, workspace_bytes, stream, &f);
 }
+
+
+namespace kgdet {
+namespace {
+NNPlan plan_group(int n, long long B, int M, int K, int H, int W) {
+  return plan_nn(B * n, M, K, H, W, 9, 1);
+}
+int nt_splits_group(int n, int tiles, int total_stages) {
+  if (n <= 1) return nt_splits(tiles, total_stages);
+  const long long all = (long long)tiles * n;
+  const int most = (total_stages + 31) / 32;
+  const int s_max = (int)(2 * ((256 + all - 1) / all) < 128 ? 2 * ((256 + all - 1) / all) : 128);
+  double best = 1e30;
+  int splits = 1;
+  for (int s = 1; s <= s_max && s <= most; ++s) {
+    const double t = (double)((all * s + 255) / 256) / s;
+    if (t < best * (1.0 - 1e-9)) { best = t; splits = s; }
+  }
+  return splits;
+}
+struct GwShape {
+  int W_true, Wp, tiles, n_mt, n_nt, total;
+};
+bool gw_group_shape(int64_t B, int32_t O, int32_t C, int32_t H, int32_t W, GwShape &g) {
+  if (B <= 0 || O <= 0 || C <= 0 || H <= 0 || W < 4 || C % kTN != 0 || !ntp_on(9)) return false;
+  if ((long long)H * W > (1ll << 21) || (long long)(O > C ? O : C) * H * ((W + 3) & ~3) >= (1ll << 30)) return false;
+  g.W_true = W;
+  g.Wp = (W + 3) & ~3;
+  g.n_mt = (O + kTM - 1) / kTM;
+  g.n_nt = 9 * C / kTN;
+  g.tiles = g.n_mt * g.n_nt;
+  g.total = (int)(B * (((long long)H * g.Wp + kTK - 1) / kTK));
+  return true;
+}
+}
+}
+
+extern "C" int kgdet_conv3x3_group_ksplit(int32_t n, int64_t B, int32_t M, int32_t K, int32_t H, int32_t W) {
+  if (n < 1 || n > kConvGroupMax || B <= 0 || M <= 0 || K <= 0 || K % kTK || H <= 0 || W <= 0) return -1;
+  const NNPlan plan = plan_group(n, B, M, K, H, W);
+  return plan.patch ? plan.ks : -1;
+}
+
+extern "C" size_t kgdet_conv3x3_group_workspace_bytes(int32_t n, int64_t B, int32_t M, int32_t K, int32_t H, int32_t W,
+                                                      int32_t ksplit, int32_t sum_all) {
+  const int ks = ksplit > 0 ? ksplit : kgdet_conv3x3_group_ksplit(n, B, M, K, H, W);
+  if (ks < 1) return 0;
+  const long long parts = sum_all ? (long long)n * ks : (ks > 1 ? (long long)n * ks : 0);
+  return (size_t)parts * B * M * H * W * sizeof(float);
+}
+
+extern "C" int kgdet_conv3x3_group_apply(int32_t n, const void *const *packed, const float *const *x, float *const *y,
+                                         int32_t sum_all, int64_t B, int32_t M, int32_t K, int32_t H, int32_t W,
+                                         int32_t operand_format, int32_t ksplit, void *workspace, size_t workspace_bytes,
+                                         void *stream) {
+  const bool f16 = operand_format == 1;
+  KGDET_CHECK_SHAPE(n >= 1 && n <= kConvGroupMax, "a group holds 1..%d problems (%d)", kConvGroupMax, n);
+  KGDET_CHECK_SHAPE(B >= 0 && M > 0 && K > 0 && H >= 0 && W >= 0 && (long long)H * W < (1LL << 30), "bad sizes");
+  KGDET_CHECK_SHAPE(K % kTK == 0, "reduction length %d is not a multiple of 16", K);
+  const long long HW = (long long)H * W;
+  if (B * HW == 0) return KGDET_OK;
+  KGDET_CHECK_SHAPE(packed && x && y, "null pointer");
+  for (int p = 0; p < n; ++p) KGDET_CHECK_SHAPE(packed[p] && x[p] && ((sum_all && p > 0) || y[p]), "null pointer (problem %d)", p);
+  NNPlan plan = plan_group(n, B, M, K, H, W);
+  if (!plan.patch || !(conv_patch_mode() >= 2 || f16)) {
+    set_error("conv3x3_group_apply: no patch-kernel plan for [%lld, %d, %d, %d, %d]", (long long)B, M, K, H, W);
+    return KGDET_E_UNSUPPORTED;
+  }
+  if (ksplit > 0) plan.ks = ksplit;
+  const int ks = plan.ks, n_mt = (M + kTM - 1) / kTM;
+  const long long tiles = plan.tiles / n;
+  const long long part_stride = B * M * HW;
+  KGDET_CHECK_SHAPE(tiles * ks * 2 * n < (1LL << 28), "too many tiles");
+  const bool parts = sum_all || ks > 1;
+  if (parts) {
+    KGDET_CHECK_SHAPE(workspace && workspace_bytes >= (size_t)n * ks * part_stride * sizeof(float), "workspace too small");
+    KGDET_CHECK_SHAPE(part_stride % 2 == 0, "B*M*H*W must be even");
+  }
+  ConvPatchGroup g;
+  for (int p = 0; p < kConvGroupMax; ++p) {
+    const int q = p < n ? p : 0;
+    g.img[p] = (const unsigned char *)packed[q];
+    g.x[p] = x[q];
+    g.y[p] = parts ? (float *)workspace + (long long)q * ks * part_stride : y[q];
+  }
+  g.n = n;
+  const long long all = tiles * n;
+  const bool halves = (ks == 1 && all > 256 && all < 400) || M <= 64;
+#define KGDET_P4G_LAUNCH(WV, NBK, GRID, THR)                                                                                  \
+  do {                                                                                                                        \
+    if (f16) hipLaunchKernelGGL((conv3x3_patch4_group<WV, NBK, true>), dim3(GRID), dim3(THR), 0, (hipStream_t)stream, g, M, K, H, \
+                                W, n_mt, plan.tiles_x, plan.n_nt, (int)tiles, ks, part_stride, plan.TX, plan.TY);             \
+    else hipLaunchKernelGGL((conv3x3_patch4_group<WV, NBK, false>), dim3(GRID), dim3(THR), 0, (hipStream_t)stream, g, M, K, H,    \
+                            W, n_mt, plan.tiles_x, plan.n_nt, (int)tiles, ks, part_stride, plan.TX, plan.TY);                 \
+  } while (0)
+  if (plan.NB == 5)
+    KGDET_P4G_LAUNCH(4, 5, (all * ks + 7) / 8 * 8, 256);
+  else if (halves)
+    KGDET_P4G_LAUNCH(2, 4, (all * ks * 2 + 7) / 8 * 8, 128);
+  else
+    KGDET_P4G_LAUNCH(4, 4, (all * ks + 7) / 8 * 8, 256);
+#undef KGDET_P4G_LAUNCH
+  KGDET_CHECK_LAUNCH("conv3x3_patch4_group");
+  if (!parts) return KGDET_OK;
+  const long long blocks = (part_stride / 2 + 255) / 256;
+  const unsigned gx = (unsigned)(blocks > 2048 ? 2048 : blocks);
+  if (sum_all) {
+    hipLaunchKernelGGL(conv_group_sum_all, dim3(gx), dim3(256), 0, (hipStream_t)stream, (const float *)workspace, y[0],
+                       part_stride, ks, n);
+  } else {
+    ConvSumGroup s;
+    for (int p = 0; p < kConvGroupMax; ++p) s.out[p] = y[p < n ? p : 0];
+    hipLaunchKernelGGL(conv_group_sum, dim3(gx, n), dim3(256), 0, (hipStream_t)stream, (const float *)workspace, s, part_stride, ks);
+  }
+  KGDET_CHECK_LAUNCH("conv_group_sum");
+  return KGDET_OK;
+}
+
+extern "C" int kgdet_conv3x3_grad_weight_group_splits(int32_t n, int64_t B, int32_t O, int32_t C, int32_t H, int32_t W) {
+  GwShape s;
+  if (n < 1 || n > kConvGroupMax || !gw_group_shape(B, O, C, H, W, s)) return -1;
+  return nt_splits_group(n, s.tiles, s.total);
+}
+
+extern "C" size_t kgdet_conv3x3_grad_weight_group_workspace_bytes(int32_t n, int64_t B, int32_t O, int32_t C, int32_t H, int32_t W,
+                                                                  int32_t splits) {
+  if (splits <= 0) splits = kgdet_conv3x3_grad_weight_group_splits(n, B, O, C, H, W);
+  if (splits <= 0) return 0;
+  return (size_t)n * splits * O * C * 9 * sizeof(float);
+}
+
+extern "C" int kgdet_conv3x3_grad_weight_group(int32_t n, const float *const *grad_y, const float *const *x, float *const *grad_w,
+                                               int64_t B, int32_t O, int32_t C, int32_t H, int32_t W, int32_t splits,
+                                               void *workspace, size_t workspace_bytes, void *stream) {
+  KGDET_CHECK_SHAPE(n >= 1 && n <= kConvGroupMax, "a group holds 1..%d problems (%d)", kConvGroupMax, n);
+  GwShape s;
+  if (!gw_group_shape(B, O, C, H, W, s)) {
+    set_error("conv3x3_grad_weight_group: no conv_ntp plan for [%lld, %d, %d, %d, %d]", (long long)B, O, C, H, W);
+    return KGDET_E_UNSUPPORTED;
+  }
+  KGDET_CHECK_SHAPE(grad_y && x && grad_w && workspace, "null pointer");
+  for (int p = 0; p < n; ++p) KGDET_CHECK_SHAPE(grad_y[p] && x[p] && grad_w[p], "null pointer (problem %d)", p);
+  if (splits <= 0) splits = nt_splits_group(n, s.tiles, s.total);
+  KGDET_CHECK_SHAPE(splits <= 128, "too many pixel parts (%d)", splits);
+  const long long per_part = (long long)O * C * 9;
+  KGDET_CHECK_SHAPE(workspace_bytes >= (size_t)n * splits * per_part * sizeof(float), "workspace too small");
+  if (int rc = ntp_attr()) return rc;
+  ConvNtpGroup g;
+  ConvSumGroup out;
+  for (int p = 0; p < kConvGroupMax; ++p) {
+    const int q = p < n ? p : 0;
+    g.a[p] = grad_y[q];
+    g.b[p] = x[q];
+    g.partial[p] = (float *)workspace + (long long)q * splits * per_part;
+    out.out[p] = grad_w[q];
+  }
+  g.n = n;
+  const int L = H * s.W_true;
+  const int spi32 = (L + kPK - 1) / kPK, total32 = (int)(B * spi32), per32 = (total32 + splits - 1) / splits;
+  const int units = s.tiles * splits;
+  const unsigned grid = (unsigned)((units * n + 7) / 8 * 8);
+  if (s.W_true % 4 == 0)
+    hipLaunchKernelGGL((conv_ntp_group<9, true>), dim3(grid), dim3(kPThreads), ntp_lds(), (hipStream_t)stream, g, O, 9 * C, L,
+                       (int)B, s.n_mt, s.n_nt, spi32, per32, H, s.W_true, C, units);
+  else
+    hipLaunchKernelGGL((conv_ntp_group<9, false>), dim3(grid), dim3(kPThreads), ntp_lds(), (hipStream_t)stream, g, O, 9 * C, L,
+                       (int)B, s.n_mt, s.n_nt, spi32, per32, H, s.W_true, C, units);
+  KGDET_CHECK_LAUNCH("conv_ntp_group<9>");
+  const long long blocks = (per_part + 255) / 256;
+  hipLaunchKernelGGL(conv3x3_wsum_group, dim3((unsigned)(blocks > 4096 ? 4096 : blocks), n), dim3(256), 0, (hipStream_t)stream,
+                     (const float *)workspace, out, O, C, splits);
+  KGDET_CHECK_LAUNCH("conv3x3_wsum_group");
+  return KGDET_OK;
+}
diff --git a/kgdet_amd/heads.py b/kgdet_amd/heads.py
--- a/kgdet_amd/heads.py
+++ b/kgdet_amd/heads.py
@@ -8,7 +8,7 @@
 import torch.nn as nn
 
 from . import conv1x1, dcn, moment
-from .layers import ConvModule, bias_init_with_prob, normal_init
+from .layers import ConvModule, bias_init_with_prob, gn_act_applicable, gn_act_backward, gn_act_forward, normal_init
 from .points import (PointGenerator, dense_targets_applicable, multi_apply, point_target_kp,
                      point_target_kp_dense)
 from .postprocess import multiclass_nms_kp, multiclass_nms_kp_batched
@@ -164,6 +164,89 @@
             keypts_out = conv1x1.conv_bias_act(self.keypts_out, conv1x1.conv_bias_act(self.keypts_conv, pts_feat, relu=True))
             reppts_out = conv1x1.conv_bias_act(self.reppts_out, keypts_out)
         return cls_out, keypts_out, reppts_out
+
+
+FUSED_TOWERS = os.environ.get('KGDET_FUSED_TOWERS', '1') == '1'
+
+
+class _Towers(torch.autograd.Function):
+
+    @staticmethod
+    def forward(ctx, x, groups, eps, *flat):
+        n = len(flat) // 6
+        cur = [x, x]
+        saved, imgs_t = [], []
+        for i in range(n):
+            ws = [flat[6 * i].contiguous(), flat[6 * i + 3].contiguous()]
+            pairs = [conv1x1.forward_images(cur[t], ws[t], grad_input=True) for t in range(2)]
+            imgs_t.append([p[1] if p[1] is not None else conv1x1._pack(w, True) for p, w in zip(pairs, ws)])
+            z = conv1x1.apply_group([p[0] for p in pairs], cur, ws[0].shape[0],
+                                    ksplit=conv1x1.group_ksplit(1, cur[0], ws[0].shape[0]))
+            out = []
+            for t in range(2):
+                y, stats = gn_act_forward(z[t], flat[6 * i + 3 * t + 1], flat[6 * i + 3 * t + 2], groups, eps, True)
+                saved += [cur[t], z[t], y, stats]
+                out.append(y)
+            cur = out
+        ctx.save_for_backward(*(saved + list(flat)))
+        ctx.imgs_t, ctx.n, ctx.groups = imgs_t, n, groups
+        return cur[0], cur[1]
+
+    @staticmethod
+    def backward(ctx, g_cls, g_reg):
+        n, groups = ctx.n, ctx.groups
+        st = ctx.saved_tensors
+        saved, flat = st[:8 * n], st[8 * n:]
+        g = [gr if gr is not None else torch.zeros_like(saved[8 * (n - 1) + 4 * t + 2])
+             for t, gr in enumerate((g_cls, g_reg))]
+        grads = [None] * (6 * n)
+        xs, gzs, gx = [], [], None
+        for i in reversed(range(n)):
+            gz = []
+            for t in range(2):
+                inp, z, y, stats = saved[8 * i + 4 * t: 8 * i + 4 * t + 4]
+                gzt, sums = gn_act_backward(g[t], z, y, flat[6 * i + 3 * t + 1], stats, groups, True)
+                grads[6 * i + 3 * t + 1], grads[6 * i + 3 * t + 2] = sums[0], sums[1]
+                gz.append(gzt)
+                xs.append(inp)
+                gzs.append(gzt)
+            C = saved[8 * i].shape[1]
+            ks = conv1x1.group_ksplit(1, gz[0], C)
+            if i > 0:
+                g = conv1x1.apply_group(ctx.imgs_t[i], gz, C, ksplit=ks)
+            else:
+                gx = conv1x1.apply_group(ctx.imgs_t[0], gz, C, sum_all=True, ksplit=ks)
+        gws = conv1x1.grad_weight_group(xs, gzs, splits=conv1x1.grad_weight_group_splits(1, xs[0], gzs[0].shape[1]))
+        for k, i in enumerate(reversed(range(n))):
+            grads[6 * i], grads[6 * i + 3] = gws[2 * k], gws[2 * k + 1]
+        return (gx, None, None) + tuple(grads)
+
+
+def towers_applicable(cls_convs, reg_convs, x):
+    if not (FUSED_TOWERS and torch.is_grad_enabled() and len(cls_convs) == len(reg_convs) >= 1
+            and 2 * len(cls_convs) <= conv1x1.GROUP_MAX and x.dim() == 4 and x.is_contiguous()):
+        return False
+    C = x.shape[1]
+    gn = cls_convs[0].norm if cls_convs[0].with_norm else None
+    for m in list(cls_convs) + list(reg_convs):
+        conv = m.conv
+        if (type(conv) is not nn.Conv2d or conv.bias is not None or tuple(conv.kernel_size) != (3, 3)
+                or tuple(conv.stride) != (1, 1) or tuple(conv.padding) != (1, 1) or tuple(conv.dilation) != (1, 1)
+                or conv.groups != 1 or conv.in_channels != C or conv.out_channels != C
+                or m.order != ('conv', 'norm', 'act') or m.activation != 'relu' or not m.with_norm
+                or not isinstance(m.norm, nn.GroupNorm) or m.norm.num_groups != gn.num_groups or m.norm.eps != gn.eps
+                or m.norm.weight is None or m.norm.bias is None):
+            return False
+    w = cls_convs[0].conv.weight
+    return conv1x1.group_applicable(x, w) and gn_act_applicable(x, gn) and x.shape[2] * x.shape[3] % 2 == 0
+
+
+def towers(cls_convs, reg_convs, x):
+    flat = []
+    for c, r in zip(cls_convs, reg_convs):
+        flat += [c.conv.weight, c.norm.weight, c.norm.bias, r.conv.weight, r.norm.weight, r.norm.bias]
+    gn = cls_convs[0].norm
+    return _Towers.apply(x, gn.num_groups, gn.eps, *flat)
 
 
 def _normalised_loss(loss_module, pred, target, weight, normalize_term, avg_factor):
@@ -318,6 +401,7 @@
 
     def _init_layers(self):
         self.relu = nn.ReLU(inplace=False)
+        self.fused_towers = FUSED_TOWERS
         self.cls_convs = nn.ModuleList()
         self.reg_convs = nn.ModuleList()
         for i in range(self.stacked_convs):
@@ -338,12 +422,15 @@
             normal_init(m.conv, std=0.01)
 
     def forward_single(self, x):
-        cls_feat = x
-        pts_feat = x
-        for cls_conv in self.cls_convs:
-            cls_feat = cls_conv(cls_feat)
-        for reg_conv in self.reg_convs:
-            pts_feat = reg_conv(pts_feat)
+        if self.fused_towers and towers_applicable(self.cls_convs, self.reg_convs, x):
+            cls_feat, pts_feat = towers(self.cls_convs, self.reg_convs, x)
+        else:
+            cls_feat = x
+            pts_feat = x
+            for cls_conv in self.cls_convs:
+                cls_feat = cls_conv(cls_feat)
+            for reg_conv in self.reg_convs:
+                pts_feat = reg_conv(pts_feat)
 
         cls_out_1, keypts_out_1, reppts_out_1 = self.kp_rep_block_1(cls_feat, pts_feat)
         bbox_out_1 = self.points2bbox(reppts_out_1)
diff --git a/kgdet_amd/layers.py b/kgdet_amd/layers.py
--- a/kgdet_amd/layers.py
+++ b/kgdet_amd/layers.py
@@ -127,41 +127,50 @@
     return y
 
 
+def gn_act_forward(x, gamma, beta, groups, eps, relu):
+    from . import _lib
+    N, C = x.shape[0], x.shape[1]
+    HW = x.shape[2] * x.shape[3]
+    y = torch.empty_like(x)
+    stats = torch.empty((2, N * groups), dtype=torch.float32, device=x.device)
+    scratch = _gn_scratch(x, N, C, groups, HW)
+    _lib.check(_lib.lib().kgdet_gn_act_forward_split(
+        _lib.ptr(x), _lib.ptr(gamma), _lib.ptr(beta), ctypes.c_int32(groups), ctypes.c_float(eps),
+        ctypes.c_int32(1 if relu else 0), _lib.ptr(y), ctypes.c_void_p(stats[0].data_ptr()),
+        ctypes.c_void_p(stats[1].data_ptr()), _lib.ptr(scratch), ctypes.c_int64(N), ctypes.c_int32(C), ctypes.c_int64(HW),
+        _lib.current_stream()), 'gn_act_forward')
+    return y, stats
+
+
+def gn_act_backward(gy, x, y, gamma, stats, groups, relu, want_gx=True):
+    from . import _lib
+    N, C = x.shape[0], x.shape[1]
+    HW = x.shape[2] * x.shape[3]
+    gy = gy.contiguous()
+    gx = torch.empty_like(x) if want_gx else None
+    dgb = torch.empty((2, N, C), dtype=torch.float32, device=x.device)
+    scratch = _gn_scratch(x, N, C, groups, HW)
+    _lib.check(_lib.lib().kgdet_gn_act_backward_split(
+        _lib.ptr(gy), _lib.ptr(x), _lib.ptr(y), _lib.ptr(gamma), ctypes.c_void_p(stats[0].data_ptr()),
+        ctypes.c_void_p(stats[1].data_ptr()), ctypes.c_int32(groups), ctypes.c_int32(1 if relu else 0),
+        _lib.ptr(gx), _lib.ptr(dgb), _lib.ptr(scratch), ctypes.c_int64(N), ctypes.c_int32(C), ctypes.c_int64(HW),
+        _lib.current_stream()), 'gn_act_backward')
+    return gx, (dgb.sum(1) if N > 1 else dgb[:, 0])
+
+
 class _GNAct(torch.autograd.Function):
 
     @staticmethod
     def forward(ctx, x, gamma, beta, groups, eps, relu):
-        from . import _lib
-        N, C = x.shape[0], x.shape[1]
-        HW = x.shape[2] * x.shape[3]
-        y = torch.empty_like(x)
-        stats = torch.empty((2, N * groups), dtype=torch.float32, device=x.device)
-        scratch = _gn_scratch(x, N, C, groups, HW)
-        _lib.check(_lib.lib().kgdet_gn_act_forward_split(
-            _lib.ptr(x), _lib.ptr(gamma), _lib.ptr(beta), ctypes.c_int32(groups), ctypes.c_float(eps),
-            ctypes.c_int32(1 if relu else 0), _lib.ptr(y), ctypes.c_void_p(stats[0].data_ptr()),
-            ctypes.c_void_p(stats[1].data_ptr()), _lib.ptr(scratch), ctypes.c_int64(N), ctypes.c_int32(C), ctypes.c_int64(HW),
-            _lib.current_stream()), 'gn_act_forward')
+        y, stats = gn_act_forward(x, gamma, beta, groups, eps, relu)
         ctx.save_for_backward(x, y if relu else None, gamma, stats)
         ctx.groups, ctx.relu, ctx.has_beta = groups, relu, beta is not None
         return y
 
     @staticmethod
     def backward(ctx, gy):
-        from . import _lib
         x, y, gamma, stats = ctx.saved_tensors
-        N, C = x.shape[0], x.shape[1]
-        HW = x.shape[2] * x.shape[3]
-        gy = gy.contiguous()
-        gx = torch.empty_like(x) if ctx.needs_input_grad[0] else None
-        dgb = torch.empty((2, N, C), dtype=torch.float32, device=x.device)
-        scratch = _gn_scratch(x, N, C, ctx.groups, HW)
-        _lib.check(_lib.lib().kgdet_gn_act_backward_split(
-            _lib.ptr(gy), _lib.ptr(x), _lib.ptr(y), _lib.ptr(gamma), ctypes.c_void_p(stats[0].data_ptr()),
-            ctypes.c_void_p(stats[1].data_ptr()), ctypes.c_int32(ctx.groups), ctypes.c_int32(1 if ctx.relu else 0),
-            _lib.ptr(gx), _lib.ptr(dgb), _lib.ptr(scratch), ctypes.c_int64(N), ctypes.c_int32(C), ctypes.c_int64(HW),
-            _lib.current_stream()), 'gn_act_backward')
-        sums = dgb.sum(1) if N > 1 else dgb[:, 0]
+        gx, sums = gn_act_backward(gy, x, y, gamma, stats, ctx.groups, ctx.relu, ctx.needs_input_grad[0])
         ggamma = sums[0] if (gamma is not None and ctx.needs_input_grad[1]) else None
         gbeta = sums[1] if (ctx.has_beta and ctx.needs_input_grad[2]) else None
         return gx, ggamma, gbeta, None, None, None
```

Result: faster. 186.8 img/s (median of 6 runs) (+1.4%).
